# numericalEFT/FeynmanDiagram.jl

Hardware: AMD Instinct MI355X
Metric: graph-evaluations/sec (higher is better)
Workload: dtype f64

## Files before the change

### feynmandiagram.jl_amd/capi.py

```python
from __future__ import annotations

import ctypes as C
import os
from typing import Optional

import numpy as np

from .nodetable import NodeTable

_HERE = os.path.dirname(os.path.abspath(__file__))
LIB_PATH = os.environ.get("FDG_LIBRARY") or os.path.join(_HERE, "lib", "libfdg.so")
KERNEL_CACHE = os.path.join(_HERE, "kernel_cache")

FDG_OK = 0
FDG_E_INVALID, FDG_E_UNSUPPORTED, FDG_E_NO_DEVICE, FDG_E_NOMEM, FDG_E_JIT, FDG_E_INTERNAL = -1, -2, -3, -4, -5, -6
FDG_SPEC_DEFAULT, FDG_SPEC_KEEP_SOURCE, FDG_SPEC_FAST_MATH, FDG_SPEC_ISA, FDG_SPEC_AUTOTUNE = 0, 1, 2, 4, 8
FDG_DT_F64, FDG_DT_F32, FDG_DT_C64, FDG_DT_C32 = 0, 1, 2, 3
DTYPES = {"Float64": FDG_DT_F64, "Float32": FDG_DT_F32, "ComplexF64": FDG_DT_C64, "ComplexF32": FDG_DT_C32}
FDG_SPEC_ROW_MAJOR_COMPANION = 16
FDG_ASSOC_STATIC, FDG_ASSOC_INTERP = 0, 1
FDG_TILE_SAMPLES = 64

EXPORTS = [
    "fdg_last_error", "fdg_version", "fdg_graph_create", "fdg_graph_destroy", "fdg_graph_query",
    "fdg_graph_emit_source", "fdg_free", "fdg_graph_specialize", "fdg_eval_device", "fdg_eval",
    "fdg_accumulate_device", "fdg_fill_uniform_device", "fdg_copy_device", "fdg_read_device", "fdg_clock_probe_device", "fdg_graph_specialize_typed", "fdg_eval_device_typed", "fdg_graph_create_complex_view", "fdg_isa_check_hazards", "fdg_graph_release_device", "fdg_powi",
    "fdg_eval_strided", "fdg_graph_coop_program", "fdg_graph_set_opt_params", "fdg_graph_opt_program", "fdg_graph_set_schedule_groups", "fdg_leaf_eval_device", "fdg_leaf_eval_device_tiled",
    "fdg_comm_unique_id", "fdg_comm_create", "fdg_comm_destroy", "fdg_reduce_device",
    "fdg_graph_specialize_fused", "fdg_mc_eval_device", "fdg_mc_accumulate_device", "fdg_graph_mc_program",
    "fdg_graph_kernel_info",
    "fdg_eval_device_tiled", "fdg_accumulate_device_tiled", "fdg_fill_uniform_device_tiled", "fdg_graph_set_association",
    "fdg_batch_alloc", "fdg_batch_free", "fdg_graph_pool_program", "fdg_batch_alloc_pair", "fdg_graph_set_option", "fdg_graph_get_option", "fdg_set_default_option", "fdg_get_default_option", "fdg_selftest_pair_search",
    "fdg_repack_tile_major", "fdg_unpack_tile_major",
    "fdg_accumulate_device_binned", "fdg_mc_accumulate_device_binned",
    "fdg_accumulate_device_moments", "fdg_mc_accumulate_device_moments",
    "fdg_vegas_sample_device", "fdg_accumulate_device_vegas", "fdg_mc_accumulate_device_vegas", "fdg_vegas_refine",
    "fdg_vegas_sample_device_discrete", "fdg_accumulate_device_vegas_binned", "fdg_mc_accumulate_device_vegas_binned",
    "fdg_vegas_refine_discrete",
    "fdg_vegas_sample_device_polar", "fdg_sincos",
    "fdg_matsubara_phase", "fdg_accumulate_device_matsubara", "fdg_mc_accumulate_device_matsubara",
    "fdg_vegas_sample_device_grouped", "fdg_accumulate_device_grouped", "fdg_mc_accumulate_device_grouped",
    "fdg_accumulate_device_observables", "fdg_mc_accumulate_device_observables",
    "fdg_accumulate_device_freq_observables", "fdg_mc_accumulate_device_freq_observables",
    "fdg_vegas_sample_device_strat", "fdg_accumulate_device_strat", "fdg_mc_accumulate_device_strat", "fdg_strat_allocate",
    "fdg_vegas_sample_device_strat_grouped", "fdg_accumulate_device_strat_grouped", "fdg_mc_accumulate_device_strat_grouped",
    "fdg_strat_allocate_cols",
    "fdg_chain_propose_device", "fdg_chain_step_device", "fdg_mc_chain_step_device", "fdg_chain_reduce_device",
    "fdg_chain_step_device_matsubara", "fdg_mc_chain_step_device_matsubara",
    "fdg_chain_step_device_grouped", "fdg_mc_chain_step_device_grouped",
    "fdg_chain_propose_device_discrete", "fdg_chain_step_device_binned", "fdg_mc_chain_step_device_binned",
    "fdg_chain_propose_device_polar",
]
FDG_BIN_MAX = 16384
FDG_VEGAS_DIM_MAX, FDG_VEGAS_GRID_MAX = 64, 1024
FDG_VEGAS_EXT_MAX = 16
FDG_VEGAS_POLAR_MAX = 21
FDG_MATSUBARA_FREQ_MAX = 64
FDG_WEIGHT_GROUP_MAX = 8
FDG_OBS_MAX = 16
FDG_FREQ_OBS_MAX = 8
FDG_STRAT_CUBE_MAX = 1 << 20
FDG_CHAIN_INIT, FDG_CHAIN_MEASURE = 1, 2
FDG_CHAIN_BIN_MAX = 64
COMM_ID_BYTES = 128


class FdgLibraryMissing(ImportError):
    pass


class FdgError(RuntimeError):
    def __init__(self, code: int, msg: str):
        super().__init__(f"fdg error {code}: {msg}")
        self.code = code


class GraphDesc(C.Structure):
    _fields_ = [("n_leaf", C.c_uint32), ("n_node", C.c_uint32), ("n_root", C.c_uint32), ("n_edge", C.c_uint32),
                ("op", C.POINTER(C.c_uint8)), ("power", C.POINTER(C.c_int32)),
                ("child_off", C.POINTER(C.c_uint32)), ("child_idx", C.POINTER(C.c_uint32)),
                ("child_fac", C.POINTER(C.c_double)), ("root_slot", C.POINTER(C.c_uint32))]


class GraphInfo(C.Structure):
    _fields_ = [("n_leaf", C.c_uint32), ("n_node", C.c_uint32), ("n_root", C.c_uint32), ("n_edge", C.c_uint32),
                ("n_live_node", C.c_uint32), ("n_live_leaf", C.c_uint32),
                ("flops_alg", C.c_uint64), ("bytes_alg", C.c_uint64),
                ("max_live", C.c_uint32), ("n_slot_lds", C.c_uint32), ("n_slot_mem", C.c_uint32),
                ("n_ops", C.c_uint32), ("specialized", C.c_int32),
                ("spec_vgpr", C.c_uint32), ("spec_lds_bytes", C.c_uint32), ("spec_scratch_bytes", C.c_uint32)]

    def asdict(self):
        return {k: int(getattr(self, k)) for k, _ in self._fields_}


class KernelInfo(C.Structure):
    _fields_ = [("last_kernel", C.c_char * 48), ("n_valu", C.c_uint64 * 3), ("n_ld_leaf", C.c_uint32 * 3),
                ("n_panel", C.c_uint32 * 3), ("n_lds", C.c_uint32 * 3), ("waves_per_cu", C.c_uint32 * 3),
                ("has_acc", C.c_uint32), ("has_rm", C.c_uint32), ("has_coop", C.c_uint32), ("rm_bufs", C.c_uint32),
                ("has_pool", C.c_uint32), ("pool_fetch", C.c_uint32), ("pool_valu", C.c_uint64),
                ("has_rl", C.c_uint32), ("rl_reserved", C.c_uint32), ("rl_valu", C.c_uint64)]


class LeafTables(C.Structure):
    _fields_ = [("n_leaf", C.c_uint32), ("n_basis", C.c_uint32), ("n_loop", C.c_uint32), ("dim", C.c_uint32),
                ("n_tau", C.c_uint32), ("leaf_type", C.c_void_p), ("leaf_order", C.c_void_p), ("tau_in", C.c_void_p),
                ("tau_out", C.c_void_p), ("loop_index", C.c_void_p), ("basis", C.c_void_p),
                ("kF", C.c_double), ("beta", C.c_double), ("lambda_", C.c_double)]


class Matsubara(C.Structure):
    _fields_ = [("n_freq", C.c_uint32), ("fermionic", C.c_int32), ("freq", C.c_void_p), ("root_tau_in", C.c_void_p),
                ("root_tau_out", C.c_void_p), ("beta", C.c_double), ("d_T", C.c_void_p), ("t_sample_stride", C.c_int64),
                ("t_comp_stride", C.c_int64), ("n_tau", C.c_uint32), ("d_acc_re", C.c_void_p), ("d_acc_im", C.c_void_p),
                ("d_acc2_re", C.c_void_p), ("d_acc2_im", C.c_void_p)]


class ChainMatsubara(C.Structure):
    _fields_ = [("n_freq", C.c_uint32), ("fermionic", C.c_int32), ("freq", C.c_void_p), ("weight_freq", C.c_uint32),
                ("root_col_in", C.c_void_p), ("root_col_out", C.c_void_p), ("beta", C.c_double)]


class ChainGroups(C.Structure):
    _fields_ = [("n_group", C.c_uint32), ("root_group", C.c_void_p), ("var_mask", C.c_void_p), ("reweight", C.c_void_p)]


class WeightGroups(C.Structure):
    _fields_ = [("n_group", C.c_uint32), ("root_group", C.c_void_p), ("var_mask", C.c_void_p), ("weight_group_stride", C.c_int64)]


class Observables(C.Structure):
    _fields_ = [("n_obs", C.c_uint32), ("coef", C.c_void_p), ("d_obs", C.c_void_p), ("d_cov", C.c_void_p)]


class FreqObservables(C.Structure):
    _fields_ = [("n_obs", C.c_uint32), ("coef", C.c_void_p), ("d_fobs", C.c_void_p), ("d_fcov", C.c_void_p)]


class OptParams(C.Structure):
    _fields_ = [("n_reg", C.c_uint32), ("n_lds", C.c_uint32), ("lookahead_lds", C.c_uint32),
                ("lookahead_mem", C.c_uint32), ("lookahead_leaf", C.c_uint32), ("n_acc", C.c_uint32),
                ("vn_window", C.c_uint32), ("fma", C.c_uint32), ("remat_window", C.c_uint32), ("remat_cost", C.c_uint32)]


class MOp(C.Structure):
    _fields_ = [("kind", C.c_uint8), ("nega", C.c_uint8), ("negb", C.c_uint8), ("negc", C.c_uint8),
                ("d", C.c_uint32), ("a", C.c_uint32), ("b", C.c_uint32), ("imm", C.c_double),
                ("c", C.c_uint32), ("param", C.c_uint32)]


MOP_DTYPE = np.dtype([("kind", "u1"), ("nega", "u1"), ("negb", "u1"), ("negc", "u1"),
                      ("d", "<u4"), ("a", "<u4"), ("b", "<u4"), ("imm", "<f8"), ("c", "<u4"), ("param", "<u4")])

_lib = None


class BatchPairInfo(C.Structure):
    _fields_ = [("leaf_bytes", C.c_uint64), ("root_bytes", C.c_uint64), ("chunk_tiles", C.c_uint64), ("n_chunk", C.c_uint32),
                ("n_candidate", C.c_uint32), ("n_filler", C.c_uint32), ("n_probe", C.c_uint32), ("n_matched", C.c_uint32),
                ("calibrated", C.c_uint32), ("gbs_fast", C.c_double), ("gbs_slow", C.c_double), ("gbs_before_mean", C.c_double),
                ("gbs_before_min", C.c_double), ("gbs_after_mean", C.c_double), ("gbs_after_min", C.c_double), ("seconds", C.c_double),
                ("seconds_settling", C.c_double), ("level_reached", C.c_uint32), ("span_gb", C.c_uint32)]


def lib():
    global _lib
    if _lib is not None:
        return _lib
    if not os.path.exists(LIB_PATH):
        raise FdgLibraryMissing(
            f"{LIB_PATH} not found: build the HIP extension first "
            "(python -c 'import __graft_entry__ as g; g.build()' or make -C feynmandiagram.jl_amd/csrc). "
            "There is no CPU fallback for the evaluator.")
    if not os.environ.get("FDG_NO_TORCH_PRELOAD"):
        try:
            import torch
        except ImportError:
            pass
    L = C.CDLL(LIB_PATH)
    vp, i64, u64, u32, dp = C.c_void_p, C.c_int64, C.c_uint64, C.c_uint32, C.c_void_p
    L.fdg_last_error.restype = C.c_char_p
    L.fdg_version.restype = C.c_int
    L.fdg_graph_create.argtypes = [C.POINTER(GraphDesc), C.POINTER(vp)]
    L.fdg_graph_destroy.argtypes = [vp]
# ... 132 lines not shown
def check(rc: int):
    if rc != 0:
        raise FdgError(rc, lib().fdg_last_error().decode("utf-8", "replace"))


class GraphHandle:

    def __init__(self, table: NodeTable):
        t = table.normalized()
        t.validate()
        self.table = t
        d = GraphDesc()
        d.n_leaf, d.n_node, d.n_root, d.n_edge = t.n_leaf, t.n_node, t.n_root, t.n_edge
        d.op = t.op.ctypes.data_as(C.POINTER(C.c_uint8))
        d.power = t.power.ctypes.data_as(C.POINTER(C.c_int32))
        d.child_off = t.child_off.ctypes.data_as(C.POINTER(C.c_uint32))
        d.child_idx = t.child_idx.ctypes.data_as(C.POINTER(C.c_uint32))
        d.child_fac = t.child_fac.ctypes.data_as(C.POINTER(C.c_double))
        d.root_slot = t.root_slot.ctypes.data_as(C.POINTER(C.c_uint32))
        h = C.c_void_p()
        check(lib().fdg_graph_create(C.byref(d), C.byref(h)))
        self._h = h
        if getattr(t, "sched_group", None) is not None:
            self.set_schedule_groups(t.sched_group)

    def complex_view(self) -> "GraphHandle":
        from .nodetable import complex_to_real
        h = C.c_void_p()
        check(lib().fdg_graph_create_complex_view(self._h, C.byref(h)))
        v = GraphHandle.__new__(GraphHandle)
        v.table = complex_to_real(self.table)
        v._h = h
        return v

    def set_option(self, name: str, value=None):
        check(lib().fdg_graph_set_option(self._h, name.encode(), None if value is None else str(value).encode()))

    def set_options(self, options):
        for k, v in (options or {}).items():
            self.set_option(k, v)

    def get_option(self, name: str):
        v = lib().fdg_graph_get_option(self._h, name.encode())
        return None if v is None else v.decode()

    def set_association(self, assoc: int):
        check(lib().fdg_graph_set_association(self._h, assoc))

    def set_schedule_groups(self, group):
        if group is None:
            check(lib().fdg_graph_set_schedule_groups(self._h, None, 0))
            return
        g = np.ascontiguousarray(group, dtype=np.uint32)
        check(lib().fdg_graph_set_schedule_groups(self._h, g.ctypes.data, g.shape[0]))

    def close(self):
        if getattr(self, "_h", None):
            lib().fdg_graph_destroy(self._h)
            self._h = None

    def __del__(self):
        try:
            self.close()
        except Exception:
            pass

    @property
    def ptr(self):
        return self._h

    def info(self) -> dict:
        gi = GraphInfo()
        check(lib().fdg_graph_query(self._h, C.byref(gi)))
        return gi.asdict()

    def kernel_info(self) -> dict:
        ki = KernelInfo()
        check(lib().fdg_graph_kernel_info(self._h, C.byref(ki)))
        out = {"last_kernel": ki.last_kernel.decode()}
        for k in ("n_valu", "n_ld_leaf", "n_panel", "n_lds", "waves_per_cu"):
            out[k] = [int(x) for x in getattr(ki, k)]
        for k in ("has_acc", "has_rm", "has_coop", "rm_bufs", "has_pool", "pool_fetch", "pool_valu", "has_rl", "rl_valu"):
            out[k] = int(getattr(ki, k))
        return out

    def emit_source(self, flags: int = 0) -> str:
        s = C.c_char_p()
        check(lib().fdg_graph_emit_source(self._h, flags, C.byref(s)))
        try:
            return s.value.decode()
        finally:
            lib().fdg_free(s)

    def set_opt_params(self, n_reg=0, n_lds=0, lookahead_lds=0, lookahead_mem=0, lookahead_leaf=0, n_acc=0, vn_window=0, fma=0, remat_window=0, remat_cost=0):
        q = OptParams(n_reg, n_lds, lookahead_lds, lookahead_mem, lookahead_leaf, n_acc, vn_window, fma, remat_window, remat_cost)
        check(lib().fdg_graph_set_opt_params(self._h, C.byref(q)))

    def opt_program(self, n_reg=0, n_lds=0, lookahead_lds=0, lookahead_mem=0, lookahead_leaf=0, n_acc=0, vn_window=0, fma=0, remat_window=0, remat_cost=0):
        q = OptParams(n_reg, n_lds, lookahead_lds, lookahead_mem, lookahead_leaf, n_acc, vn_window, fma, remat_window, remat_cost)
        ops = C.POINTER(MOp)()
        n = C.c_uint64()
        nr, nl, nm, na = C.c_uint32(), C.c_uint32(), C.c_uint32(), C.c_uint32()
        check(lib().fdg_graph_opt_program(self._h, C.byref(q), C.byref(ops), C.byref(n), C.byref(nr), C.byref(nl),
                                          C.byref(nm), C.byref(na)))
        try:
            buf = C.string_at(ops, n.value * C.sizeof(MOp))
            arr = np.frombuffer(buf, dtype=MOP_DTYPE).copy()
        finally:
            lib().fdg_free(ops)
        self.last_n_acc = na.value
        return arr, nr.value, nl.value, nm.value

    def mc_program(self, tables, n_reg=0, n_lds=0, lookahead_lds=0, lookahead_mem=0, lookahead_leaf=0, n_acc=0, vn_window=0, fma=0, remat_window=0, remat_cost=0):
        q = OptParams(n_reg, n_lds, lookahead_lds, lookahead_mem, lookahead_leaf, n_acc, vn_window, fma, remat_window, remat_cost)
        ops = C.POINTER(MOp)()
        n = C.c_uint64()
        nr, nl, nm, na = C.c_uint32(), C.c_uint32(), C.c_uint32(), C.c_uint32()
        check(lib().fdg_graph_mc_program(self._h, C.byref(tables), C.byref(q), C.byref(ops), C.byref(n), C.byref(nr),
                                         C.byref(nl), C.byref(nm), C.byref(na)))
        try:
            arr = np.frombuffer(C.string_at(ops, n.value * C.sizeof(MOp)), dtype=MOP_DTYPE).copy()
        finally:
            lib().fdg_free(ops)
        return arr, nr.value, nl.value, nm.value

    def pool_program(self, **kw):
        return self.coop_program(_pooled=True, **kw)

    def coop_program(self, _pooled=False, **kw):
        q = OptParams(kw.get("n_reg", 0), kw.get("n_lds", 0), kw.get("lookahead_lds", 0), kw.get("lookahead_mem", 0),
                      kw.get("lookahead_leaf", 0), kw.get("n_acc", 0), kw.get("vn_window", 0), 0, 0, 0)
        progs, per_wave = [], []
        info = None
        for w in range(16):
            ops = C.POINTER(MOp)()
            n = C.c_uint64()
            inf = (C.c_uint32 * 8)()
            rc = (lib().fdg_graph_pool_program if _pooled else lib().fdg_graph_coop_program)(self._h, C.byref(q), w, C.byref(ops), C.byref(n), inf)
            if rc != 0 and w >= 4:
                break
            check(rc)
            try:
                progs.append(np.frombuffer(C.string_at(ops, n.value * C.sizeof(MOp)), dtype=MOP_DTYPE).copy())
            finally:
                lib().fdg_free(ops)
            per_wave.append(dict(n_reg=inf[0], n_lds=inf[1], n_mem=inf[2], n_acc=inf[3]))
            info = dict(n_shared=inf[4], n_epoch=inf[5], n_transfer=inf[6], n_duplicate=inf[7], waves=per_wave)
        return progs, info

    def specialize(self, cache_dir: Optional[str] = None, flags: int = 0):
        check(lib().fdg_graph_specialize(self._h, cache_dir.encode() if cache_dir else None, flags))

    def specialize_typed(self, dtype: int, cache_dir: Optional[str] = None, flags: int = 0):
        check(lib().fdg_graph_specialize_typed(self._h, dtype, cache_dir.encode() if cache_dir else None, flags))

    def eval_device_typed(self, dtype: int, d_leaf: int, ss: int, ls: int, d_root: int, rs: int, rk: int, B: int, stream: int = 0):
        check(lib().fdg_eval_device_typed(self._h, dtype, d_leaf, ss, ls, d_root, rs, rk, B, stream))

    def eval_device(self, d_leaf: int, ss: int, ls: int, d_root: int, rs: int, rk: int, B: int, stream: int = 0):
        check(lib().fdg_eval_device(self._h, d_leaf, ss, ls, d_root, rs, rk, B, stream))

    def accumulate_device(self, d_leaf: int, ss: int, ls: int, d_weight: int, d_acc: int, B: int, stream: int = 0):
        check(lib().fdg_accumulate_device(self._h, d_leaf, ss, ls, d_weight or None, d_acc, B, stream))

    def eval_device_tiled(self, d_leaf: int, ss: int, ls: int, lts: int, d_root: int, rs: int, rk: int, rts: int, B: int, stream: int = 0):
        check(lib().fdg_eval_device_tiled(self._h, d_leaf, ss, ls, lts, d_root, rs, rk, rts, B, stream))
# ... 1367 lines not shown
```

### feynmandiagram.jl_amd/csrc/fdg_internal.h

```cpp
#pragma once
#include <cstdint>
#include <mutex>
#include <string>
#include <vector>

#include "../../include/fdg.h"
#include "fdg_knobs.h"

namespace fdg {

constexpr uint32_t SP_LDS = 0u, SP_MEM = 1u, SP_LEAF = 2u;
constexpr uint32_t LOC_FAC = 1u << 29;
constexpr uint32_t LOC_IDX_MASK = (1u << 29) - 1u;
inline uint32_t mkloc(uint32_t space, uint32_t idx) { return (space << 30) | idx; }

constexpr uint32_t UOP_SUM = 0, UOP_PROD = 1, UOP_POW = 2, UOP_ROOT = 3, UOP_LEAF = 4, UOP_END = 5, UOP_PRODI = 6;

struct Lowered {
  uint32_t L = 0, N = 0, R = 0, E = 0;
  std::vector<uint8_t> op;
  std::vector<int32_t> power;
  std::vector<uint32_t> off, idx;
  std::vector<double> fac;
  std::vector<uint32_t> root_slot;

  std::vector<uint32_t> sched_group;
  bool assoc_interp = false;

  std::vector<uint8_t> live;
  std::vector<uint32_t> order;
  uint32_t n_live_leaf = 0;
  uint64_t flops_alg = 0;
  uint32_t max_live = 0;

  uint32_t lds_slots = 0;
  uint32_t mem_slots = 0;
  std::vector<uint32_t> code;
  uint32_t n_ops = 0;
  uint64_t opnd_lds = 0, opnd_mem = 0, opnd_leaf = 0;
};

int validate_desc(const fdg_graph_desc *d, std::string &err);
struct RealTwinTable { uint32_t n_leaf = 0; std::vector<uint8_t> op; std::vector<int32_t> power; std::vector<uint32_t> off, idx, root_slot; std::vector<double> fac; };
bool complex_to_real_table(const Lowered &p, RealTwinTable &out, std::string &why);
void analyse(Lowered &p);
void build_interpreter_program(Lowered &p, uint32_t lds_slot_budget);

std::string emit_hip_source(const Lowered &p, unsigned flags);
std::string emit_hip_source_typed(const Lowered &p, int dtype, bool &ok, std::string &why);
std::string emit_fused_source(const Lowered &p, const std::string &leaf_stmts, const std::string &device_functions);

void set_error(const std::string &s);

double powi(double x, int32_t n);

}

struct fdg_ws_set {
  void *key = nullptr;
  void *d_ws = nullptr, *d_ws2 = nullptr, *d_ws3 = nullptr, *d_ws4 = nullptr;
  size_t ws_bytes = 0, ws2_bytes = 0, ws3_bytes = 0, ws4_bytes = 0;
  void *s2 = nullptr, *ev_t[2] = {nullptr, nullptr}, *ev_k[2] = {nullptr, nullptr}, *ev_in = nullptr;
  uint64_t last_use = 0;
};

struct fdg_launch_cfg {
  bool no_rl = false, no_fused_acc = false, no_pool = false, pool_no_acc = false, no_streaming = false, no_w2 = false, no_coop = false, no_rm = false;
  bool transpose_narrow = false;
  uint32_t root_scratch_min = 16;
  uint64_t root_scratch_mb = 256;
  int waves_per_cu = 0;
  int oversub = 0;
  long mem_waves = -1;
  long mem_oversub = 1;
  double mem_ratio = 2.5;
  uint64_t sm_chunk_bytes = 1ull << 29;
  long long eval_chunk = 0, mc_chunk = 0;
};

enum { FDG_K_EVAL = 0, FDG_K_NT, FDG_K_W2, FDG_K_ACC, FDG_K_ACC_NT, FDG_K_RM, FDG_K_RM_ACC, FDG_K_RL, FDG_K_RL_ACC, FDG_K_COOP, FDG_K_POOL, FDG_K_COUNT };
static const char *const FDG_ISA_KERNEL[FDG_K_COUNT] = {"fdg_isa_eval", "fdg_isa_eval_nt", "fdg_isa_eval_w2", "fdg_isa_eval_acc", "fdg_isa_eval_acc_nt",
    "fdg_isa_eval_rm", "fdg_isa_eval_rm_acc", "fdg_isa_eval_rl", "fdg_isa_eval_rl_acc", "fdg_isa_eval_coop", "fdg_isa_eval_pool"};
inline const char *fdg_isa_suffix(int k) { return FDG_ISA_KERNEL[k] + sizeof("fdg_isa_eval") - 1; }
struct fdg_isa_kernel {
  bool present = false;
  void *fn = nullptr;
  uint32_t vgpr = 0, lds_bytes = 0, mem_slots = 0, threads = 64;
};

struct fdg_graph {
  fdg::Lowered prog;
  fdg::KnobMap knobs;
  fdg_launch_cfg cfg;
  fdg_opt_params opt = {0, 0, 0, 0, 0, 0, 0, 0, 0, 0};
  bool has_opt = false;
  std::vector<fdg_ws_set> ws_pool;
  void *ws_key = nullptr;
  bool ws_bound = true;
  uint64_t ws_clock = 0;
  std::vector<char> code_object;
  std::string spec_source_hash;
  unsigned spec_flags = 0;
  uint32_t spec_vgpr = 0, spec_lds = 0, spec_scratch = 0;
  std::mutex mu;
  void *d_code = nullptr;
  void *d_root_live = nullptr;
  void *d_ws = nullptr;
  size_t ws_bytes = 0;
  void *module = nullptr;
  void *fn_eval_sm = nullptr, *fn_eval_gen = nullptr;
  bool isa = false;
  bool isa_fma = false;
  fdg_isa_kernel kern[FDG_K_COUNT];
  uint64_t st_valu[3] = {0, 0, 0};
  uint32_t st_ld_leaf[3] = {0, 0, 0}, st_panel[3] = {0, 0, 0}, st_lds[3] = {0, 0, 0};
  const char *last_kernel = "";
  uint32_t rm_bufs = 0;
  uint64_t rl_valu = 0;
  bool coop_enabled = false;
  uint32_t coop_panel_wg = 0;
  uint32_t pool_panel_wg = 0, pool_fetch = 0, pool_unit = 1;
  uint64_t pool_valu = 0;
  std::vector<char> alt_code;
  void *alt_module = nullptr, *fn_alt_sm = nullptr, *fn_alt_gen = nullptr;
  std::vector<char> fused_code;
  void *fused_module = nullptr, *fn_fused = nullptr;
  std::vector<char> typed_code[4];
  void *typed_module[4] = {nullptr, nullptr, nullptr, nullptr}, *fn_typed[4] = {nullptr, nullptr, nullptr, nullptr};
  fdg_graph *cx_twin = nullptr;
  bool cx_twin_tried = false;
  int mc_route = 0;
  std::vector<int32_t> lt_i32[5];
  std::vector<double> lt_basis;
  uint32_t lt_hdr[5] = {0, 0, 0, 0, 0};
  std::vector<char> mc_code;
  void *mc_module = nullptr;
  bool mc_built = false;
  fdg_isa_kernel mc_kern[FDG_K_COUNT];
  std::string mc_dir;
  unsigned mc_flags = 0;
  void *d_ws4 = nullptr;
  size_t ws4_bytes = 0;
  void *d_ws2 = nullptr;
  size_t ws2_bytes = 0;
  void *d_ws3 = nullptr;
  size_t ws3_bytes = 0;
  void *s2 = nullptr;
  void *ev_t[2] = {nullptr, nullptr}, *ev_k[2] = {nullptr, nullptr}, *ev_in = nullptr;
  int device = -1;
  int n_cu = 0;
};

#ifdef FDG_RUNTIME_TU
#include <hip/hip_runtime.h>
#define HIP_TRY(expr)                                                                   \
  do {                                                                                  \
    hipError_t e_ = (expr);                                                             \
    if (e_ != hipSuccess) {                                                             \
      fdg::set_error(std::string(#expr) + ": " + hipGetErrorString(e_));                     \
      return FDG_E_NO_DEVICE;                                                           \
    }                                                                                   \
  } while (0)

__device__ __forceinline__ void philox4x32_10(uint32_t c0, uint32_t c1, uint32_t c2, uint32_t c3,
                                              uint32_t k0, uint32_t k1, uint32_t out[4]) {
#pragma unroll
  for (int r = 0; r < 10; ++r) {
    const uint64_t p0 = (uint64_t)0xD2511F53u * c0;
    const uint64_t p1 = (uint64_t)0xCD9E8D57u * c2;
    const uint32_t n0 = (uint32_t)(p1 >> 32) ^ c1 ^ k0;
    const uint32_t n1 = (uint32_t)p1;
    const uint32_t n2 = (uint32_t)(p0 >> 32) ^ c3 ^ k1;
    const uint32_t n3 = (uint32_t)p0;
    c0 = n0; c1 = n1; c2 = n2; c3 = n3;
    k0 += 0x9E3779B9u; k1 += 0xBB67AE85u;
  }
  out[0] = c0; out[1] = c1; out[2] = c2; out[3] = c3;
}

__device__ __forceinline__ double fdg_philox_u53(uint64_t sample, uint32_t column, uint64_t seed) {
  uint32_t o[4];
  philox4x32_10((uint32_t)sample, (uint32_t)(sample >> 32), column, 0u, (uint32_t)seed, (uint32_t)(seed >> 32), o);
  const uint64_t m = ((uint64_t)(o[0] >> 5) << 26) | (uint64_t)(o[1] >> 6);
  return (double)m * 0x1.0p-53;
}

void parse_launch_cfg(fdg_graph *g);
int ensure_device(fdg_graph *g);
int fdg_bind_stream_ws(fdg_graph *g, void *stream);
int ensure_ws(fdg_graph *g, size_t bytes);
int fdg_run_locked(fdg_graph *g, int mode, const double *d_leaf, int64_t ss, int64_t ls, double *d_root, int64_t rs, int64_t rk,
                   const double *d_weight, double *d_acc, int64_t B, hipStream_t st,
                   int64_t lts = 0, int64_t rts = 0);
int launch_reduce_partials(const double *partial, uint32_t nblk, uint32_t R, double *acc, hipStream_t st);
int ensure_root_scratch(fdg_graph *g, size_t need);
int root_live_mask(fdg_graph *g, const uint8_t **out);
int fdg_mc_run_locked(fdg_graph *g, int mode, const double *d_K, int64_t ks, int64_t kc, const double *d_T, int64_t ts, int64_t tc,
                      double kF, double beta, double lambda, double *d_root, int64_t rs, int64_t rk, const double *d_weight,
                      double *d_acc, int64_t B, hipStream_t st);
// ... 15 lines not shown
```

### feynmandiagram.jl_amd/csrc/fdg_isa.cpp

```cpp
#include <algorithm>
#include <cctype>
#include <cinttypes>
#include <cmath>
#include <cstdio>
#include <cstdlib>
#include <cstring>
#include <map>
#include <sstream>

#include "fdg_opt.h"

namespace fdg {
namespace {

constexpr int V_LANE8 = 1, V_LEAFOFF = 2, V_ROOTOFF = 3, V_TMP = 4, V_BASE = 6;
constexpr int S_LEAF = 4, S_SS = 6, S_LS = 8, S_ROOT = 10, S_RS = 12, S_RK = 14, S_WS = 16, S_B = 18, S_NWG = 20;
constexpr int S_TILE = 22, S_NTILES = 23, S_LT = 24, S_RT = 26, S_PANEL = 28, S_LS8 = 30, S_RK8 = 32, S_A = 34,
              S_T = 36, S_C = 38, S_X = 40;
constexpr int S_WGT = 44;
constexpr int S_RTS = 44;
constexpr int S_LTS = 46;
constexpr int S_LP = 48;
constexpr int S_DELTA = 50;
constexpr int N_DELTA = 6;
constexpr int S_POOL = S_DELTA + 2 * N_DELTA;
constexpr int N_POOL = 20;
constexpr int S_END = S_POOL + 2 * N_POOL;
constexpr int N_POOL_MC = 13;
constexpr int S_PARAM = S_POOL + 2 * N_POOL_MC;
constexpr int S_LEAF2 = S_PARAM + 2 * MC_N_PARAM, S_LS82 = S_LEAF2 + 2, S_LT2 = S_LEAF2 + 4;
static_assert(S_LT2 + 2 == S_END && S_PARAM % 4 == 0 && S_LEAF2 % 4 == 0, "SGPR map");

const double kLog2e = 0x1.71547652b82fep+0, kLn2Hi = 0x1.62e42fefa39efp-1, kLn2Lo = 0x1.abc9e3b39803fp-56;
constexpr int kExpDeg = 11;
const double kExpC[kExpDeg + 1] = {0x1.0000000000000p+0, 0x1.0000000000000p+0, 0x1.0000000000011p-1, 0x1.555555555555ap-3,
                                   0x1.555555554f0a5p-5, 0x1.111111110f218p-7, 0x1.6c16c18804745p-10, 0x1.a01a01b148c00p-13,
                                   0x1.a019919593233p-16, 0x1.71ddf5667e394p-19, 0x1.28b41ab9f014bp-22, 0x1.af63371ef88d9p-26};


enum HzRes : uint8_t { HZ_VGPR, HZ_SGPR  };
enum HzProd : uint8_t {
  HP_TRANS,
  HP_VALU_SGPR,
  HP_VALU_VGPR,
  HP_STORE_WIDE,
  HP_SALU_SGPR,
};
enum HzCons : uint8_t {
  HC_VALU_READ,
  HC_DIV_FMAS,
  HC_VMEM_SADDR,
  HC_LANE_READ,
  HC_VALU_WRITE,
  HC_LDS_DIRECT,
};
struct HzRule { HzProd prod; HzCons cons; HzRes res; int wait; const char *what; };
const HzRule kHazards[] = {
    {HP_TRANS, HC_VALU_READ, HZ_VGPR, 2, "trans result -> VALU read (gfx940: not forwarded; measured: stale read with 0)"},
    {HP_VALU_SGPR, HC_VALU_READ, HZ_SGPR, 2, "VALU write of SGPR/VCC -> VALU read as mask/carry/constant (gfx940; measured with v_cmp -> v_cndmask)"},
    {HP_VALU_SGPR, HC_DIV_FMAS, HZ_SGPR, 4, "VALU write of VCC -> v_div_fmas"},
    {HP_VALU_SGPR, HC_VMEM_SADDR, HZ_SGPR, 5, "VALU write of SGPR -> VMEM/SMEM read of it"},
    {HP_VALU_VGPR, HC_LANE_READ, HZ_VGPR, 2, "VALU write of VGPR -> v_readlane/v_readfirstlane (measured: stale read with 0)"},
    {HP_STORE_WIDE, HC_VALU_WRITE, HZ_VGPR, 2, "store data wider than 64 bits -> VALU overwrite of the data registers"},
    {HP_SALU_SGPR, HC_VMEM_SADDR, HZ_SGPR, 0, "SALU write of SGPR -> VMEM read of it: interlocked by hardware (every leaf load does this back to back)"},
    {HP_SALU_SGPR, HC_LDS_DIRECT, HZ_SGPR, 1, "SALU write of M0 -> LDS-direct load (global_load_lds_*)"},
};
constexpr int HZ_MAX_WAIT = 5;

constexpr int HR_AGPR = 512, HR_SGPR = 1024, HR_VCC = 1024 + 106, HR_EXEC = 1024 + 126, HR_M0 = 1024 + 124;
struct HzInst {
  std::string op;
  bool valu = false, salu = false, vmem = false, ds = false, smem = false, trans = false, lane_read = false, div_fmas = false, store = false, lds_direct = false;
  int nop = 0;
  std::vector<int> wr, rd;
  std::vector<int> store_wide;
};
static bool hz_starts(const std::string &s, const char *p) { return s.compare(0, std::strlen(p), p) == 0; }
static void hz_parse_reg(std::string t, int &first, int &n) {
  first = 0; n = 0;
  while (!t.empty() && (t[0] == '-' || t[0] == '|' || t[0] == ' ')) t.erase(0, 1);
  while (!t.empty() && (t.back() == '|' || t.back() == ' ')) t.pop_back();
  if (t == "vcc") { first = HR_VCC; n = 2; return; }
  if (t == "vcc_lo") { first = HR_VCC; n = 1; return; }
  if (t == "vcc_hi") { first = HR_VCC + 1; n = 1; return; }
  if (t == "exec") { first = HR_EXEC; n = 2; return; }
  if (t == "m0") { first = HR_M0; n = 1; return; }
  if (t.size() < 2 || (t[0] != 'v' && t[0] != 's' && t[0] != 'a')) return;
  const int base = t[0] == 'v' ? 0 : (t[0] == 'a' ? HR_AGPR : HR_SGPR);
  if (t[1] == '[') {
    int a = 0, b = 0;
    if (std::sscanf(t.c_str() + 2, "%d:%d", &a, &b) == 2 && b >= a) { first = base + a; n = b - a + 1; }
    return;
  }
  if (t[1] < '0' || t[1] > '9') return;
  first = base + std::atoi(t.c_str() + 1); n = 1;
}
static HzInst hz_decode(const std::string &line) {
  HzInst I;
  size_t p = 0;
  while (p < line.size() && (line[p] == ' ' || line[p] == '\t')) ++p;
  size_t q = p;
  while (q < line.size() && line[q] != ' ' && line[q] != '\t') ++q;
  I.op = line.substr(p, q - p);
  std::vector<std::string> opnd;
  {
    std::string rest = line.substr(q), cur;
    int depth = 0;
    for (char c : rest) {
      if (c == '[') depth++;
      if (c == ']') depth--;
      if (c == ',' && depth == 0) { opnd.push_back(cur); cur.clear(); } else cur.push_back(c);
    }
    if (!cur.empty()) opnd.push_back(cur);
    for (std::string &o : opnd) {
      while (!o.empty() && (o[0] == ' ' || o[0] == '\t')) o.erase(0, 1);
      const size_t sp = o.find_first_of(" \t");
      if (sp != std::string::npos) o.erase(sp);
    }
  }
  auto add = [](std::vector<int> &v, const std::string &t) { int f, n; hz_parse_reg(t, f, n); for (int i = 0; i < n; ++i) v.push_back(f + i); };
  const std::string &op = I.op;
  if (op == "s_nop") { I.salu = true; I.nop = (opnd.empty() ? 0 : std::atoi(opnd[0].c_str())) + 1; return I; }
  if (hz_starts(op, "s_waitcnt") || op == "s_endpgm" || op == "s_barrier" || hz_starts(op, "s_cbranch") || op == "s_branch") { I.salu = true; return I; }
  if (hz_starts(op, "s_load") || hz_starts(op, "s_buffer_load")) {
    I.smem = true;
    if (!opnd.empty()) add(I.wr, opnd[0]);
    for (size_t i = 1; i < opnd.size(); ++i) add(I.rd, opnd[i]);
    return I;
  }
  if (hz_starts(op, "s_")) {
    I.salu = true;
    const bool nodst = hz_starts(op, "s_cmp") || hz_starts(op, "s_setpc") || hz_starts(op, "s_bitcmp");
    for (size_t i = 0; i < opnd.size(); ++i) add((i == 0 && !nodst) ? I.wr : I.rd, opnd[i]);
    if (hz_starts(op, "s_addc") || hz_starts(op, "s_subb") || hz_starts(op, "s_cselect")) {}
    return I;
  }
  if (hz_starts(op, "global_load") || hz_starts(op, "global_store") || hz_starts(op, "buffer_") || hz_starts(op, "flat_")) {
    I.vmem = true;
    I.store = op.find("store") != std::string::npos;
    if (op.find("_lds_") != std::string::npos) {
      I.lds_direct = true;
      I.rd.push_back(HR_M0);
      for (size_t i = 0; i < opnd.size(); ++i) add(I.rd, opnd[i]);
      return I;
    }
    const bool wide = op.find("dwordx3") != std::string::npos || op.find("dwordx4") != std::string::npos;
    for (size_t i = 0; i < opnd.size(); ++i) {
      if (!I.store && i == 0) add(I.wr, opnd[i]);
      else { add(I.rd, opnd[i]); if (I.store && i == 1 && wide) add(I.store_wide, opnd[i]); }
    }
    return I;
  }
  if (hz_starts(op, "ds_")) {
    I.ds = true;
    I.store = hz_starts(op, "ds_write");
    const bool wide = op.find("b96") != std::string::npos || op.find("b128") != std::string::npos;
    for (size_t i = 0; i < opnd.size(); ++i) {
      if (!I.store && i == 0) add(I.wr, opnd[i]);
      else { add(I.rd, opnd[i]); if (I.store && i == 1 && wide) add(I.store_wide, opnd[i]); }
    }
    return I;
  }
  if (hz_starts(op, "v_")) {
    I.valu = true;
    static const char *trans[] = {"v_rcp_", "v_rsq_", "v_sqrt_", "v_exp_", "v_log_", "v_sin_", "v_cos_"};
    for (const char *t : trans) if (hz_starts(op, t)) I.trans = true;
    I.lane_read = hz_starts(op, "v_readlane") || hz_starts(op, "v_readfirstlane");
    I.div_fmas = hz_starts(op, "v_div_fmas");
    size_t ndst = 1;
    if (hz_starts(op, "v_div_scale") || ((hz_starts(op, "v_add_co") || hz_starts(op, "v_sub_co") || hz_starts(op, "v_addc_co") || hz_starts(op, "v_subb_co")) && opnd.size() >= 4)) ndst = 2;
    if (hz_starts(op, "v_cmpx")) { ndst = 0; I.wr.push_back(HR_EXEC); I.wr.push_back(HR_EXEC + 1); }
    for (size_t i = 0; i < opnd.size(); ++i) add(i < ndst ? I.wr : I.rd, opnd[i]);
    if (I.div_fmas) { I.rd.push_back(HR_VCC); I.rd.push_back(HR_VCC + 1); }
    return I;
  }
  return I;
}
static bool hz_is_inst(const std::string &line) {
  size_t p = 0;
  while (p < line.size() && (line[p] == ' ' || line[p] == '\t')) ++p;
  if (p >= line.size() || line[p] == '.' || line[p] == ';' || line[p] == '/' || line[p] == '-') return false;
  const size_t q = line.find_first_of(" \t", p);
  const std::string w = line.substr(p, q == std::string::npos ? std::string::npos : q - p);
  if (!w.empty() && w.back() == ':') return false;
  return hz_starts(w, "s_") || hz_starts(w, "v_") || hz_starts(w, "ds_") || hz_starts(w, "global_") || hz_starts(w, "buffer_") || hz_starts(w, "flat_");
}

struct HzTracker {
  struct Past { HzInst inst; int age; };
  std::vector<Past> past;
  int missing(const HzInst &I, const char **why = nullptr) const {
    int need = 0;
    auto has = [](const std::vector<int> &v, int r) { return std::find(v.begin(), v.end(), r) != v.end(); };
    for (const Past &P : past) {
      for (const HzRule &R : kHazards) {
        if (R.wait <= P.age) continue;
        const std::vector<int> *pr = nullptr;
        switch (R.prod) {
          case HP_TRANS: if (P.inst.trans) pr = &P.inst.wr; break;
          case HP_VALU_SGPR: if (P.inst.valu) pr = &P.inst.wr; break;
          case HP_VALU_VGPR: if (P.inst.valu) pr = &P.inst.wr; break;
          case HP_STORE_WIDE: if (!P.inst.store_wide.empty()) pr = &P.inst.store_wide; break;
          case HP_SALU_SGPR: if (P.inst.salu) pr = &P.inst.wr; break;
        }
        if (!pr) continue;
        const std::vector<int> *cr = nullptr;
        switch (R.cons) {
          case HC_VALU_READ: if (I.valu && !I.div_fmas) cr = &I.rd; break;
          case HC_DIV_FMAS: if (I.div_fmas) cr = &I.rd; break;
          case HC_VMEM_SADDR: if (I.vmem || I.smem) cr = &I.rd; break;
          case HC_LANE_READ: if (I.lane_read) cr = &I.rd; break;
          case HC_VALU_WRITE: if (I.valu) cr = &I.wr; break;
          case HC_LDS_DIRECT: if (I.lds_direct) cr = &I.rd; break;
        }
        if (!cr) continue;
        for (int r : *pr) {
          const bool sg = r >= HR_SGPR;
          if ((R.res == HZ_SGPR) != sg) continue;
          if (R.cons == HC_LDS_DIRECT && r != HR_M0) continue;
          if (has(*cr, r)) { if (R.wait - P.age > need) { need = R.wait - P.age; if (why) *why = R.what; } break; }
// ... 138 lines not shown

std::string f64_inline(double f, bool &ok) {
  ok = true;
  if (f == 0.5) return "0.5";
  if (f == -0.5) return "-0.5";
  if (f == 2.0) return "2.0";
  if (f == -2.0) return "-2.0";
  if (f == 4.0) return "4.0";
  if (f == -4.0) return "-4.0";
  if (f == 1.0) return "1.0";
  if (f == -1.0) return "-1.0";
  ok = false;
  return "";
}

std::string hex32(uint32_t v) {
  char b[16];
  std::snprintf(b, sizeof b, "0x%08x", v);
  return b;
}

void emit_scaled_addr(Emit &E, int dst, int base, int mul8, uint32_t k) {
  if (k == 0) {
    E.ins("s_mov_b64 s[" + std::to_string(dst) + ":" + std::to_string(dst + 1) + "], s[" + std::to_string(base) + ":" +
          std::to_string(base + 1) + "]");
    return;
  }
  const std::string ks = hex32(k);
  E.ins("s_mul_i32 s" + std::to_string(S_X) + ", s" + std::to_string(mul8) + ", " + ks);
  E.ins("s_mul_hi_u32 s" + std::to_string(S_X + 1) + ", s" + std::to_string(mul8) + ", " + ks);
  E.ins("s_mul_i32 s" + std::to_string(S_X + 2) + ", s" + std::to_string(mul8 + 1) + ", " + ks);
  E.ins("s_add_u32 s" + std::to_string(S_X + 1) + ", s" + std::to_string(S_X + 1) + ", s" + std::to_string(S_X + 2));
  E.ins("s_add_u32 s" + std::to_string(dst) + ", s" + std::to_string(base) + ", s" + std::to_string(S_X));
  E.ins("s_addc_u32 s" + std::to_string(dst + 1) + ", s" + std::to_string(base + 1) + ", s" + std::to_string(S_X + 1));
}

struct KernelMeta { std::string name; uint32_t lds_bytes, accum, n_agpr; int n_args, n_sgpr; uint32_t wg = 64; };

constexpr uint32_t RM_CHUNK = 16, RM_BUF_BYTES = 64 * RM_CHUNK * 8, RM_WINDOW = 800;
struct RmFetch { uint32_t chunk, buf; };
static void rm_plan(const Lowered &p, const OptProgram &prog, uint32_t rm_bufs, std::vector<std::vector<RmFetch>> &rm_fetch,
                    std::vector<int> &rm_ld_buf) {
  const uint32_t rm_full = p.L / RM_CHUNK, rm_tail = (p.L % RM_CHUNK) ? 1u : 0u, n_chunk = rm_full + rm_tail;
  auto rm_chunk_of = [&](uint32_t leaf) { return leaf < rm_full * RM_CHUNK ? leaf / RM_CHUNK : rm_full; };
  const uint32_t G = (prog.params.rm_pair && rm_bufs >= 4 && rm_bufs % 2 == 0) ? 2u : 1u;
  const uint32_t n_unit = (n_chunk + G - 1) / G, n_ubuf = rm_bufs / G;
  const size_t n_ops = prog.ops.size();
  rm_fetch.assign(n_ops + 1, {});
  rm_ld_buf.assign(n_ops, -1);
  std::vector<std::vector<size_t>> uses(n_unit);
  for (size_t q = 0; q < n_ops; ++q) if (prog.ops[q].kind == M_LD_LEAF) uses[rm_chunk_of(prog.ops[q].a) / G].push_back(q);
  std::vector<size_t> cursor(uses.size(), 0);
  std::vector<int64_t> resident(n_ubuf, -1);
  std::vector<size_t> free_from(n_ubuf, 0);
  for (size_t q = 0; q < n_ops; ++q) {
    if (prog.ops[q].kind != M_LD_LEAF) continue;
    const uint32_t c = rm_chunk_of(prog.ops[q].a), u = c / G;
    cursor[u]++;
    int b = -1;
    for (uint32_t k = 0; k < n_ubuf; ++k) if (resident[k] == (int64_t)u) b = (int)k;
    if (b < 0) {
      size_t soon = 1;
      for (size_t k = cursor[u]; k < uses[u].size() && uses[u][k] <= q + RM_WINDOW; ++k) soon++;
      if (soon < 3) continue;
      size_t far = 0;
      for (uint32_t k = 0; k < n_ubuf; ++k) {
        size_t nu;
        if (resident[k] < 0) nu = std::numeric_limits<size_t>::max();
        else { const auto &uu = uses[(size_t)resident[k]]; const size_t cu = cursor[(size_t)resident[k]]; nu = cu < uu.size() ? uu[cu] : std::numeric_limits<size_t>::max() - 1; }
        if (b < 0 || nu > far) { b = (int)k; far = nu; }
      }
      for (uint32_t k = 0; k < G && G * u + k < n_chunk; ++k)
        rm_fetch[std::min(free_from[(size_t)b], q)].push_back(RmFetch{G * u + k, G * (uint32_t)b + k});
      resident[(size_t)b] = u;
    }
    rm_ld_buf[q] = (int)(G * (uint32_t)b + c % G);
    free_from[(size_t)b] = q + 1;
  }
}

struct CoopSec { uint32_t wave, n_shared, priv_base_bytes, panel_wg_bytes, panel_prefix_bytes; bool pooled = false; uint32_t pool_unit = 1;
                 uint32_t slack = 0, flag_base_bytes = 0, n_wave = 4; };
static KernelMeta emit_kernel(Emit &E, const Lowered &p, const OptProgram &prog, const std::string &kname, int W, bool accumulate = false,
                              uint32_t rm_bufs = 0, const CoopSec *cs = nullptr, bool rl = false) {
  E.vm_issued = E.lg_issued = E.vm_done = E.lg_done = 0;
  E.pend.assign(std::max<uint32_t>(prog.n_reg_used, 1), {0, 0});
  const uint32_t SLOT = 512u * W;
  const uint32_t stage_base = (prog.n_lds_used * SLOT + 1023u) & ~1023u;
  const uint32_t rl_image = rl ? ((512u * p.L + 1023u) & ~1023u) : 0u;
  const uint32_t lds_bytes = rl ? stage_base + rl_image : (rm_bufs ? stage_base + rm_bufs * RM_BUF_BYTES : prog.n_lds_used * SLOT);
  const uint32_t panel_bytes_per_wave = std::max<uint32_t>(prog.n_mem_used, 1) * SLOT;
  const int RW = 2 * W;
  const int TSH = W == 2 ? 7 : 6;
  const std::string sfx = "_" + kname;
  std::ostringstream &os = E.os;
  if (!cs) {
    os << "\t.text\n\t.protected\t" << kname << "\n\t.globl\t" << kname << "\n\t.p2align\t8\n\t.type\t" << kname << ",@function\n";
    os << kname << ":\n";
    E.off = 0;
    E.klabel = kname;
    E.pad_ok = true;
    for (int i = 0; i < E.shift; ++i) E.ins("s_nop 0");
  } else {
    os << ".Lsec" << sfx << ":\n";
  }
  auto S = [](int r) { return "s" + std::to_string(r); };
  auto S2 = [](int r) { return "s[" + std::to_string(r) + ":" + std::to_string(r + 1) + "]"; };
  auto V = [](int r) { return "v" + std::to_string(r); };
  auto vlo = [&](uint32_t r) { const int b = V_BASE + RW * r; return "v[" + std::to_string(b) + ":" + std::to_string(b + 1) + "]"; };
  auto vhi = [&](uint32_t r) { const int b = V_BASE + RW * r + 2; return "v[" + std::to_string(b) + ":" + std::to_string(b + 1) + "]"; };
  auto vall = [&](uint32_t r) { const int b = V_BASE + RW * r; return "v[" + std::to_string(b) + ":" + std::to_string(b + RW - 1) + "]"; };
  const std::string LD = W == 2 ? "global_load_dwordx4 " : "global_load_dwordx2 ";
  const std::string ST = W == 2 ? "global_store_dwordx4 " : "global_store_dwordx2 ";
  const std::string leaf_policy_env = fdg::knob("FDG_ISA_LEAF_POLICY") ? std::string(" ") + fdg::knob("FDG_ISA_LEAF_POLICY") : std::string();
  const std::string root_policy = fdg::knob("FDG_ISA_ROOT_POLICY") ? std::string(" ") + fdg::knob("FDG_ISA_ROOT_POLICY") : std::string(E.streaming || (cs && cs->pooled) ? " nt" : "");
  std::vector<uint8_t> final_load(prog.ops.size(), 0);
  if (E.streaming) {
    const long nt_dist = fdg::knob("FDG_ISA_NT_DIST") ? std::atol(fdg::knob("FDG_ISA_NT_DIST")) : E.nt_dist;
    std::vector<long> next_at(p.L + 1, -1);
    long ord = 0;
    for (size_t i = prog.ops.size(); i-- > 0;)
      if ((prog.ops[i].kind == M_LD_LEAF || prog.ops[i].kind == M_LD_LEAF_ACC) && prog.ops[i].a < next_at.size()) {
        const uint32_t a = prog.ops[i].a;
        if (next_at[a] < 0 || (nt_dist >= 0 && ord - next_at[a] > nt_dist)) final_load[i] = 1;
        next_at[a] = ord++;
      }
  }
  std::string leaf_policy = leaf_policy_env;
  const std::string DSR = W == 2 ? "ds_read_b128 " : "ds_read_b64 ";
  const std::string DSW = W == 2 ? "ds_write_b128 " : "ds_write_b64 ";

  const char *dbg = fdg::knob("FDG_ISA_DEBUG");
  const bool dbg_noleaf = dbg && std::strstr(dbg, "noleaf");
  const bool dbg_nolds = dbg && std::strstr(dbg, "nolds");
  const bool use_ldexp = fdg::knob("FDG_ISA_NO_LDEXP") == nullptr;
  const bool dbg_novalu = dbg && std::strstr(dbg, "novalu");
  const bool dbg_nopanel = dbg && std::strstr(dbg, "nopanel");
  const bool dbg_norecv = dbg && std::strstr(dbg, "norecv");
  const bool dbg_nofetch = dbg && std::strstr(dbg, "nopoolfetch");
  const bool dbg_noacc = dbg && std::strstr(dbg, "noacc");
  const bool dbg_nohead = dbg && std::strstr(dbg, "nohead");
  bool in_head = true;
  int tile_run = 0;
  if (dbg && std::strstr(dbg, "chunk") && !cs) tile_run = std::max(0, std::min(9, std::atoi(std::strstr(dbg, "chunk") + 5)));
  const bool tile_xcd = dbg && std::strstr(dbg, "xcd") && !cs && !tile_run;
  int tile_rot = 0;
  if (dbg && std::strstr(dbg, "rot") && !cs && !tile_run && !tile_xcd) tile_rot = std::max(0, std::atoi(std::strstr(dbg, "rot") + 3));
  const int S_ROTB = S_POOL + 2 * (N_POOL - 1), S_ROTS = S_ROTB + 1;
  E.vm_slack = (dbg && std::strstr(dbg, "noackwait") && !accumulate) ? p.R : 0;
  E.no_vm_wait = dbg && std::strstr(dbg, "novmwait");
  if (cs) E.ins("v_and_b32_e32 v0, 63, v0");
  E.ins("s_load_dwordx8 s[4:11], s[0:1], 0x0");
  E.ins("s_load_dwordx8 s[12:19], s[0:1], 0x20");
  E.ins("s_load_dwordx2 s[20:21], s[0:1], 0x40");
  if (accumulate) E.ins("s_load_dwordx2 " + S2(S_WGT) + ", s[0:1], 0x48");
  const uint32_t n_k = prog.mc_n_k;
  const bool mc = n_k > 0 || prog.mc_n_t > 0;
  const bool tm_imm = dbg && std::strstr(dbg, "tmimm") && !mc && !rm_bufs && !rl && !cs && W == 1;
  int64_t tm_base = -1;
  const int tile_arg = mc ? 0x80 : 0x50;
  E.ins("s_load_dwordx2 " + S2(S_LTS) + ", s[0:1], " + hex32((uint32_t)tile_arg));
  if (!accumulate) E.ins("s_load_dwordx2 " + S2(S_RTS) + ", s[0:1], " + hex32((uint32_t)tile_arg + 8));
  if (mc) {
    E.ins("s_load_dwordx4 s[" + std::to_string(S_LEAF2) + ":" + std::to_string(S_LEAF2 + 3) + "], s[0:1], 0x50");
    E.ins("s_load_dwordx8 s[" + std::to_string(S_PARAM) + ":" + std::to_string(S_PARAM + 7) + "], s[0:1], 0x60");
  }
  E.ins("s_waitcnt lgkmcnt(0)");
  uint64_t w_seq = 0;
  const uint32_t acc0 = V_BASE + RW * std::max<uint32_t>(prog.n_reg_used, 1);
  const bool aa = accumulate && prog.params.acc_in_agpr;
  const uint32_t A0 = RW * prog.n_acc_used;
  const uint32_t acc_pairs_v = accumulate ? (aa ? 3 : p.R + 2) : 0;
  const uint32_t wgt0 = aa ? acc0 : acc0 + 2 * p.R;
  auto vpair = [&](uint32_t b) { return "v[" + std::to_string(b) + ":" + std::to_string(b + 1) + "]"; };
  auto vacc = [&](uint32_t k) { return vpair(acc0 + 2 * k); };
  const std::string vwgt = vpair(wgt0), vtmp = vpair(wgt0 + 2), vtmp2 = vpair(wgt0 + 4);
  auto acc_to_tmp2 = [&](uint32_t k) {
    E.ins("v_accvgpr_read_b32 v" + std::to_string(wgt0 + 4) + ", a" + std::to_string(A0 + 2 * k));
    E.ins("v_accvgpr_read_b32 v" + std::to_string(wgt0 + 5) + ", a" + std::to_string(A0 + 2 * k + 1));
  };
  auto tmp2_to_acc = [&](uint32_t k) {
    E.ins("v_accvgpr_write_b32 a" + std::to_string(A0 + 2 * k) + ", v" + std::to_string(wgt0 + 4));
    E.ins("v_accvgpr_write_b32 a" + std::to_string(A0 + 2 * k + 1) + ", v" + std::to_string(wgt0 + 5));
  };
  bool has_macro = false;
  uint32_t n_tmp_pairs = 0;
  for (const MOp &o : prog.ops) { if (mop_is_macro(o.kind)) has_macro = true; n_tmp_pairs = std::max(n_tmp_pairs, mop_tmp_pairs(o.kind)); }
  const uint32_t tmp0 = acc0 + 2 * acc_pairs_v;
  auto tpair = [&](uint32_t k) { return "v[" + std::to_string(tmp0 + 2 * k) + ":" + std::to_string(tmp0 + 2 * k + 1) + "]"; };
  const std::string tA = tpair(0), tB = tpair(1), tC = tpair(2), tD = tpair(3);
  auto tAd = [&](int h) { return "v" + std::to_string(tmp0 + h); };
  if (accumulate)
    for (uint32_t k = 0; k < p.R; ++k) {
      if (aa) {
        E.ins("v_accvgpr_write_b32 a" + std::to_string(A0 + 2 * k) + ", 0");
        E.ins("v_accvgpr_write_b32 a" + std::to_string(A0 + 2 * k + 1) + ", 0");
        continue;
      }
      E.ins("v_mov_b32_e32 v" + std::to_string(acc0 + 2 * k) + ", 0");
      E.ins("v_mov_b32_e32 v" + std::to_string(acc0 + 2 * k + 1) + ", 0");
    }
  E.ins("v_lshlrev_b32_e32 " + V(V_LANE8) + ", " + std::to_string(W == 2 ? 4 : 3) + ", v0");
  E.ins("v_mul_lo_u32 " + V(V_LEAFOFF) + ", v0, " + S(S_SS));
  E.ins("v_lshlrev_b32_e32 " + V(V_LEAFOFF) + ", " + std::to_string(W == 2 ? 4 : 3) + ", " + V(V_LEAFOFF));
  E.ins("v_mul_lo_u32 " + V(V_ROOTOFF) + ", v0, " + S(S_RS));
  E.ins("v_lshlrev_b32_e32 " + V(V_ROOTOFF) + ", " + std::to_string(W == 2 ? 4 : 3) + ", " + V(V_ROOTOFF));
  E.ins("s_lshl_b64 " + S2(S_LS8) + ", " + S2(S_LS) + ", 3");
  E.ins("s_lshl_b64 " + S2(S_RK8) + ", " + S2(S_RK) + ", 3");
  if (mc) E.ins("s_lshl_b64 " + S2(S_LS82) + ", " + S2(S_LS82) + ", 3");
  const uint32_t rm0 = tmp0 + 2 * n_tmp_pairs;
  const int S_ROW8 = S_DELTA, S_FA = S_DELTA + 2;
  if (cs) {
    E.ins("v_add_u32_e32 v" + std::to_string(rm0) + ", " + hex32(cs->priv_base_bytes) + ", " + V(V_LANE8));
    E.ins("v_add_u32_e32 v" + std::to_string(rm0 + 1) + ", 0x10000, " + V(V_LANE8));
    E.ins("v_lshlrev_b32_e32 v" + std::to_string(rm0 + 2) + ", 4, v0");
    if (cs->pooled) {
      E.ins("s_mov_b32 " + S(S_DELTA + 4) + ", 0");
      E.ins("s_mov_b32 " + S(S_DELTA + 5) + ", -1");
    }
    if (cs->slack) {
      E.ins("v_lshlrev_b32_e32 v" + std::to_string(rm0 + 4) + ", 2, v0");
      E.ins("v_add_u32_e32 v" + std::to_string(rm0 + 4) + ", " + hex32(cs->flag_base_bytes + 256u * cs->wave) + ", v" + std::to_string(rm0 + 4));
      E.ins("v_and_b32_e32 v" + std::to_string(rm0 + 5) + ", " + std::to_string(cs->n_wave - 1) + ", v0");
      E.ins("v_lshlrev_b32_e32 v" + std::to_string(rm0 + 5) + ", 8, v" + std::to_string(rm0 + 5));
      E.ins("v_add_u32_e32 v" + std::to_string(rm0 + 5) + ", " + hex32(cs->flag_base_bytes) + ", v" + std::to_string(rm0 + 5));
      E.ins("s_movk_i32 " + S(S_DELTA + 6) + ", 0x400");
      E.ins("v_mov_b32_e32 " + V(V_TMP) + ", " + S(S_DELTA + 6));
      E.ins("ds_write_b32 v" + std::to_string(rm0 + 4) + ", " + V(V_TMP));
      E.ins("s_waitcnt lgkmcnt(0)");
      E.ins("s_barrier");
      E.ins("ds_read_b32 v" + std::to_string(rm0 + 6) + ", v" + std::to_string(rm0 + 5));
      E.ins("s_waitcnt lgkmcnt(0)");
    }
  }
  if (rl) {
    E.ins("v_mul_u32_u24_e32 v" + std::to_string(rm0) + ", " + hex32(8u * p.L) + ", v0");
    E.ins("v_lshlrev_b32_e32 v" + std::to_string(rm0 + 1) + ", 4, v0");
  }
  if (rm_bufs) {
    const std::string vg = "v" + std::to_string(rm0), vg2 = "v" + std::to_string(rm0 + 9);
    auto vj = [&](int j) { return "v" + std::to_string(rm0 + 1 + j); };
    E.ins("v_lshrrev_b32_e32 " + vj(0) + ", 3, v0");
    E.ins("v_mul_lo_u32 " + vj(0) + ", " + vj(0) + ", " + S(S_SS));
    E.ins("v_lshlrev_b32_e32 " + vj(0) + ", 3, " + vj(0));
    E.ins("v_lshrrev_b32_e32 " + vj(1) + ", 4, v0");
    E.ins("v_and_b32_e32 " + vj(2) + ", 7, v0");
    E.ins("v_xor_b32_e32 " + vj(1) + ", " + vj(1) + ", " + vj(2));
    E.ins("v_xor_b32_e32 " + vj(2) + ", 4, " + vj(1));
    E.ins("v_lshlrev_b32_e32 " + vj(1) + ", 4, " + vj(1));
    E.ins("v_lshlrev_b32_e32 " + vj(2) + ", 4, " + vj(2));
    E.ins("v_add_u32_e32 " + vg + ", " + vj(0) + ", " + vj(1));
    E.ins("v_add_u32_e32 " + vg2 + ", " + vj(0) + ", " + vj(2));
    E.ins("v_lshlrev_b32_e32 " + V(V_TMP) + ", 7, v0");
    E.ins("v_bfe_u32 " + V(V_TMP + 1) + ", v0, 1, 3");
    for (int j = 0; j < 8; ++j) {
      E.ins("v_xor_b32_e32 " + vj(j) + ", " + std::to_string(j) + ", " + V(V_TMP + 1));
      E.ins("v_lshlrev_b32_e32 " + vj(j) + ", 4, " + vj(j));
      E.ins("v_add_u32_e32 " + vj(j) + ", " + vj(j) + ", " + V(V_TMP));
    }
    E.ins("s_lshl_b64 " + S2(S_ROW8) + ", " + S2(S_SS) + ", 6");
  }
  std::vector<int64_t> delta_tab;
  {
    std::map<int64_t, int> hist;
    int64_t last = -1;
    for (const MOp &o : prog.ops) if (o.kind == M_LD_LEAF || o.kind == M_LD_LEAF_ACC) {
      const bool same_space = !mc || (o.a < n_k && last < (int64_t)n_k);
      if (last >= 0 && same_space && (int64_t)o.a - last > 1) hist[(int64_t)o.a - last]++;
      last = o.a;
    }
    std::vector<std::pair<int, int64_t>> v;
    for (auto &kv : hist) if (kv.second >= 2) v.push_back({kv.second, kv.first});
    std::sort(v.begin(), v.end(), [](const auto &x, const auto &y) { return x.first > y.first || (x.first == y.first && x.second < y.second); });
    for (size_t i = 0; i < v.size() && i < (size_t)N_DELTA && !rm_bufs && !rl; ++i) delta_tab.push_back(v[i].second);
  }
  for (size_t k = 0; k < delta_tab.size(); ++k) {
    const int d = S_DELTA + 2 * (int)k;
    const std::string ks = hex32((uint32_t)delta_tab[k]);
    E.ins("s_mul_i32 " + S(d) + ", " + S(S_LS8) + ", " + ks);
    E.ins("s_mul_hi_u32 " + S(d + 1) + ", " + S(S_LS8) + ", " + ks);
    E.ins("s_mul_i32 " + S(S_X) + ", " + S(S_LS8 + 1) + ", " + ks);
    E.ins("s_add_u32 " + S(d + 1) + ", " + S(d + 1) + ", " + S(S_X));
  }
  std::vector<uint64_t> pool;
  {
    std::map<uint64_t, int> hist;
    auto count = [&](double f) { bool inl; f64_inline(f, inl); if (!inl) { uint64_t u; std::memcpy(&u, &f, 8); hist[u]++; } };
    for (const MOp &o : prog.ops) {
      if ((o.kind == M_MULC || o.kind == M_FMAC || o.kind == M_ADDC || o.kind == M_FIXZ || o.kind == M_SELC || o.kind == M_FMAK) && !o.param) count(o.imm);
      if (o.kind == M_EXP) { count(kLog2e); count(-kLn2Hi); count(-kLn2Lo); for (int k = 0; k <= kExpDeg; ++k) count(kExpC[k]); }
    }
    std::vector<std::pair<int, uint64_t>> v;
    for (auto &kv : hist) v.push_back({kv.second, kv.first});
    std::sort(v.begin(), v.end(), [](const auto &x, const auto &y) { return x.first > y.first || (x.first == y.first && x.second < y.second); });
    for (size_t i = 0; i < v.size() && i < (size_t)(mc ? N_POOL_MC : (has_macro ? N_POOL : 16)); ++i) pool.push_back(v[i].second);
  }
  for (size_t k = 0; k < pool.size(); ++k) {
    E.ins("s_mov_b32 " + S(S_POOL + 2 * (int)k) + ", " + hex32((uint32_t)pool[k]));
    E.ins("s_mov_b32 " + S(S_POOL + 2 * (int)k + 1) + ", " + hex32((uint32_t)(pool[k] >> 32)));
  }
  E.ins("s_add_u32 " + S(S_X) + ", " + S(S_B) + ", " + std::to_string((1 << TSH) - 1));
  E.ins("s_addc_u32 " + S(S_X + 1) + ", " + S(S_B + 1) + ", 0");
  E.ins("s_lshr_b64 " + S2(S_X) + ", " + S2(S_X) + ", " + std::to_string(TSH));
  E.ins("s_mov_b32 " + S(S_NTILES) + ", " + S(S_X));
  if (tile_run) E.ins("s_lshl_b32 " + S(S_TILE) + ", s2, " + std::to_string(tile_run));
  else if (tile_xcd) {
    E.ins("s_and_b32 " + S(S_X) + ", s2, 7");
    E.ins("s_add_u32 " + S(S_T) + ", " + S(S_NTILES) + ", 7");
    E.ins("s_lshr_b32 " + S(S_T) + ", " + S(S_T) + ", 3");
    E.ins("s_mul_i32 " + S(S_A) + ", " + S(S_X) + ", " + S(S_T));
    E.ins("s_lshr_b32 " + S(S_A + 1) + ", s2, 3");
    E.ins("s_add_u32 " + S(S_TILE) + ", " + S(S_A) + ", " + S(S_A + 1));
    E.ins("s_add_u32 " + S(S_A) + ", " + S(S_A) + ", " + S(S_T));
    E.ins("s_min_u32 " + S(S_NTILES) + ", " + S(S_A) + ", " + S(S_NTILES));
  }
  else {
    E.ins("s_mov_b32 " + S(S_TILE) + ", s2");
    if (tile_rot) { E.ins("s_mov_b32 " + S(S_ROTB) + ", 0"); E.ins("s_mov_b32 " + S(S_ROTS) + ", s2"); }
  }
  E.ins("s_mul_i32 " + S(S_X) + ", s2, " + hex32(cs ? cs->panel_wg_bytes : panel_bytes_per_wave));
  E.ins("s_mul_hi_u32 " + S(S_X + 1) + ", s2, " + hex32(cs ? cs->panel_wg_bytes : panel_bytes_per_wave));
  E.ins("s_add_u32 " + S(S_PANEL) + ", " + S(S_WS) + ", " + S(S_X));
  E.ins("s_addc_u32 " + S(S_PANEL + 1) + ", " + S(S_WS + 1) + ", " + S(S_X + 1));
  if (cs && cs->panel_prefix_bytes) {
    E.ins("s_add_u32 " + S(S_PANEL) + ", " + S(S_PANEL) + ", " + hex32(cs->panel_prefix_bytes));
    E.ins("s_addc_u32 " + S(S_PANEL + 1) + ", " + S(S_PANEL + 1) + ", 0");
  }
  std::map<uint32_t, int> panel_base;
  if (!mc) {
    std::map<uint32_t, uint64_t> hist;
    for (const MOp &o : prog.ops) {
      if (o.kind != M_LD_MEM && o.kind != M_ST_MEM) continue;
      const uint32_t slot = o.kind == M_LD_MEM ? o.a : o.d;
      const uint64_t byte = (uint64_t)slot * SLOT;
      if (byte >= 4096) hist[(uint32_t)((byte + 4096) / 8192)]++;
    }
    std::vector<std::pair<uint64_t, uint32_t>> v;
    for (auto &kv : hist) v.push_back({kv.second, kv.first});
    std::sort(v.begin(), v.end(), [](const auto &x, const auto &y) { return x.first > y.first || (x.first == y.first && x.second < y.second); });
    for (size_t i = 0; i < v.size() && pool.size() + i < (size_t)N_POOL; ++i) {
      const int r = S_POOL + 2 * (int)(pool.size() + i);
      panel_base[v[i].second] = r;
      E.ins("s_add_u32 " + S(r) + ", " + S(S_PANEL) + ", " + hex32(v[i].second * 8192u));
      E.ins("s_addc_u32 " + S(r + 1) + ", " + S(S_PANEL + 1) + ", 0");
    }
  }
  E.ins("s_cmp_ge_u32 " + S(S_TILE) + ", " + S(S_NTILES));
  E.ins("s_cbranch_scc0 .Ltile" + sfx);
  E.ins("s_endpgm");
  os << ".Ltile" << sfx << ":\n";
  if (cs && cs->slack) E.ins("s_mov_b32 " + S(S_DELTA + 7) + ", " + S(S_DELTA + 6));
  E.ins("s_mov_b32 " + S(S_X + 1) + ", 0");
  E.ins("s_mov_b32 " + S(S_X) + ", " + S(S_TILE));
  E.ins("s_lshl_b64 " + S2(S_X) + ", " + S2(S_X) + ", " + std::to_string(TSH));
  if (W == 1) {
    E.ins("s_sub_u32 " + S(S_T) + ", " + S(S_B) + ", " + S(S_X));
    E.ins("s_subb_u32 " + S(S_T + 1) + ", " + S(S_B + 1) + ", " + S(S_X + 1));
    E.ins("s_cmp_lg_u32 " + S(S_T + 1) + ", 0");
    E.ins("s_cselect_b32 " + S(S_T) + ", 64, " + S(S_T));
    E.ins("s_min_u32 " + S(S_T) + ", " + S(S_T) + ", 64");
    E.ins("s_bfm_b64 " + S2(S_A) + ", " + S(S_T) + ", 0");
    E.ins("s_cmp_ge_u32 " + S(S_T) + ", 64");
    E.ins("s_cselect_b64 exec, -1, " + S2(S_A));
  }
  auto tile_base = [&](int dst, int base, int stride) {
    E.ins("s_mul_i32 " + S(S_A) + ", " + S(S_TILE) + ", " + S(stride));
    E.ins("s_mul_hi_u32 " + S(S_A + 1) + ", " + S(S_TILE) + ", " + S(stride));
    E.ins("s_mul_i32 " + S(S_T) + ", " + S(S_TILE) + ", " + S(stride + 1));
    E.ins("s_add_u32 " + S(S_A + 1) + ", " + S(S_A + 1) + ", " + S(S_T));
    E.ins("s_lshl_b64 " + S2(S_A) + ", " + S2(S_A) + ", 3");
    E.ins("s_add_u32 " + S(dst) + ", " + S(base) + ", " + S(S_A));
    E.ins("s_addc_u32 " + S(dst + 1) + ", " + S(base + 1) + ", " + S(S_A + 1));
  };
  tile_base(S_LT, S_LEAF, S_LTS);
  if (mc) tile_base(S_LT2, S_LEAF2, S_LTS);
  if (!accumulate) tile_base(S_RT, S_ROOT, S_RTS);
  if (accumulate) {
    E.ins("v_mov_b32_e32 v" + std::to_string(wgt0) + ", 0");
    E.ins("v_mov_b32_e32 v" + std::to_string(wgt0 + 1) + ", 0x3ff00000");
    E.ins("s_cmp_eq_u64 " + S2(S_WGT) + ", 0");
    E.ins("s_cbranch_scc1 .Lnow" + sfx);
    E.ins("s_lshl_b64 " + S2(S_A) + ", " + S2(S_X) + ", 3");
    E.ins("s_add_u32 " + S(S_A) + ", " + S(S_A) + ", " + S(S_WGT));
    E.ins("s_addc_u32 " + S(S_A + 1) + ", " + S(S_A + 1) + ", " + S(S_WGT + 1));
    E.ins("global_load_dwordx2 " + vwgt + ", " + V(V_LANE8) + ", " + S2(S_A));
    os << ".Lnow" << sfx << ":\n";
    w_seq = ++E.vm_issued;
  }

  uint64_t rl_ready = 0;
  if (rl) {
    const uint32_t n_inst = (512u * p.L + 1023u) / 1024u;
    E.ins("s_mov_b64 " + S2(S_DELTA + 2) + ", " + S2(S_LT));
    for (uint32_t n = 0; n < n_inst; ++n) {
      if (n && n % 4 == 0) {
        E.ins("s_add_u32 " + S(S_DELTA + 2) + ", " + S(S_DELTA + 2) + ", 0x1000");
        E.ins("s_addc_u32 " + S(S_DELTA + 3) + ", " + S(S_DELTA + 3) + ", 0");
      }
      const bool half = (n + 1) * 1024u > 512u * p.L;
      if (half) E.ins("s_mov_b64 exec, 0xffffffff");
      if (n % 4 == 0 || half) E.ins("s_mov_b32 m0, " + hex32(stage_base + (n / 4) * 4096u));
      E.ins("global_load_lds_dwordx4 v" + std::to_string(rm0 + 1) + ", " + S2(S_DELTA + 2) + " offset:" + std::to_string((n % 4) * 1024u) + " nt");
      if (half) E.ins("s_mov_b64 exec, -1");
      ++E.vm_issued;
    }
    rl_ready = E.vm_issued;
  }
  auto panel_operand = [&](uint32_t slot) -> std::string {
    const uint64_t byte = (uint64_t)slot * SLOT;
    const uint64_t hi = byte & ~4095ull, lo = byte & 4095ull;
    if (hi == 0) return S2(S_PANEL) + " offset:" + std::to_string(lo);
    const auto it = panel_base.find((uint32_t)((byte + 4096) / 8192));
    if (it != panel_base.end()) return S2(it->second) + " offset:" + std::to_string((int64_t)byte - (int64_t)it->first * 8192);
    E.ins("s_add_u32 " + S(S_A) + ", " + S(S_PANEL) + ", " + hex32((uint32_t)hi));
    E.ins("s_addc_u32 " + S(S_A + 1) + ", " + S(S_PANEL + 1) + ", " + hex32((uint32_t)(hi >> 32)));
    return S2(S_A) + " offset:" + std::to_string(lo);
  };
  auto valu2 = [&](const std::string &opc, const MOp &o, const std::string &second_lo, const std::string &second_hi) {
    E.ins(opc + vlo(o.d) + ", " + (o.nega ? "-" : "") + vlo(o.a) + ", " + second_lo);
    if (W == 2) E.ins(opc + vhi(o.d) + ", " + (o.nega ? "-" : "") + vhi(o.a) + ", " + second_hi);
  };

  auto const_operand = [&](double imm) -> std::string {
    bool inl;
    std::string c = f64_inline(imm, inl);
    if (inl) return c;
    uint64_t u;
    std::memcpy(&u, &imm, 8);
    for (size_t k = 0; k < pool.size(); ++k) if (pool[k] == u) return S2(S_POOL + 2 * (int)k);
    E.ins("s_mov_b32 " + S(S_C) + ", " + hex32((uint32_t)u));
    E.ins("s_mov_b32 " + S(S_C + 1) + ", " + hex32((uint32_t)(u >> 32)));
    return S2(S_C);
  };
  auto const_sgpr = [&](double imm) -> int {
// ... 414 lines not shown
        E.wait_reg(o.c);
        E.wait_reg(o.d);
        const std::string k = o.kind == M_FMAC ? op_const(o) : std::string();
        for (int h = 0; h < W; ++h) {
          auto part = [&](uint32_t r) { return h ? vhi(r) : vlo(r); };
          E.ins("v_fma_f64 " + part(o.d) + ", " + (o.nega ? "-" : "") + part(o.a) + ", " +
                (o.kind == M_FMA ? (o.negb ? "-" : "") + part(o.b) : k) + ", " + (o.negc ? "-" : "") + part(o.c));
        }
        break;
      }
      case M_LD_ACC:
        if (dbg_noacc) break;
        E.wait_reg(o.d);
        if (o.a < E.pend_acc.size() && E.pend_acc[o.a]) { E.wait_vm(E.pend_acc[o.a]); E.pend_acc[o.a] = 0; }
        for (int k = 0; k < RW; ++k)
          E.ins("v_accvgpr_read_b32 v" + std::to_string(V_BASE + RW * o.d + k) + ", a" + std::to_string(RW * o.a + k));
        break;
      case M_ST_ACC:
        if (dbg_noacc) break;
        E.wait_reg(o.a);
        for (int k = 0; k < RW; ++k)
          E.ins("v_accvgpr_write_b32 a" + std::to_string(RW * o.d + k) + ", v" + std::to_string(V_BASE + RW * o.a + k));
        break;
      case M_ROOT: {
        E.wait_reg(o.a);
        if (accumulate) {
          if (w_seq > E.vm_done) {
            const uint64_t n = std::min<uint64_t>(E.vm_issued - w_seq, 63);
            E.ins("s_waitcnt vmcnt(" + std::to_string(n) + ")");
            E.vm_done = std::max(E.vm_done, std::max(E.vm_issued - n, w_seq));
          }
          E.ins("v_mul_f64 " + vtmp + ", " + vwgt + ", " + (o.nega ? "-" : "") + vlo(o.a));
          if (aa) {
            acc_to_tmp2(o.d);
            E.ins("v_add_f64 " + vtmp2 + ", " + vtmp2 + ", " + vtmp);
            tmp2_to_acc(o.d);
            break;
          }
          E.ins("v_add_f64 " + vacc(o.d) + ", " + vacc(o.d) + ", " + vtmp);
          break;
        }
        emit_scaled_addr(E, S_A, S_RT, S_RK8, o.d);
        for (int h = 0; h < W; ++h) {
          const int src = V_BASE + RW * o.a + 2 * h;
          if (h == 1) {
            E.ins("s_lshl_b64 " + S2(S_T) + ", " + S2(S_RS) + ", 3");
            E.ins("s_add_u32 " + S(S_A) + ", " + S(S_A) + ", " + S(S_T));
            E.ins("s_addc_u32 " + S(S_A + 1) + ", " + S(S_A + 1) + ", " + S(S_T + 1));
          }
          if (o.nega) {
            E.ins("v_mov_b32_e32 " + V(V_TMP) + ", v" + std::to_string(src));
            E.ins("v_xor_b32_e32 " + V(V_TMP + 1) + ", 0x80000000, v" + std::to_string(src + 1));
            E.ins("global_store_dwordx2 " + V(V_ROOTOFF) + ", v[" + std::to_string(V_TMP) + ":" + std::to_string(V_TMP + 1) + "], " + S2(S_A) + root_policy);
          } else {
            E.ins("global_store_dwordx2 " + V(V_ROOTOFF) + ", v[" + std::to_string(src) + ":" + std::to_string(src + 1) + "], " + S2(S_A) + root_policy);
          }
          ++E.vm_issued;
        }
        break;
      }
      default:
        break;
    }
  }
  for (uint32_t r = 0; r < E.pend.size(); ++r) E.wait_reg(r);
  E.ins("s_waitcnt lgkmcnt(0)");
  if (tile_run) {
    E.ins("s_add_u32 " + S(S_TILE) + ", " + S(S_TILE) + ", 1");
    E.ins("s_and_b32 " + S(S_X) + ", " + S(S_TILE) + ", " + std::to_string((1 << tile_run) - 1));
    E.ins("s_cbranch_scc1 .Lrun" + sfx);
    E.ins("s_lshl_b32 " + S(S_X) + ", " + S(S_NWG) + ", " + std::to_string(tile_run));
    E.ins("s_add_u32 " + S(S_TILE) + ", " + S(S_TILE) + ", " + S(S_X));
    E.ins("s_sub_u32 " + S(S_TILE) + ", " + S(S_TILE) + ", " + std::to_string(1 << tile_run));
    os << ".Lrun" << sfx << ":\n";
  } else if (tile_xcd) {
    E.ins("s_lshr_b32 " + S(S_X) + ", " + S(S_NWG) + ", 3");
    E.ins("s_add_u32 " + S(S_TILE) + ", " + S(S_TILE) + ", " + S(S_X));
  } else if (tile_rot) {
    E.ins("s_add_u32 " + S(S_ROTB) + ", " + S(S_ROTB) + ", " + S(S_NWG));
    E.ins("s_add_u32 " + S(S_ROTS) + ", " + S(S_ROTS) + ", " + std::to_string(tile_rot));
    E.ins("s_sub_u32 " + S(S_X) + ", " + S(S_NWG) + ", 1");
    E.ins("s_and_b32 " + S(S_ROTS) + ", " + S(S_ROTS) + ", " + S(S_X));
    E.ins("s_add_u32 " + S(S_TILE) + ", " + S(S_ROTB) + ", " + S(S_ROTS));
  } else {
    E.ins("s_add_u32 " + S(S_TILE) + ", " + S(S_TILE) + ", " + S(S_NWG));
  }
  E.ins("s_cmp_ge_u32 " + S(S_TILE) + ", " + S(S_NTILES));
  E.ins("s_cbranch_scc0 .Lback" + sfx);
  if (accumulate) {
    E.ins("s_mov_b64 exec, -1");
    E.ins("v_lshlrev_b32_e32 " + V(V_TMP) + ", 2, v0");
    if (aa)
      for (uint32_t k = 0; k < p.R; ++k) {
        acc_to_tmp2(k);
        for (int off = 32; off >= 1; off >>= 1) {
          E.ins("v_xor_b32_e32 " + V(V_TMP + 1) + ", " + std::to_string(off * 4) + ", " + V(V_TMP));
          E.ins("ds_bpermute_b32 v" + std::to_string(wgt0 + 2) + ", " + V(V_TMP + 1) + ", v" + std::to_string(wgt0 + 4));
          E.ins("ds_bpermute_b32 v" + std::to_string(wgt0 + 3) + ", " + V(V_TMP + 1) + ", v" + std::to_string(wgt0 + 5));
          E.ins("s_waitcnt lgkmcnt(0)");
          E.ins("v_add_f64 " + vtmp2 + ", " + vtmp2 + ", " + vtmp);
        }
        tmp2_to_acc(k);
      }
    for (int off = 32; off >= 1 && !aa; off >>= 1) {
      E.ins("v_xor_b32_e32 " + V(V_TMP + 1) + ", " + std::to_string(off * 4) + ", " + V(V_TMP));
      for (uint32_t k = 0; k < p.R; ++k) {
        const uint32_t a = acc0 + 2 * k, t = acc0 + 2 * (p.R + 1);
        E.ins("ds_bpermute_b32 v" + std::to_string(t) + ", " + V(V_TMP + 1) + ", v" + std::to_string(a));
        E.ins("ds_bpermute_b32 v" + std::to_string(t + 1) + ", " + V(V_TMP + 1) + ", v" + std::to_string(a + 1));
        E.ins("s_waitcnt lgkmcnt(0)");
        E.ins("v_add_f64 " + vacc(k) + ", " + vacc(k) + ", " + vtmp);
      }
    }
    E.ins("s_mov_b64 exec, 1");
    E.ins("v_mov_b32_e32 " + V(V_TMP) + ", 0");
    E.ins("s_lshl_b32 " + S(S_X) + ", s2, 3");
    E.ins("s_add_u32 " + S(S_A) + ", " + S(S_ROOT) + ", " + S(S_X));
    E.ins("s_addc_u32 " + S(S_A + 1) + ", " + S(S_ROOT + 1) + ", 0");
    E.ins("s_lshl_b32 " + S(S_T) + ", " + S(S_NWG) + ", 3");
    for (uint32_t k = 0; k < p.R; ++k) {
      if (aa) acc_to_tmp2(k);
      E.ins("global_store_dwordx2 " + V(V_TMP) + ", " + (aa ? vtmp2 : vacc(k)) + ", " + S2(S_A));
      E.ins("s_add_u32 " + S(S_A) + ", " + S(S_A) + ", " + S(S_T));
      E.ins("s_addc_u32 " + S(S_A + 1) + ", " + S(S_A + 1) + ", 0");
    }
  }
  E.ins("s_endpgm");
  os << ".Lback" << sfx << ":\n";
  E.ins("s_getpc_b64 " + S2(S_A));
  os << ".Lpc" << sfx << ":\n";
  E.ins("s_add_u32 " + S(S_A) + ", " + S(S_A) + ", (.Ltile" + sfx + "-.Lpc" + sfx + ")&0xffffffff");
  E.ins("s_addc_u32 " + S(S_A + 1) + ", " + S(S_A + 1) + ", (.Ltile" + sfx + "-.Lpc" + sfx + ")>>32");
  E.ins("s_setpc_b64 " + S2(S_A));
  E.ins("s_endpgm");

  const uint32_t next_vgpr = std::max<uint32_t>(V_BASE + RW * std::max<uint32_t>(prog.n_reg_used, 1) + 2 * acc_pairs_v + 2 * n_tmp_pairs + (rm_bufs ? 10 : 0) + (cs ? (cs->slack ? 7 : 4) : 0) + (rl ? 2 : 0), 8);
  const uint32_t accum = (next_vgpr + 3) & ~3u;
  const uint32_t n_agpr = RW * prog.n_acc_used + (aa ? 2 * p.R : 0);
  if (cs) return KernelMeta{kname, lds_bytes, accum, n_agpr, 12, (mc || has_macro) ? S_END : S_POOL + 2 * 16};
  os << "\t.section\t.rodata,\"a\",@progbits\n\t.p2align\t6, 0x0\n\t.amdhsa_kernel " << kname << "\n";
  os << "\t\t.amdhsa_group_segment_fixed_size " << lds_bytes << "\n";
  os << "\t\t.amdhsa_private_segment_fixed_size 0\n\t\t.amdhsa_kernarg_size " << (mc ? 144 : 96) << "\n\t\t.amdhsa_user_sgpr_count 2\n";
  os << "\t\t.amdhsa_user_sgpr_kernarg_segment_ptr 1\n\t\t.amdhsa_system_sgpr_workgroup_id_x 1\n";
  os << "\t\t.amdhsa_system_vgpr_workitem_id 0\n";
  const int n_sgpr = (mc || has_macro) ? S_END : S_POOL + 2 * 16;
  os << "\t\t.amdhsa_next_free_vgpr " << (accum + n_agpr) << "\n\t\t.amdhsa_next_free_sgpr " << n_sgpr << "\n";
  os << "\t\t.amdhsa_accum_offset " << accum << "\n\t\t.amdhsa_reserve_vcc 1\n";
  os << "\t\t.amdhsa_float_round_mode_32 0\n\t\t.amdhsa_float_round_mode_16_64 0\n";
  os << "\t\t.amdhsa_float_denorm_mode_32 3\n\t\t.amdhsa_float_denorm_mode_16_64 3\n";
  os << "\t\t.amdhsa_dx10_clamp 1\n\t\t.amdhsa_ieee_mode 1\n";
  os << "\t.end_amdhsa_kernel\n";
  (void)p;
  return KernelMeta{kname, lds_bytes, accum, n_agpr, mc ? 18 : 12, n_sgpr};
}

}

static KernelMeta emit_coop(Emit &E, const Lowered &p, const CoopProgram &cp, const std::string &kname) {
  std::ostringstream &os = E.os;
  os << "\t.text\n\t.protected\t" << kname << "\n\t.globl\t" << kname << "\n\t.p2align\t8\n\t.type\t" << kname << ",@function\n";
  os << kname << ":\n";
  E.off = 0;
  E.klabel = kname;
  const char *ca = fdg::knob("FDG_COOP_ALIGN");
  E.pad_ok = ca ? ca[0] == '1' : cp.pooled;
  const int align_before = E.align;
  if (cp.pooled && !ca && E.align == 1) E.align = 2;
  E.hz.reset();
  E.ins("v_lshrrev_b32_e32 v1, 6, v0");
  E.ins("v_readfirstlane_b32 s3, v1");
  for (uint32_t w = 0; w < cp.n_wave; ++w) {
    const std::string lab = ".Lsec_" + kname + "_w" + std::to_string(w), here = ".Lpc_" + kname + "_d" + std::to_string(w);
    E.ins("s_cmp_lg_u32 s3, " + std::to_string(w));
    E.ins("s_cbranch_scc1 .Lnot_" + kname + "_" + std::to_string(w));
    E.ins("s_getpc_b64 s[4:5]");
    os << here << ":\n";
    E.ins("s_add_u32 s4, s4, (" + lab + "-" + here + ")&0xffffffff");
    E.ins("s_addc_u32 s5, s5, (" + lab + "-" + here + ")>>32");
    E.ins("s_setpc_b64 s[4:5]");
    os << ".Lnot_" << kname << "_" << w << ":\n";
  }
  E.ins("s_endpgm");
  uint32_t panel_wg = 0, prefix[CoopProgram::MAXW];
  for (uint32_t w = 0; w < cp.n_wave; ++w) { prefix[w] = panel_wg; panel_wg += std::max<uint32_t>(cp.wave[w].n_mem_used, 1) * 512u; }
  uint32_t accum = 0, n_agpr = 0;
  int n_sgpr = 0;
  for (uint32_t w = 0; w < cp.n_wave; ++w) {
    const CoopSec cs{w, cp.n_shared, (cp.n_shared + w * cp.n_priv_lds) * 512u, panel_wg, prefix[w], cp.pooled, cp.pool_unit,
                     cp.pooled ? cp.slack : 0u, (cp.n_shared + cp.n_wave * cp.n_priv_lds) * 512u, cp.n_wave};
    E.hz.reset();
    const KernelMeta m = emit_kernel(E, p, cp.wave[w], kname + "_w" + std::to_string(w), 1, false, 0, &cs);
    accum = std::max(accum, m.accum); n_agpr = std::max(n_agpr, m.n_agpr); n_sgpr = std::max(n_sgpr, m.n_sgpr);
  }
  const uint32_t lds_bytes = (cp.n_shared + cp.n_wave * cp.n_priv_lds) * 512u + (cp.pooled && cp.slack ? 256u * cp.n_wave : 0u);
  E.align = align_before;
  os << "\t.section\t.rodata,\"a\",@progbits\n\t.p2align\t6, 0x0\n\t.amdhsa_kernel " << kname << "\n";
  os << "\t\t.amdhsa_group_segment_fixed_size " << lds_bytes << "\n";
  os << "\t\t.amdhsa_private_segment_fixed_size 0\n\t\t.amdhsa_kernarg_size 96\n\t\t.amdhsa_user_sgpr_count 2\n";
  os << "\t\t.amdhsa_user_sgpr_kernarg_segment_ptr 1\n\t\t.amdhsa_system_sgpr_workgroup_id_x 1\n";
  os << "\t\t.amdhsa_system_vgpr_workitem_id 0\n";
  os << "\t\t.amdhsa_next_free_vgpr " << (accum + n_agpr) << "\n\t\t.amdhsa_next_free_sgpr " << n_sgpr << "\n";
  os << "\t\t.amdhsa_accum_offset " << accum << "\n\t\t.amdhsa_reserve_vcc 1\n";
  os << "\t\t.amdhsa_float_round_mode_32 0\n\t\t.amdhsa_float_round_mode_16_64 0\n";
  os << "\t\t.amdhsa_float_denorm_mode_32 3\n\t\t.amdhsa_float_denorm_mode_16_64 3\n";
  os << "\t\t.amdhsa_dx10_clamp 1\n\t\t.amdhsa_ieee_mode 1\n";
  os << "\t.end_amdhsa_kernel\n";
  return KernelMeta{kname, lds_bytes, accum, n_agpr, 12, n_sgpr};
}

void rm_plan_stats(const Lowered &p, const OptProgram &prog, uint32_t bufs, uint64_t &fetches, uint64_t &gathers) {
  std::vector<std::vector<RmFetch>> f;
  std::vector<int> ld;
  rm_plan(p, prog, bufs, f, ld);
  fetches = gathers = 0;
  for (const auto &v : f) fetches += v.size();
  for (size_t q = 0; q < prog.ops.size(); ++q) if (prog.ops[q].kind == M_LD_LEAF && ld[q] < 0) gathers++;
}

int check_isa_hazards(const std::string &text, std::string &report) {
  HzTracker hz;
  std::istringstream in(text);
  std::string line;
  std::ostringstream rep;
  long lineno = 0, n_inst = 0, n_bad = 0, n_nop = 0, n_trans = 0, n_sgpr_w = 0;
  while (std::getline(in, line)) {
    ++lineno;
    if (!hz_is_inst(line)) continue;
    const HzInst I = hz_decode(line);
    ++n_inst;
    if (I.nop) n_nop++;
    if (I.trans) n_trans++;
    if (I.valu) for (int r : I.wr) if (r >= HR_SGPR) { n_sgpr_w++; break; }
    const char *why = nullptr;
    const int need = hz.missing(I, &why);
    if (need > 0) {
      ++n_bad;
      if (n_bad <= 50) rep << "line " << lineno << ": " << line << "   ; " << need << " more wait state(s): " << (why ? why : "") << "\n";
    }
    hz.issue(I);
  }
  rep << "checked " << n_inst << " instructions (" << n_trans << " transcendental, " << n_sgpr_w << " VALU writes of SGPR/VCC, " << n_nop
      << " s_nop) against " << (sizeof(kHazards) / sizeof(kHazards[0])) << " rules: " << n_bad << " violation(s)\n";
  report = rep.str();
  return (int)n_bad;
}

std::string isa_hazard_table() {
  std::ostringstream os;
  for (const HzRule &R : kHazards) os << R.wait << " wait state(s): " << R.what << "\n";
  return os.str();
}

std::string emit_isa(const Lowered &p, const IsaPrograms &V, std::vector<IsaKernelRecord> *records) {
  const OptProgram &prog = *V.main, *prog2 = V.w2_prog(), *prog_acc = V.acc_prog(), *prog_rm = V.rm_prog(), *prog_rm_acc = V.rm_acc_prog(), *prog_rl = V.rl_prog(),
                   *prog_rl_acc = V.rl_acc_prog();
  const CoopProgram *coop = V.coop_prog(), *pool = V.pool_prog();
  const std::string &kname = V.kname;
  const uint32_t rm_bufs = V.rm_bufs;
  Emit E;
  { const char *a = fdg::knob("FDG_ISA_ALIGN"); E.align = a && a[0] >= '0' && a[0] <= '2' ? a[0] - '0' : 1; }
  { const char *a = fdg::knob("FDG_ISA_SHIFT"); E.shift = a ? std::atoi(a) : 0; }
  E.check_off = fdg::knob("FDG_ISA_CHECK_OFF") != nullptr;
  E.os << "\t.amdgcn_target \"amdgcn-amd-amdhsa--gfx950\"\n\t.amdhsa_code_object_version 6\n";
  std::vector<KernelMeta> ks;
  const bool long_program = prog.ops.size() > 60000 && prog.mc_n_k == 0 && prog.mc_n_t == 0 && !fdg::knob("FDG_ISA_NO_STREAMING");
  E.streaming = long_program;
  E.nt_dist = long_program ? 512 : -1;
  ks.push_back(emit_kernel(E, p, prog, kname, 1));
  E.streaming = false;
  if (prog2) ks.push_back(emit_kernel(E, p, *prog2, kname + "_w2", 2));
  if (prog_acc) {
    E.streaming = long_program && prog_acc->ops.size() > 60000;
    ks.push_back(emit_kernel(E, p, *prog_acc, kname + "_acc", 1, true));
    E.streaming = false;
  }
  E.nt_dist = -1;
  if (!fdg::knob("FDG_ISA_NO_STREAMING") && prog.ops.size() <= 60000 && prog.mc_n_k == 0 && prog.mc_n_t == 0) {
    E.streaming = true;
    ks.push_back(emit_kernel(E, p, prog, kname + "_nt", 1));
    if (prog_acc && prog_acc->ops.size() <= 60000) ks.push_back(emit_kernel(E, p, *prog_acc, kname + "_acc_nt", 1, true));
    E.streaming = false;
  }
  if (prog_rm) ks.push_back(emit_kernel(E, p, *prog_rm, kname + "_rm", 1, false, rm_bufs));
  if (prog_rm_acc) ks.push_back(emit_kernel(E, p, *prog_rm_acc, kname + "_rm_acc", 1, true, rm_bufs));
  if (prog_rl) ks.push_back(emit_kernel(E, p, *prog_rl, kname + "_rl", 1, false, 0, nullptr, true));
  if (prog_rl_acc) ks.push_back(emit_kernel(E, p, *prog_rl_acc, kname + "_rl_acc", 1, true, 0, nullptr, true));
  if (coop) { ks.push_back(emit_coop(E, p, *coop, kname + "_coop")); ks.back().wg = 64 * coop->n_wave; }
  if (pool) { ks.push_back(emit_coop(E, p, *pool, kname + "_pool")); ks.back().wg = 64 * pool->n_wave; }
  std::ostringstream &os = E.os;
  os << "\t.text\n\t.amdgpu_metadata\n---\namdhsa.kernels:\n";
  const char *kinds[18] = {"global_buffer", "by_value", "by_value", "global_buffer", "by_value", "by_value",
                           "global_buffer", "by_value", "by_value", "global_buffer", "global_buffer", "by_value",
                           "by_value", "by_value", "by_value", "by_value", "by_value", "by_value"};
  for (const KernelMeta &k : ks) {
    os << "  - .agpr_count: " << k.n_agpr << "\n    .args:\n";
    for (int i = 0; i < k.n_args; ++i) {
      const char *kind = (k.n_args == 12 && i >= 10) ? "by_value" : kinds[i];
      os << "      - .offset: " << i * 8 << "\n        .size: 8\n        .value_kind: " << kind << "\n";
      if (std::strcmp(kind, "global_buffer") == 0) os << "        .address_space: global\n";
    }
    os << "    .group_segment_fixed_size: " << k.lds_bytes << "\n    .kernarg_segment_align: 8\n    .kernarg_segment_size: " << 8 * k.n_args << "\n";
    os << "    .max_flat_workgroup_size: " << k.wg << "\n    .name: " << k.name << "\n    .private_segment_fixed_size: 0\n";
    os << "    .sgpr_count: " << (k.n_sgpr + 6) << "\n    .sgpr_spill_count: 0\n    .symbol: " << k.name << ".kd\n";
    os << "    .uniform_work_group_size: 1\n    .uses_dynamic_stack: false\n    .vgpr_count: " << (k.accum + k.n_agpr)
       << "\n    .vgpr_spill_count: 0\n    .wavefront_size: 64\n";
  }
  if (records) for (const KernelMeta &k : ks) records->push_back(IsaKernelRecord{k.name, k.accum + k.n_agpr, k.lds_bytes, k.wg});
  os << "amdhsa.target: amdgcn-amd-amdhsa--gfx950\namdhsa.version:\n  - 1\n  - 2\n...\n\t.end_amdgpu_metadata\n";
  return os.str();
}

}
```

### feynmandiagram.jl_amd/csrc/fdg_opt.h

```cpp
#pragma once
#include <cstdint>
#include <string>
#include <vector>

#include "fdg_internal.h"

namespace fdg {

enum MKind : uint8_t {
  M_LD_LEAF = 0,
  M_LD_LDS,
  M_LD_MEM,
  M_ST_LDS,
  M_ST_MEM,
  M_MUL,
  M_ADD,
  M_MULC,
  M_ROOT,
  M_MOV,
  M_LD_ACC,
  M_ST_ACC,
  M_FMA = 14,
  M_FMAC = 15,
  M_ADDC = 16,
// ... 34 lines not shown
  uint32_t n_lds = 80;
  uint32_t n_acc = 0;
  uint32_t lookahead_lds = 32;
  uint32_t lookahead_mem = 128;
  uint32_t vn_window = 200;
  uint32_t lookahead_leaf = 300;
  bool fma = false;
  uint32_t remat_window = 0;
  uint32_t remat_cost = 4;
  bool roots_last = false;
  bool keep_root_order = false;
  uint32_t n_land = 0;
  uint32_t lookahead_land = 1500;
  bool keep_minus_one = false;
  bool mul_keeps_signs = false;
  bool acc_in_agpr = false;
  bool pool_leaves = false;
  bool leaves_once = false;
  bool rm_pair = false;
  uint32_t reserve_pairs = 0;
};

struct OptProgram {
  OptParams params;
  std::vector<MOp> ops;
  uint32_t n_reg_used = 0, n_lds_used = 0, n_mem_used = 0, n_acc_used = 0;
  uint64_t n_valu = 0, n_ld_leaf = 0, n_ld_lds = 0, n_ld_mem = 0, n_st_lds = 0, n_st_mem = 0, n_ld_acc = 0, n_st_acc = 0;
  uint64_t n_send = 0, n_recv = 0, n_barrier = 0;
  uint64_t n_ld_land = 0;
  uint32_t max_live = 0;
  uint32_t mc_n_k = 0, mc_n_t = 0;
  bool supported = true;
  std::string why;
};

void build_opt_program(const Lowered &p, const OptParams &prm, OptProgram &out);

struct LeafSpec {
  const fdg_leaf_tables *tab = nullptr;
  double kF = 0, beta = 0, lambda = 0;
};
void build_mc_program(const Lowered &p, const LeafSpec &ls, const OptParams &prm, OptProgram &out);

struct SchedOp { uint8_t kind; uint32_t d, a, b; double imm; };
bool build_schedule(const Lowered &p, const OptParams &prm, std::vector<SchedOp> &ops, uint32_t &n_value, std::string &why);
struct CoopProgram {
  static constexpr uint32_t MAXW = 16;
  uint32_t n_wave = 4;
  OptProgram wave[MAXW];
  uint32_t n_shared = 0;
  uint32_t n_priv_lds = 0;
  uint32_t n_epoch = 0;
  uint64_t n_transfer = 0;
  uint64_t n_duplicate = 0;
  bool pooled = false;
  uint32_t pool_unit = 1;
  uint32_t slack = 0;
  uint64_t n_fetch = 0;
  bool supported = false;
  std::string why;
};
void build_coop_program(const Lowered &p, const OptParams &prm, CoopProgram &out, uint32_t n_wave = 4);
void build_pool_program(const Lowered &p, const OptParams &prm, CoopProgram &out, uint32_t n_wave = 8, uint32_t epoch_ops = 0, uint32_t ahead = 0);

struct IsaPrograms {
  const OptProgram *main = nullptr;
  std::string kname = "fdg_isa_eval";
  OptProgram p2, pa, pr, pra, prl, prla;
  CoopProgram coop, pool;
  bool w2 = false, acc = false, rm_acc = false, rl = false, rl_acc = false;
  uint32_t rm_bufs = 0;
  int coop_verdict = -1;
  const OptProgram *w2_prog() const { return w2 ? &p2 : nullptr; }
  const OptProgram *acc_prog() const { return acc ? &pa : nullptr; }
  const OptProgram *rm_prog() const { return rm_bufs ? &pr : nullptr; }
  const OptProgram *rm_acc_prog() const { return rm_bufs && rm_acc ? &pra : nullptr; }
  const OptProgram *rl_prog() const { return rl ? &prl : nullptr; }
  const OptProgram *rl_acc_prog() const { return rl && rl_acc ? &prla : nullptr; }
  const CoopProgram *coop_prog() const { return coop.supported ? &coop : nullptr; }
  const CoopProgram *pool_prog() const { return pool.supported ? &pool : nullptr; }
};
struct IsaKernelRecord { std::string name; uint32_t vgpr = 0 , lds_bytes = 0, threads = 64; };
std::string emit_isa(const Lowered &p, const IsaPrograms &V, std::vector<IsaKernelRecord> *records = nullptr);

void rm_plan_stats(const Lowered &p, const OptProgram &prog, uint32_t bufs, uint64_t &fetches, uint64_t &gathers);
int check_isa_hazards(const std::string &text, std::string &report);
std::string isa_hazard_table();

}
```

### feynmandiagram.jl_amd/csrc/fdg_runtime.hip

```cpp
#include <hip/hip_runtime.h>
#include <hip/hiprtc.h>
#include <fcntl.h>
#include <sys/stat.h>
#include <sys/wait.h>
#include <unistd.h>

#include <atomic>
#include <cstdio>
#include <cstdlib>
#include <cstring>
#include <fstream>
#include <sstream>

#define FDG_RUNTIME_TU 1
#include "fdg_internal.h"
#include "fdg_opt.h"
#include "fdg_powi.h"

using namespace fdg;


typedef const __attribute__((address_space(4))) uint32_t cword;

__device__ __forceinline__ double fdg_block_sum256(double v, double *sh) {
// ... 474 lines not shown
  if (g->d_code) return FDG_OK;
  const size_t nb = g->prog.code.size() * sizeof(uint32_t);
  HIP_TRY(hipMalloc(&g->d_code, nb));
  HIP_TRY(hipMemcpy(g->d_code, g->prog.code.data(), nb, hipMemcpyHostToDevice));
  return FDG_OK;
}

int root_live_mask(fdg_graph *g, const uint8_t **out) {
  *out = nullptr;
  const Lowered &p = g->prog;
  bool any = false;
  for (uint32_t k = 0; k < p.R; ++k) any = any || p.root_slot[k] == FDG_NO_ROOT;
  if (!any) return FDG_OK;
  if (!g->d_root_live) {
    std::vector<uint8_t> m(p.R);
    for (uint32_t k = 0; k < p.R; ++k) m[k] = p.root_slot[k] != FDG_NO_ROOT;
    HIP_TRY(hipMalloc(&g->d_root_live, p.R));
    HIP_TRY(hipMemcpy(g->d_root_live, m.data(), p.R, hipMemcpyHostToDevice));
  }
  *out = (const uint8_t *)g->d_root_live;
  return FDG_OK;
}

static uint32_t isa_waves_per_cu(uint32_t vgpr, uint32_t lds_bytes) {
  const uint32_t valloc = std::max<uint32_t>(8, (vgpr + 7) & ~7u);
  uint32_t per_cu = std::min<uint32_t>(8, 512 / valloc) * 4;
  if (lds_bytes) per_cu = std::min<uint32_t>(per_cu, (160u * 1024u) / lds_bytes);
  return std::max<uint32_t>(1, std::min<uint32_t>(per_cu, 32));
}

static int resolve_isa_kernels(hipModule_t m, const std::string &kname, fdg_isa_kernel *kern) {
  for (int k = 0; k < FDG_K_COUNT; ++k) {
    if (!kern[k].present) continue;
    hipFunction_t f;
    const hipError_t e = hipModuleGetFunction(&f, m, (kname + fdg_isa_suffix(k)).c_str());
    if (e != hipSuccess) { hipModuleUnload(m); set_error("kernel " + kname + fdg_isa_suffix(k) + " is missing from its code object: " + hipGetErrorString(e)); return FDG_E_NO_DEVICE; }
    kern[k].fn = f;
  }
  return FDG_OK;
}
static void forget_isa_kernels(fdg_isa_kernel *kern) { for (int k = 0; k < FDG_K_COUNT; ++k) kern[k].fn = nullptr; }

static int ensure_module(fdg_graph *g) {
  if (g->module || g->code_object.empty()) return FDG_OK;
  hipModule_t m;
  hipError_t e = hipModuleLoadData(&m, g->code_object.data());
  if (e != hipSuccess) { set_error("hipModuleLoadData failed: " + std::string(hipGetErrorString(e))); return FDG_E_JIT; }
  if (g->isa) {
    const int rc = resolve_isa_kernels(m, "fdg_isa_eval", g->kern);
    if (rc) return rc;
    g->module = m;
    return FDG_OK;
  }
  hipFunction_t f1, f2;
  HIP_TRY(hipModuleGetFunction(&f1, m, "fdg_spec_sm"));
  HIP_TRY(hipModuleGetFunction(&f2, m, "fdg_spec_gen"));
  g->module = m; g->fn_eval_sm = f1; g->fn_eval_gen = f2;
  int v = 0;
  if (hipFuncGetAttribute(&v, HIP_FUNC_ATTRIBUTE_NUM_REGS, f1) == hipSuccess) g->spec_vgpr = (uint32_t)v;
  if (hipFuncGetAttribute(&v, HIP_FUNC_ATTRIBUTE_SHARED_SIZE_BYTES, f1) == hipSuccess) g->spec_lds = (uint32_t)v;
  if (hipFuncGetAttribute(&v, HIP_FUNC_ATTRIBUTE_LOCAL_SIZE_BYTES, f1) == hipSuccess) g->spec_scratch = (uint32_t)v;
  return FDG_OK;
}

void parse_launch_cfg(fdg_graph *g) {
  fdg_launch_cfg c;
  auto get = [&](const char *n) -> const char * { auto it = g->knobs.find(n); return it == g->knobs.end() ? nullptr : it->second.c_str(); };
  c.no_rl = get("FDG_ISA_NO_RL") != nullptr;
  c.no_fused_acc = get("FDG_ISA_NO_FUSED_ACC") != nullptr;
  c.no_pool = get("FDG_ISA_NO_POOL") != nullptr;
  c.pool_no_acc = get("FDG_ISA_POOL_NO_ACC") != nullptr;
  c.no_streaming = get("FDG_ISA_NO_STREAMING") != nullptr;
  c.no_w2 = get("FDG_ISA_NO_W2") != nullptr;
  c.no_coop = get("FDG_ISA_NO_COOP") != nullptr;
  c.no_rm = get("FDG_ISA_NO_RM") != nullptr;
  c.transpose_narrow = get("FDG_TRANSPOSE_NARROW") != nullptr;
  if (const char *e = get("FDG_ROOT_SCRATCH_MIN")) c.root_scratch_min = (uint32_t)std::max(0, std::atoi(e));
  if (const char *e = get("FDG_ROOT_SCRATCH_MB")) c.root_scratch_mb = (uint64_t)std::max(1, std::atoi(e));
  if (const char *e = get("FDG_ISA_WAVES_PER_CU")) c.waves_per_cu = std::max(1, std::atoi(e));
  if (const char *e = get("FDG_ISA_OVERSUB")) c.oversub = std::max(1, std::atoi(e));
  if (const char *e = get("FDG_ISA_MEM_WAVES")) c.mem_waves = std::max(0l, std::atol(e));
  if (const char *e = get("FDG_ISA_MEM_OVERSUB")) c.mem_oversub = std::max(1l, std::atol(e));
  if (const char *e = get("FDG_ISA_MEM_RATIO")) c.mem_ratio = std::atof(e);
  if (const char *e = get("FDG_SM_CHUNK_MB")) c.sm_chunk_bytes = (uint64_t)std::max(1, std::atoi(e)) << 20;
  if (const char *e = get("FDG_EVAL_CHUNK")) c.eval_chunk = std::atoll(e);
  if (const char *e = get("FDG_MC_CHUNK")) c.mc_chunk = std::atoll(e);
  g->cfg = c;
}

static int run(fdg_graph *g, int mode, const double *d_leaf, int64_t ss, int64_t ls, double *d_root,
               int64_t rs, int64_t rk, const double *d_weight, double *d_acc, int64_t B, hipStream_t st,
               int64_t lts = 0, int64_t rts = 0) {
  if (!g) { set_error("null handle"); return FDG_E_INVALID; }
  if (B < 0) { set_error("n_sample < 0"); return FDG_E_INVALID; }
  if (B == 0) return FDG_OK;
  if ((g->prog.L && !d_leaf) || (mode == 0 && g->prog.R && !d_root) || (mode == 1 && !d_acc)) {
    set_error("null device buffer"); return FDG_E_INVALID;
  }
  if (mode == 1 && g->prog.R == 0) return FDG_OK;
  std::lock_guard<std::mutex> lk(g->mu);
  fdg::KnobScope knob_scope(&g->knobs);
  { const int rcb = fdg_bind_stream_ws(g, (void *)st); if (rcb) return rcb; }
  return fdg_run_locked(g, mode, d_leaf, ss, ls, d_root, rs, rk, d_weight, d_acc, B, st, lts, rts);
}

static int launch_hip_source(fdg_graph *g, hipFunction_t fn, int mode, const double *d_leaf, int64_t ss, int64_t ls, double *d_root,
                             int64_t rs, int64_t rk, const double *d_weight, double *d_acc, int64_t B, hipStream_t st) {
  const uint32_t R = g->prog.R;
  const long nblk = (long)((B + 255) / 256);
  const long grid = std::min<long>(nblk, (long)g->n_cu * 8);
  double *partial = nullptr;
  if (mode == 1) {
    int rc = ensure_ws(g, (size_t)grid * R * sizeof(double));
    if (rc) return rc;
    partial = (double *)g->d_ws;
  }
  long a_ss = ss, a_ls = ls, a_rs = rs, a_rk = rk, a_B = B;
  int a_mode = mode;
  void *args[] = {(void *)&d_leaf, &a_ss, &a_ls, (void *)&d_root, &a_rs, &a_rk, (void *)&d_weight,
                  (void *)&partial, &a_B, &a_mode};
  HIP_TRY(hipModuleLaunchKernel(fn, (unsigned)grid, 1, 1, 256, 1, 1, 0, st, args, nullptr));
  if (mode == 1) {
    hipLaunchKernelGGL(fdg_reduce_partials, dim3(std::min<uint32_t>(R, 64u)), dim3(256), 0, st, partial,
                       (uint32_t)grid, R, d_acc);
    HIP_TRY(hipGetLastError());
  }
  return FDG_OK;
}

namespace {
struct RunArgs {
  int mode;
  const double *d_leaf; int64_t ss, ls;
  double *d_root; int64_t rs, rk;
  const double *d_weight; double *d_acc;
  int64_t B; hipStream_t st;
  int64_t lts, rts;
};
inline bool root_stride_ok(const RunArgs &a) { return !(a.rs < 0 || a.rs >= (1ll << 23)); }
}

int ensure_root_scratch(fdg_graph *g, size_t need) {
  if (g->ws2_bytes >= need) return FDG_OK;
  if (g->d_ws2) { HIP_TRY(hipDeviceSynchronize()); HIP_TRY(hipFree(g->d_ws2)); g->d_ws2 = nullptr; g->ws2_bytes = 0; }
  if (hipMalloc(&g->d_ws2, need) != hipSuccess) { set_error("hipMalloc(root scratch) failed"); return FDG_E_NOMEM; }
  g->ws2_bytes = need;
  return FDG_OK;
}

namespace {

int run_through_root_scratch(fdg_graph *g, const RunArgs &a) {
  const uint32_t R = g->prog.R;
  long Bc = std::max<long>(64, (long)((g->cfg.root_scratch_mb << 20) / (8ull * R)) & ~63l);
  Bc = std::min<long>(Bc, (long)((a.B + 63) & ~(int64_t)63));
  int rc = ensure_root_scratch(g, (size_t)Bc * R * sizeof(double) + (size_t)2048 * R * sizeof(double));
  if (rc) return rc;
  double *scratch = (double *)g->d_ws2;
  const uint8_t *live = nullptr;
  rc = root_live_mask(g, &live);
  if (rc) return rc;
  for (long c0 = 0; c0 < (long)a.B; c0 += Bc) {
    const long n = std::min<long>(Bc, (long)a.B - c0);
    const double *lf = a.lts ? a.d_leaf + (size_t)(c0 / 64) * (size_t)a.lts : a.d_leaf + (size_t)c0 * (size_t)a.ss;
    rc = fdg_run_locked(g, 0, lf, a.ss, a.ls, scratch, 1, Bc, nullptr, nullptr, n, a.st, a.lts, 0);
    if (rc) return rc;
    const long ntile = ((n + 63) / 64) * ((R + 31) / 32);
    hipLaunchKernelGGL(fdg_transpose_from_leaf_major, dim3((unsigned)std::min<long>(ntile, (long)g->n_cu * 16)), dim3(256), 0, a.st,
                       scratch, Bc, a.d_root + (size_t)c0 * (size_t)a.rs, (long)a.rs, (long)a.rk, n, R, live);
    HIP_TRY(hipGetLastError());
  }
  return FDG_OK;
}

int run_companion(fdg_graph *g, const RunArgs &a) {
  if (!g->alt_module) {
    hipModule_t m; hipFunction_t f1, f2;
    hipError_t e = hipModuleLoadData(&m, g->alt_code.data());
    if (e != hipSuccess) { set_error("hipModuleLoadData failed: " + std::string(hipGetErrorString(e))); return FDG_E_JIT; }
    HIP_TRY(hipModuleGetFunction(&f1, m, "fdg_spec_sm"));
    HIP_TRY(hipModuleGetFunction(&f2, m, "fdg_spec_gen"));
    g->alt_module = m; g->fn_alt_sm = f1; g->fn_alt_gen = f2;
  }
  g->last_kernel = "fdg_spec_sm";
  return launch_hip_source(g, (hipFunction_t)g->fn_alt_sm, a.mode, a.d_leaf, a.ss, a.ls, a.d_root, a.rs, a.rk, a.d_weight, a.d_acc, a.B, a.st);
}

int run_interpreter(fdg_graph *g, const RunArgs &a) {
  const Lowered &p = g->prog;
  const uint32_t R = p.R;
  const int mode = a.mode;
  const long nblk = (long)((a.B + 255) / 256);
  g->last_kernel = "fdg_interp";
  int rc = ensure_code(g);
  if (rc) return rc;
  const bool staged = (a.ls == 1 && a.ss != 1 && p.L > 0);
  const size_t lds_bytes = ((size_t)p.lds_slots + (mode ? 1u : 0u)) * 256u * sizeof(double);
  int per_cu = lds_bytes ? (int)std::min<size_t>(8, (160u * 1024u) / lds_bytes) : 8;
  if (per_cu < 1) { set_error("interpreter LDS budget exceeded"); return FDG_E_INTERNAL; }
  const long grid = std::min<long>(nblk, (long)g->n_cu * per_cu);
  const size_t per_block = (size_t)(p.mem_slots + (staged ? p.L : 0u) + (mode ? R : 0u)) * 256u;
  const size_t ws_doubles = (size_t)grid * per_block + (mode ? (size_t)grid * R : 0u);
  rc = ensure_ws(g, std::max<size_t>(ws_doubles, 1) * sizeof(double));
  if (rc) return rc;
  double *ws = (double *)g->d_ws;
  double *partial = ws + (size_t)grid * per_block;
  const uint32_t *code = (const uint32_t *)g->d_code;
#define FDG_LAUNCH(M, S)                                                                              \
  do {                                                                                                \
    if (lds_bytes > 64 * 1024)                                                                        \
      HIP_TRY(hipFuncSetAttribute((const void *)fdg_interp<M, S>, hipFuncAttributeMaxDynamicSharedMemorySize, \
                                  (int)lds_bytes));                                                   \
    hipLaunchKernelGGL((fdg_interp<M, S>), dim3((unsigned)grid), dim3(256), lds_bytes, a.st, code, a.d_leaf, \
                       (long)a.ss, (long)a.ls, a.d_root, (long)a.rs, (long)a.rk, a.d_weight, partial, (long)a.B, ws,  \
                       p.lds_slots, p.mem_slots, p.L, R);                                              \
  } while (0)
  if (mode == 0) { if (staged) FDG_LAUNCH(0, true); else FDG_LAUNCH(0, false); }
  else { if (staged) FDG_LAUNCH(1, true); else FDG_LAUNCH(1, false); }
#undef FDG_LAUNCH
  HIP_TRY(hipGetLastError());
  if (mode == 1) {
    hipLaunchKernelGGL(fdg_reduce_partials, dim3(std::min<uint32_t>(R, 64u)), dim3(256), 0, a.st, partial,
                       (uint32_t)grid, R, a.d_acc);
    HIP_TRY(hipGetLastError());
  }
  return FDG_OK;
}

static int launch_reduce_lane_partials(double *part, uint32_t nwg, uint32_t R, double *acc, hipStream_t st) {
  hipLaunchKernelGGL(fdg_reduce_lane_partials, dim3(std::min<uint32_t>(R, 64u)), dim3(256), 0, st, part, nwg, R, acc);
  HIP_TRY(hipGetLastError());
  return FDG_OK;
}

struct IsaRun {
  fdg_graph *g;
  const RunArgs &a;
  const Lowered &p;
  const uint32_t R;
  const bool tiled;
  long ntiles = 0, grid = 0, grid2 = 0, grid3 = 0, grid4 = 0, grid5 = 0;
  size_t panel_all = 0;
  bool pool_ok = false, fused_acc = false, wide_ss = false, named = false;
  double *roots = nullptr;
  long a_rs = 0, a_rk = 0;

  IsaRun(fdg_graph *g_, const RunArgs &a_) : g(g_), a(a_), p(g_->prog), R(g_->prog.R), tiled(a_.lts != 0 || a_.rts != 0) {}

  const fdg_isa_kernel &K(int k) const { return g->kern[k]; }
  uint32_t waves_per_cu(const fdg_isa_kernel &k) const {
    return g->cfg.waves_per_cu > 0 ? (uint32_t)g->cfg.waves_per_cu : isa_waves_per_cu(k.vgpr, k.lds_bytes);
  }
  long oversub(long resident, size_t bytes_per_wg) const {
    if (g->cfg.waves_per_cu > 0) return resident;
    long f = g->cfg.oversub > 0 ? g->cfg.oversub : 8;
    while (f > 1 && (ntiles < resident * f * 4 || bytes_per_wg * (size_t)(resident * f) > ((size_t)32 << 20))) f >>= 1;
    return resident * f;
  }
  long shape(uint64_t valu, uint64_t bytes, const fdg_isa_kernel &k, size_t bytes_per_wg, bool accumulating = false) const {
    const long full = (long)waves_per_cu(k);
    const long mem_waves = g->cfg.mem_waves >= 0 ? g->cfg.mem_waves : (p.L >= 24 ? 4 : (accumulating ? 8 : 5));
    if (mem_waves > 0 && g->cfg.waves_per_cu <= 0 && g->cfg.oversub <= 0 && bytes && (double)valu < g->cfg.mem_ratio * (double)bytes && full > mem_waves) {
      long f = g->cfg.mem_oversub;
      while (f > 1 && ntiles < (long)g->n_cu * mem_waves * f * 4) f >>= 1;
      return (long)g->n_cu * mem_waves * f;
    }
    return oversub((long)g->n_cu * full, bytes_per_wg);
  }
  bool line_aligned(const void *base, long sample_stride, long col_stride) const {
    return sample_stride == 1 && (col_stride & 15) == 0 && ((uintptr_t)base & 127) == 0 && !g->cfg.no_streaming;
  }

  int plan() {
    ntiles = (long)((a.B + 63) / 64);
    const fdg_isa_kernel &ev = K(FDG_K_EVAL), &w2 = K(FDG_K_W2), &ac = K(FDG_K_ACC), &rm = K(FDG_K_RM), &rma = K(FDG_K_RM_ACC);
    grid = std::min<long>(ntiles, shape(g->st_valu[0], 8ull * (p.L + R), ev, (size_t)ev.mem_slots * 512u));
    grid2 = w2.present ? (long)g->n_cu * waves_per_cu(w2) : 0;
    const size_t panel = std::max((size_t)std::max<uint32_t>(ev.mem_slots, 1) * 512u * (size_t)grid,
                                  (size_t)std::max<uint32_t>(w2.mem_slots, 1) * 1024u * (size_t)grid2);
    pool_ok = K(FDG_K_POOL).present && K(FDG_K_POOL).fn && a.ss == 1 && a.ls > 0 && (g->pool_unit == 1 || a.ls == 64) &&
              (uint64_t)a.ls * 8u * (uint64_t)std::max<uint32_t>(p.L, 1) < (1ull << 31) && a.B >= 64 && !g->cfg.no_pool;
    fused_acc = a.mode == 1 && ac.present && !g->cfg.no_fused_acc && !(pool_ok && !g->cfg.pool_no_acc);
    grid3 = ac.present ? shape(g->st_valu[1], 8ull * p.L, ac, ((size_t)ac.mem_slots + R) * 512u, true) : 0;
    const size_t panel3 = (size_t)std::max<uint32_t>(ac.mem_slots, 1) * 512u * (size_t)grid3;
    grid4 = rm.present ? (long)g->n_cu * waves_per_cu(rm) : 0;
    const size_t panel4 = (size_t)std::max<uint32_t>(rm.mem_slots, 1) * 512u * (size_t)grid4;
    grid5 = rma.present ? (long)g->n_cu * waves_per_cu(rma) : 0;
    const size_t panel5 = (size_t)std::max<uint32_t>(rma.mem_slots, 1) * 512u * (size_t)grid5;
    panel_all = (std::max(std::max(panel, panel3), std::max(panel4, panel5)) + 4095) & ~(size_t)4095;
    int rc = ensure_ws(g, panel_all + (size_t)std::max(grid3, grid5) * R * 512u + 4096);
    if (rc) return rc;
    roots = a.d_root; a_rs = (long)a.rs; a_rk = (long)a.rk;
    if (a.mode == 1 && !fused_acc) {
      rc = ensure_root_scratch(g, (size_t)((a.B + 15) & ~(int64_t)15) * std::max<uint32_t>(R, 1) * sizeof(double) + (size_t)2048 * R * sizeof(double));
      if (rc) return rc;
      roots = (double *)g->d_ws2; a_rs = 1; a_rk = (long)((a.B + 15) & ~(int64_t)15);
    }
    wide_ss = a.ss < 0 || a.ss >= (1ll << 23);
    return FDG_OK;
  }

  int launch(int k, const double *lf, long lss, long lls, double *rt, long rrs, long rrk, long n, long nwg, const double *wt, long tls, long trs) {
    void *a_wsp = g->d_ws;
    void *args[] = {(void *)&lf, &lss, &lls, (void *)&rt, &rrs, &rrk, &a_wsp, &n, &nwg, (void *)&wt, &tls, &trs};
    HIP_TRY(hipModuleLaunchKernel((hipFunction_t)K(k).fn, (unsigned)nwg, 1, 1, K(k).threads, 1, 1, 0, a.st, args, nullptr));
    return FDG_OK;
  }
  int launch_reduced(int k, const double *lf, long lss, long lls, double *part, long n, long nwg, const double *wt, long tls) {
    const int rc = launch(k, lf, lss, lls, part, 0, 0, n, nwg, wt, tls, 0);
    return rc ? rc : launch_reduce_lane_partials(part, (uint32_t)nwg, R, a.d_acc, a.st);
  }
  int launch_acc(const double *lf, long lss, long lls, const double *wt, long n, long tls = 0) {
    double *part = (double *)((char *)g->d_ws + panel_all);
    if (!tls) tls = 64 * lss;
    const int k = K(FDG_K_ACC_NT).fn && line_aligned(lf, lss, lls) && (tls & 15) == 0 ? FDG_K_ACC_NT : FDG_K_ACC;
    if (!named) g->last_kernel = FDG_ISA_KERNEL[k];
    return launch_reduced(k, lf, lss, lls, part, n, std::min<long>((n + 63) / 64, grid3), wt, tls);
  }
  int launch_isa(const double *lf, long lss, long lls, double *rt, long rrs, long rrk, long n, long tls = 0, long trs = 0) {
    long done = 0;
    if (K(FDG_K_W2).present && lss == 1 && n >= 128 && !tls && !trs && !g->cfg.no_w2) {
      const long n2 = n & ~127l;
      const int rc = launch(FDG_K_W2, lf, lss, lls, rt, rrs, rrk, n2, std::min<long>(n2 / 128, grid2), nullptr, 128 * lss, 128 * rrs);
      if (rc) return rc;
      g->last_kernel = FDG_ISA_KERNEL[FDG_K_W2];
      done = n2;
    }
    if (done < n) {
      const double *lf1 = lf + done * lss;
      double *rt1 = rt + done * rrs;
      const long n1 = n - done;
      if (!tls) tls = 64 * lss;
      if (!trs) trs = 64 * rrs;
      const int k = K(FDG_K_NT).fn && line_aligned(lf1, lss, lls) && line_aligned(rt1, rrs, rrk) && ((tls | trs) & 15) == 0 ? FDG_K_NT : FDG_K_EVAL;
      if (!named && done == 0) g->last_kernel = FDG_ISA_KERNEL[k];
      return launch(k, lf1, lss, lls, rt1, rrs, rrk, n1, std::min<long>((n1 + 63) / 64, grid), nullptr, tls, trs);
    }
    return FDG_OK;
  }
  int finish_scratch_acc() {
    double *partial = roots + (size_t)a_rk * R;
    const uint32_t pb = weighted_segments((long)a.B, R);
    const uint8_t *live = nullptr;
    const int rcl = root_live_mask(g, &live);
    if (rcl) return rcl;
    hipLaunchKernelGGL(fdg_weighted_partials, dim3(pb * R), dim3(256), 0, a.st, roots, a_rk, a.d_weight, (long)a.B, R, pb, partial, live);
    hipLaunchKernelGGL(fdg_reduce_partials, dim3(std::min<uint32_t>(R, 64u)), dim3(256), 0, a.st, partial, pb, R, a.d_acc);
    HIP_TRY(hipGetLastError());
    return FDG_OK;
  }

  bool wants_pool() const { return pool_ok && ((a.mode == 0 && root_stride_ok(a)) || (a.mode == 1 && !fused_acc)); }
  int run_pool() {
    const int mode = a.mode;
    const long n4 = (long)(a.B & ~(int64_t)63), tail = (long)a.B - n4;
    double *rt0 = mode == 0 ? a.d_root : roots;
    const double *lf = a.d_leaf;
    long nwg = std::min<long>(n4 / 64, (long)g->n_cu), lss = a.ss, lls = a.ls, rrs = mode == 0 ? a.rs : a_rs, rrk = mode == 0 ? a.rk : a_rk;
    int rc = ensure_ws(g, std::max(panel_all + (size_t)grid3 * R * 512u + 4096, (size_t)g->pool_panel_wg * (size_t)nwg + 4096));
    if (rc) return rc;
    long tls = a.lts ? (long)a.lts : 64 * lss, trs = (mode == 0 && a.rts) ? (long)a.rts : 64 * rrs;
    rc = launch(FDG_K_POOL, lf, lss, lls, rt0, rrs, rrk, n4, nwg, nullptr, tls, trs);
    if (rc) return rc;
    g->last_kernel = FDG_ISA_KERNEL[FDG_K_POOL];
    named = true;
    if (tail) { rc = launch_isa(a.d_leaf + (size_t)(n4 / 64) * (size_t)tls, lss, lls, rt0 + (size_t)(n4 / 64) * (size_t)trs, rrs, rrk, tail, a.lts ? tls : 0, (mode == 0 && a.rts) ? trs : 0); if (rc) return rc; }
    return mode == 1 ? finish_scratch_acc() : FDG_OK;
  }

  bool wants_coop() const {
    return a.mode == 0 && K(FDG_K_COOP).present && g->coop_enabled && K(FDG_K_COOP).fn && !(a.ls == 1 && a.ss != 1 && p.L > 1) && !wide_ss && root_stride_ok(a) && !g->cfg.no_coop;
  }
  int run_coop() {
    const double *lf = a.d_leaf; double *rt = a.d_root;
    long nwg = std::min<long>((long)((a.B + 63) / 64), (long)g->n_cu), lss = a.ss, lls = a.ls, rrs = a.rs, rrk = a.rk, n = (long)a.B;
    int rc = ensure_ws(g, std::max(panel_all + (size_t)grid3 * R * 512u + 4096, (size_t)g->coop_panel_wg * (size_t)nwg + 4096));
    if (rc) return rc;
    rc = launch(FDG_K_COOP, lf, lss, lls, rt, rrs, rrk, n, nwg, nullptr, a.lts ? (long)a.lts : 64 * lss, a.rts ? (long)a.rts : 64 * rrs);
    if (rc) return rc;
    g->last_kernel = FDG_ISA_KERNEL[FDG_K_COOP];
    return FDG_OK;
  }

  int run_rl_acc() {
    const long n4 = (long)(a.B & ~(int64_t)63), tail = (long)a.B - n4;
    const long grid7 = (long)g->n_cu * waves_per_cu(K(FDG_K_RL_ACC));
    const size_t panel7 = ((size_t)std::max<uint32_t>(K(FDG_K_RL_ACC).mem_slots, 1) * 512u * (size_t)grid7 + 4095) & ~(size_t)4095;
    int rc = ensure_ws(g, std::max(panel_all, panel7) + (size_t)std::max(std::max(grid3, grid5), grid7) * R * 512u + 4096);
    if (rc) return rc;
    double *part = (double *)((char *)g->d_ws + std::max(panel_all, panel7));
    const long lss = a.ss, lls = a.ls;
    rc = launch_reduced(FDG_K_RL_ACC, a.d_leaf, lss, lls, part, n4, std::min<long>(n4 / 64, grid7), a.d_weight, 64 * lss);
    if (rc) return rc;
    g->last_kernel = FDG_ISA_KERNEL[FDG_K_RL_ACC];
    named = true;
    if (tail) { rc = launch_acc(a.d_leaf + (size_t)n4 * (size_t)a.ss, lss, lls, a.d_weight ? a.d_weight + n4 : nullptr, tail); if (rc) return rc; }
    return FDG_OK;
  }
  int run_rl() {
    const long n4 = (long)(a.B & ~(int64_t)63), tail = (long)a.B - n4;
    const long grid6 = (long)g->n_cu * waves_per_cu(K(FDG_K_RL));
    int rc = ensure_ws(g, std::max(panel_all + (size_t)std::max(grid3, grid5) * R * 512u + 4096, (size_t)std::max<uint32_t>(K(FDG_K_RL).mem_slots, 1) * 512u * (size_t)grid6 + 4096));
    if (rc) return rc;
    const long lss = a.ss, lls = a.ls, rrs = a.rs, rrk = a.rk;
    rc = launch(FDG_K_RL, a.d_leaf, lss, lls, a.d_root, rrs, rrk, n4, std::min<long>(n4 / 64, grid6), nullptr, 64 * lss, 64 * rrs);
    if (rc) return rc;
    g->last_kernel = FDG_ISA_KERNEL[FDG_K_RL];
    named = true;
    if (tail) { rc = launch_isa(a.d_leaf + (size_t)n4 * (size_t)a.ss, lss, lls, a.d_root + (size_t)n4 * (size_t)a.rs, rrs, rrk, tail); if (rc) return rc; }
    return FDG_OK;
  }

  bool wants_rm() const {
    const bool rm_shape = a.ls == 1 && a.ss >= (int64_t)p.L && !wide_ss && p.L >= 16 && a.B >= 64 && !tiled && !g->cfg.no_rm;
    return rm_shape && ((a.mode == 0 && K(FDG_K_RM).present && K(FDG_K_RM).fn && root_stride_ok(a)) || (fused_acc && K(FDG_K_RM_ACC).present && K(FDG_K_RM_ACC).fn));
  }
  int run_rm() {
    const long n4 = (long)(a.B & ~(int64_t)63), lss = a.ss, lls = a.ls, tail = (long)a.B - n4;
    int rc;
// ... 340 lines not shown
  std::lock_guard<std::mutex> lk(const_cast<fdg_graph *>(g)->mu);
  auto it = g->knobs.find(name);
  if (it == g->knobs.end()) return nullptr;
  std::string &h = hold[slot++ & 3u];
  h = it->second;
  return h.c_str();
}

int fdg_graph_set_association(fdg_graph *g, int assoc) {
  if (!g) { set_error("null handle"); return FDG_E_INVALID; }
  if (assoc != FDG_ASSOC_STATIC && assoc != FDG_ASSOC_INTERP) { set_error("unknown association"); return FDG_E_INVALID; }
  std::lock_guard<std::mutex> lk(g->mu);
  fdg::KnobScope knob_scope(&g->knobs);
  const bool want = assoc == FDG_ASSOC_INTERP;
  if (g->prog.assoc_interp == want) return FDG_OK;
  if (!g->code_object.empty() || !g->alt_code.empty() || !g->fused_code.empty() || !g->mc_code.empty() || g->cx_twin || g->mc_route ||
      !g->typed_code[1].empty() || !g->typed_code[2].empty() || !g->typed_code[3].empty()) {
    set_error("fdg_graph_set_association must be called before the handle is specialised"); return FDG_E_INVALID;
  }
  g->prog.assoc_interp = want;
  build_interpreter_program(g->prog, interp_lds_budget());
  if (g->d_code) { hipDeviceSynchronize(); hipFree(g->d_code); g->d_code = nullptr; }
  return FDG_OK;
}

int fdg_graph_release_device(fdg_graph *g) {
  if (!g) return FDG_OK;
  std::lock_guard<std::mutex> lk(g->mu);
  fdg::KnobScope knob_scope(&g->knobs);
  if (g->d_code) { hipFree(g->d_code); g->d_code = nullptr; }
  if (g->d_root_live) { hipFree(g->d_root_live); g->d_root_live = nullptr; }
  {
    fdg_ws_set cur;
    park_current_ws(g, cur);
    free_ws_set(cur);
    load_ws(g, fdg_ws_set());
    for (fdg_ws_set &w : g->ws_pool) free_ws_set(w);
    g->ws_pool.clear();
    g->ws_bound = true;
    g->ws_key = nullptr;
  }
  if (g->module) { hipModuleUnload((hipModule_t)g->module); g->module = nullptr; g->fn_eval_sm = g->fn_eval_gen = nullptr; forget_isa_kernels(g->kern); }
  if (g->fused_module) { hipModuleUnload((hipModule_t)g->fused_module); g->fused_module = nullptr; g->fn_fused = nullptr; }
  if (g->alt_module) { hipModuleUnload((hipModule_t)g->alt_module); g->alt_module = nullptr; g->fn_alt_sm = g->fn_alt_gen = nullptr; }
  if (g->mc_module) { hipModuleUnload((hipModule_t)g->mc_module); g->mc_module = nullptr; forget_isa_kernels(g->mc_kern); }
  if (g->cx_twin) fdg_graph_release_device(g->cx_twin);
  for (int t = 0; t < 4; ++t) if (g->typed_module[t]) { hipModuleUnload((hipModule_t)g->typed_module[t]); g->typed_module[t] = nullptr; g->fn_typed[t] = nullptr; }
  return FDG_OK;
}

int fdg_graph_destroy(fdg_graph *g) {
  if (!g) return FDG_OK;
  if (g->cx_twin) { fdg_graph_destroy(g->cx_twin); g->cx_twin = nullptr; }
  fdg_graph_release_device(g);
  delete g;
  return FDG_OK;
}

int fdg_graph_query(const fdg_graph *g, fdg_graph_info *o) {
  if (!g || !o) { set_error("null argument"); return FDG_E_INVALID; }
  const Lowered &p = g->prog;
  std::memset(o, 0, sizeof *o);
  o->n_leaf = p.L; o->n_node = p.N; o->n_root = p.R; o->n_edge = p.E;
  o->n_live_node = (uint32_t)p.order.size(); o->n_live_leaf = p.n_live_leaf;
  o->flops_alg = p.flops_alg; o->bytes_alg = 8ull * ((uint64_t)p.L + p.R);
  o->max_live = p.max_live; o->n_slot_lds = p.lds_slots; o->n_slot_mem = p.mem_slots; o->n_ops = p.n_ops;
  o->specialized = g->code_object.empty() ? 0 : 1;
  o->spec_vgpr = g->spec_vgpr; o->spec_lds_bytes = g->spec_lds; o->spec_scratch_bytes = g->spec_scratch;
  return FDG_OK;
}

int fdg_graph_kernel_info(fdg_graph *g, fdg_kernel_info *o) {
  if (!g || !o) { set_error("null argument"); return FDG_E_INVALID; }
  std::lock_guard<std::mutex> lk(g->mu);
  fdg::KnobScope knob_scope(&g->knobs);
  std::memset(o, 0, sizeof *o);
  std::snprintf(o->last_kernel, sizeof o->last_kernel, "%s", g->last_kernel ? g->last_kernel : "");
  if (!(g->isa && !g->code_object.empty())) return FDG_OK;
  for (int i = 0; i < 3; ++i) { o->n_valu[i] = g->st_valu[i]; o->n_ld_leaf[i] = g->st_ld_leaf[i]; o->n_panel[i] = g->st_panel[i]; o->n_lds[i] = g->st_lds[i]; }
  const int slot[3] = {FDG_K_EVAL, FDG_K_ACC, FDG_K_RM};
  for (int i = 0; i < 3; ++i) if (g->kern[slot[i]].present) o->waves_per_cu[i] = isa_waves_per_cu(g->kern[slot[i]].vgpr, g->kern[slot[i]].lds_bytes);
  o->has_acc = g->kern[FDG_K_ACC].present; o->has_rm = g->kern[FDG_K_RM].present; o->has_coop = g->kern[FDG_K_COOP].present && g->coop_enabled; o->rm_bufs = g->rm_bufs;
  o->has_pool = g->kern[FDG_K_POOL].present; o->pool_fetch = g->pool_fetch; o->pool_valu = g->pool_valu;
  o->has_rl = g->kern[FDG_K_RL].present; o->rl_reserved = 0; o->rl_valu = g->rl_valu;
  return FDG_OK;
}

int fdg_graph_emit_source(const fdg_graph *g, unsigned flags, char **source) {
  const fdg::KnobMap knobs_now = knobs_snapshot(g);
  fdg::KnobScope knob_scope(g ? &knobs_now : nullptr);
  if (!g || !source) { set_error("null argument"); return FDG_E_INVALID; }
  std::string s = emit_hip_source(g->prog, flags);
  char *m = (char *)std::malloc(s.size() + 1);
  if (!m) { set_error("out of memory"); return FDG_E_NOMEM; }
  std::memcpy(m, s.c_str(), s.size() + 1);
  *source = m;
  return FDG_OK;
}

static void apply_land_env(fdg::OptParams &q);
static fdg::OptParams to_params(const fdg_opt_params *q) {
  fdg::OptParams prm;
  if (q) {
    if (q->n_reg) prm.n_reg = std::min<uint32_t>(q->n_reg, 125);
    if (q->n_lds) prm.n_lds = std::min<uint32_t>(q->n_lds, 127);
    if (q->lookahead_lds) prm.lookahead_lds = q->lookahead_lds;
    if (q->lookahead_mem) prm.lookahead_mem = q->lookahead_mem;
    if (q->lookahead_leaf) prm.lookahead_leaf = q->lookahead_leaf;
    if (q->n_acc) prm.n_acc = std::min<uint32_t>(q->n_acc, 124);
    if (q->vn_window) prm.vn_window = q->vn_window;
    prm.fma = q->fma != 0;
    prm.remat_window = q->remat_window;
    if (q->remat_cost) prm.remat_cost = std::min<uint32_t>(q->remat_cost, 64);
  }
  return prm;
}

int fdg_graph_set_schedule_groups(fdg_graph *g, const uint32_t *group, uint32_t n_node) {
  if (!g) { set_error("null handle"); return FDG_E_INVALID; }
  std::lock_guard<std::mutex> lk(g->mu);
  fdg::KnobScope knob_scope(&g->knobs);
  if (!group) { g->prog.sched_group.clear(); return FDG_OK; }
  if (n_node != g->prog.N) { set_error("schedule groups: length differs from n_node"); return FDG_E_INVALID; }
  g->prog.sched_group.assign(group, group + n_node);
  return FDG_OK;
}

int fdg_graph_set_opt_params(fdg_graph *g, const fdg_opt_params *prm) {
  if (!g || !prm) { set_error("null argument"); return FDG_E_INVALID; }
  std::lock_guard<std::mutex> lk(g->mu);
  fdg::KnobScope knob_scope(&g->knobs);
  g->opt = *prm;
  g->has_opt = true;
  return FDG_OK;
}

static fdg_opt_params get_opt_params(const fdg_graph *g) { return g->opt; }

int fdg_graph_opt_program(const fdg_graph *g, const fdg_opt_params *q, fdg_mop **ops, uint64_t *n_ops,
                          uint32_t *n_reg_used, uint32_t *n_lds_used, uint32_t *n_mem_used, uint32_t *n_acc_used) {
  const fdg::KnobMap knobs_now = knobs_snapshot(g);
  fdg::KnobScope knob_scope(g ? &knobs_now : nullptr);
  if (!g || !ops || !n_ops) { set_error("null argument"); return FDG_E_INVALID; }
  fdg::OptProgram prog;
  fdg::OptParams prm = to_params(q);
  apply_land_env(prm);
  fdg::build_opt_program(g->prog, prm, prog);
  if (!prog.supported) { set_error("optimizing back end does not cover this graph: " + prog.why); return FDG_E_UNSUPPORTED; }
  fdg_mop *m = (fdg_mop *)std::malloc(std::max<size_t>(1, prog.ops.size()) * sizeof(fdg_mop));
  if (!m) { set_error("out of memory"); return FDG_E_NOMEM; }
  for (size_t i = 0; i < prog.ops.size(); ++i) {
    const fdg::MOp &o = prog.ops[i];
    m[i] = fdg_mop{o.kind, o.nega, o.negb, o.negc, o.d, o.a, o.b, o.imm, o.c, o.param};
  }
  *ops = m; *n_ops = prog.ops.size();
  if (n_reg_used) *n_reg_used = prog.n_reg_used;
  if (n_lds_used) *n_lds_used = prog.n_lds_used;
  if (n_mem_used) *n_mem_used = prog.n_mem_used;
  if (n_acc_used) *n_acc_used = prog.n_acc_used;
  return FDG_OK;
}

static uint32_t coop_waves() { const char *e = fdg::knob("FDG_COOP_WAVES"); const int n = e ? std::atoi(e) : 8; return n == 4 ? 4u : (n == 16 ? 16u : 8u); }

static uint32_t pool_waves() { const char *e = fdg::knob("FDG_POOL_WAVES"); const int n = e ? std::atoi(e) : 4; return n == 8 ? 8u : 4u; }
static fdg::OptParams pool_params(fdg::OptParams q, uint32_t nw) {
  q.n_reg = std::min<uint32_t>(q.n_reg ? q.n_reg : 120, 120);
// ... 34 lines not shown
  const uint32_t nw = coop_waves();
  if (nw >= 8) prm.n_acc = 0;
  if (nw == 16) prm.n_reg = std::min<uint32_t>(prm.n_reg, 58);
  fdg::build_coop_program(g->prog, prm, cp, nw);
  if (cp.supported && wave >= cp.n_wave) { set_error("wave out of range"); return FDG_E_INVALID; }
  if (!cp.supported) { set_error("the cooperative variant does not cover this graph: " + cp.why); return FDG_E_UNSUPPORTED; }
  return coop_program_out(cp, wave, ops, n_ops, info);
}

static int coop_program_out(const fdg::CoopProgram &cp, uint32_t wave, fdg_mop **ops, uint64_t *n_ops, uint32_t *info) {
  const fdg::OptProgram &prog = cp.wave[wave];
  fdg_mop *m = (fdg_mop *)std::malloc(std::max<size_t>(1, prog.ops.size()) * sizeof(fdg_mop));
  if (!m) { set_error("out of memory"); return FDG_E_NOMEM; }
  for (size_t i = 0; i < prog.ops.size(); ++i) {
    const fdg::MOp &o = prog.ops[i];
    m[i] = fdg_mop{o.kind, o.nega, o.negb, o.negc, o.d, o.a, o.b, o.imm, o.c, o.param};
  }
  *ops = m; *n_ops = prog.ops.size();
  if (info) {
    info[0] = prog.n_reg_used; info[1] = prog.n_lds_used; info[2] = prog.n_mem_used; info[3] = prog.n_acc_used;
    info[4] = cp.n_shared; info[5] = cp.n_epoch; info[6] = (uint32_t)cp.n_transfer; info[7] = (uint32_t)cp.n_duplicate;
  }
  return FDG_OK;
}

int fdg_graph_mc_program(const fdg_graph *g, const fdg_leaf_tables *tab, const fdg_opt_params *q, fdg_mop **ops, uint64_t *n_ops,
                         uint32_t *n_reg_used, uint32_t *n_lds_used, uint32_t *n_mem_used, uint32_t *n_acc_used) {
  const fdg::KnobMap knobs_now = knobs_snapshot(g);
  fdg::KnobScope knob_scope(g ? &knobs_now : nullptr);
  if (!g || !tab || !ops || !n_ops) { set_error("null argument"); return FDG_E_INVALID; }
  if (tab->n_leaf != g->prog.L) { set_error("leaf tables: n_leaf differs from the graph's"); return FDG_E_INVALID; }
  fdg::LeafSpec ls; ls.tab = tab; ls.kF = tab->kF; ls.beta = tab->beta; ls.lambda = tab->lambda;
  fdg::OptProgram prog;
  fdg::build_mc_program(g->prog, ls, to_params(q), prog);
  if (!prog.supported) { set_error("the fused ISA step does not cover this graph / these leaves: " + prog.why); return FDG_E_UNSUPPORTED; }
  fdg_mop *m = (fdg_mop *)std::malloc(std::max<size_t>(1, prog.ops.size()) * sizeof(fdg_mop));
  if (!m) { set_error("out of memory"); return FDG_E_NOMEM; }
  for (size_t i = 0; i < prog.ops.size(); ++i) {
    const fdg::MOp &o = prog.ops[i];
    m[i] = fdg_mop{o.kind, o.nega, o.negb, o.negc, o.d, o.a, o.b, o.imm, o.c, o.param};
  }
  *ops = m; *n_ops = prog.ops.size();
  if (n_reg_used) *n_reg_used = prog.n_reg_used;
  if (n_lds_used) *n_lds_used = prog.n_lds_used;
  if (n_mem_used) *n_mem_used = prog.n_mem_used;
  if (n_acc_used) *n_acc_used = prog.n_acc_used;
  return FDG_OK;
}

static bool has_opt_params(const fdg_graph *g) { return g->has_opt; }

static int assemble_isa(const fdg_graph *g, const fdg::IsaPrograms &V, const std::string &dir, unsigned flags, std::vector<char> &co, std::string &hash,
                        std::vector<fdg::IsaKernelRecord> &records) {
  records.clear();
  const std::string src = fdg::emit_isa(g->prog, V, &records);
  char hbuf[40];
  std::snprintf(hbuf, sizeof hbuf, "%016llx", (unsigned long long)fnv1a(src, fnv1a("isa")));
  hash = hbuf;
  const std::string base = dir + "/fdg_isa_" + hbuf;
  if (!read_cached(dir, std::string("fdg_isa_") + hbuf + ".hsaco", co)) {
    const std::string tmp = base + tmp_suffix();
    if (!write_file(tmp + ".s", src.c_str(), src.size())) { set_error("cannot write " + tmp + ".s"); return FDG_E_JIT; }
    const char *llvm = fdg::knob("FDG_LLVM_BIN");
    const std::string bin = llvm ? llvm : "/opt/rocm/lib/llvm/bin";
    int rc = run_cmd({bin + "/clang", "-x", "assembler", "-target", "amdgcn-amd-amdhsa", "-mcpu=gfx950", "-c", tmp + ".s", "-o", tmp + ".o"}, tmp + ".log");
    if (rc == 0) rc = run_cmd({bin + "/ld.lld", "-shared", tmp + ".o", "-o", tmp + ".hsaco"}, tmp + ".log");
    const std::string log = slurp_and_remove(tmp + ".log");
    std::remove((tmp + ".o").c_str());
    if (flags & FDG_SPEC_KEEP_SOURCE) std::rename((tmp + ".s").c_str(), (base + ".s").c_str());
    else std::remove((tmp + ".s").c_str());
    if (rc == 0) ::chmod((tmp + ".hsaco").c_str(), 0644);
    if (rc != 0 || std::rename((tmp + ".hsaco").c_str(), (base + ".hsaco").c_str()) != 0 || !read_file(base + ".hsaco", co)) {
      std::remove((tmp + ".hsaco").c_str());
      set_error("assembling the ISA kernel failed:\n" + log.substr(0, 2000));
      return FDG_E_JIT;
    }
  } else if (flags & FDG_SPEC_KEEP_SOURCE) {
    write_file(base + ".s", src.c_str(), src.size());
  }
  return FDG_OK;
}

static void fill_isa_kernels(fdg_isa_kernel *kern, const fdg::IsaPrograms &V, const std::vector<fdg::IsaKernelRecord> &records) {
  const fdg::OptProgram *prog[FDG_K_COUNT] = {V.main, V.main, V.w2_prog(), V.acc_prog(), V.acc_prog(), V.rm_prog(), V.rm_acc_prog(), V.rl_prog(), V.rl_acc_prog(), nullptr, nullptr};
  for (int k = 0; k < FDG_K_COUNT; ++k) {
    kern[k] = fdg_isa_kernel();
    for (const fdg::IsaKernelRecord &r : records) {
      if (r.name != V.kname + fdg_isa_suffix(k)) continue;
      kern[k].present = true;
      kern[k].vgpr = r.vgpr; kern[k].lds_bytes = r.lds_bytes; kern[k].threads = r.threads;
      if (prog[k]) kern[k].mem_slots = prog[k]->n_mem_used;
    }
  }
}
static uint32_t panel_bytes_per_wg(const fdg::CoopProgram &cp) {
  uint32_t bytes = 0;
  for (uint32_t w = 0; w < cp.n_wave; ++w) bytes += std::max<uint32_t>(cp.wave[w].n_mem_used, 1) * 512u;
  return bytes;
}

static void install_isa(fdg_graph *g, const fdg::IsaPrograms &V, std::vector<char> &co, const std::string &hash, unsigned flags,
                        const std::vector<fdg::IsaKernelRecord> &records) {
  if (g->module) { hipModuleUnload((hipModule_t)g->module); g->module = nullptr; }
  fill_isa_kernels(g->kern, V, records);
  const fdg_isa_kernel *K = g->kern;
  if (K[FDG_K_RL].present) g->rl_valu = V.prl.n_valu;
  if (K[FDG_K_POOL].present) {
    g->pool_panel_wg = panel_bytes_per_wg(V.pool);
    g->pool_fetch = (uint32_t)V.pool.n_transfer;
    g->pool_unit = V.pool.pool_unit;
    g->pool_valu = 0;
    for (uint32_t w = 0; w < V.pool.n_wave; ++w) g->pool_valu += V.pool.wave[w].n_valu;
  }
  g->coop_enabled = K[FDG_K_COOP].present;
  if (K[FDG_K_COOP].present) g->coop_panel_wg = panel_bytes_per_wg(V.coop);
  g->code_object.swap(co);
  g->isa = true;
  g->spec_vgpr = K[FDG_K_EVAL].vgpr; g->spec_lds = K[FDG_K_EVAL].lds_bytes; g->spec_scratch = 0;
  const fdg::OptProgram *pp[3] = {V.main, V.acc_prog(), V.rm_prog()};
  for (int i = 0; i < 3; ++i) {
    g->st_valu[i] = pp[i] ? pp[i]->n_valu : 0;
    g->st_ld_leaf[i] = pp[i] ? (uint32_t)pp[i]->n_ld_leaf : 0;
    g->st_panel[i] = pp[i] ? (uint32_t)(pp[i]->n_ld_mem + pp[i]->n_st_mem) : 0;
    g->st_lds[i] = pp[i] ? (uint32_t)(pp[i]->n_ld_lds + pp[i]->n_st_lds) : 0;
  }
  g->rm_bufs = V.rm_bufs;
  g->last_kernel = "";
  g->spec_source_hash = hash;
  g->spec_flags = flags;
}

static void build_prog(const fdg_graph *g, fdg::OptParams prm, fdg::OptProgram &out) {
  prm.fma = prm.fma || g->isa_fma;
  if (const char *e = fdg::knob("FDG_LA_LDS")) prm.lookahead_lds = (uint32_t)std::max(1, std::atoi(e));
  if (const char *e = fdg::knob("FDG_LA_LDS_B")) { if (prm.n_acc) prm.lookahead_lds = (uint32_t)std::max(1, std::atoi(e)); }
  if (fdg::knob("FDG_ROOTS_LAST") && !g->isa_fma) prm.roots_last = true;
  fdg::build_opt_program(g->prog, prm, out);
}

static fdg::OptParams cfg_S() { fdg::OptParams S; S.n_reg = 28; S.n_lds = 1; S.n_acc = 0; S.lookahead_leaf = 300; S.vn_window = 200; return S; }
static fdg::OptParams cfg_A() { fdg::OptParams A; A.n_reg = 120; A.n_lds = 40; A.n_acc = 0; A.lookahead_leaf = 300; A.vn_window = 200; return A; }
static fdg::OptParams cfg_B() {
  fdg::OptParams B; B.n_reg = 120; B.n_lds = 80; B.n_acc = 124; B.lookahead_leaf = 100; B.lookahead_mem = 64; B.vn_window = 1000; return B;
}

static void apply_land_env(fdg::OptParams &q) {
  if (const char *e = fdg::knob("FDG_LAND")) q.n_land = q.n_acc ? std::min<uint32_t>((uint32_t)std::max(0, std::atoi(e)), q.n_acc / 2) : 0;
  if (const char *e = fdg::knob("FDG_LAND_LA")) q.lookahead_land = (uint32_t)std::max(1, std::atoi(e));
}

static fdg::OptParams auto_program(const fdg_graph *g, fdg::OptProgram &prog) {
  fdg::OptProgram ps;
  build_prog(g, cfg_S(), ps);
  const bool small_ok = ps.supported && ps.n_ld_leaf <= g->prog.n_live_leaf && ps.n_ld_lds + ps.n_st_lds + ps.n_ld_mem + ps.n_st_mem == 0;
  if (small_ok) { prog = std::move(ps); return cfg_S(); }
  build_prog(g, cfg_A(), prog);
  if (prog.supported && (prog.n_ld_mem + prog.n_st_mem) * 100 > prog.n_valu) {
    fdg::OptProgram pb;
    fdg::OptParams qb = cfg_B();
    apply_land_env(qb);
    build_prog(g, qb, pb);
    if (pb.supported) { prog = std::move(pb); return qb; }
  }
  return cfg_A();
}

static std::string tuned_path(const fdg_graph *g, const std::string &dir) {
  const fdg::Lowered &p = g->prog;
  uint64_t th = fnv1a("tuned-v2");
  auto mix = [&](const void *d, size_t n) { th = fnv1a(std::string((const char *)d, n), th); };
  mix(&p.L, 4); mix(&p.N, 4); mix(&p.R, 4);
  if (p.N) { mix(p.op.data(), p.op.size()); mix(p.power.data(), p.power.size() * 4); mix(p.off.data(), p.off.size() * 4); }
  if (p.E) { mix(p.idx.data(), p.idx.size() * 4); mix(p.fac.data(), p.fac.size() * 8); }
  if (p.R) mix(p.root_slot.data(), p.root_slot.size() * 4);
  if (!p.sched_group.empty()) mix(p.sched_group.data(), p.sched_group.size() * 4);
  if (p.assoc_interp) mix("eval!", 5);
  char hb[40];
  std::snprintf(hb, sizeof hb, "%016llx", (unsigned long long)th);
  return dir + "/fdg_tuned_" + hb + ".txt";
}

static fdg::OptParams cfg_W2() { fdg::OptParams q; q.n_reg = 60; q.n_lds = 20; q.n_acc = 0; q.lookahead_leaf = 300; q.vn_window = 200; return q; }
static fdg::OptParams cfg_W2T() { fdg::OptParams q; q.n_reg = 14; q.n_lds = 1; q.n_acc = 0; q.lookahead_leaf = 300; q.vn_window = 200; return q; }

static bool auto_program_w2(const fdg_graph *g, fdg::OptProgram &p2) {
  if (!fdg::knob("FDG_ISA_W2")) return false;
  const fdg::Lowered &p = g->prog;
  build_prog(g, cfg_W2T(), p2);
  bool ok = p2.supported && p2.n_ld_leaf <= p.n_live_leaf && p2.n_ld_lds + p2.n_st_lds + p2.n_ld_mem + p2.n_st_mem == 0;
  if (!ok) {
    build_prog(g, cfg_W2(), p2);
    ok = p2.supported && p2.n_ld_mem + p2.n_st_mem == 0;
  }
  if (!ok) return false;
  for (const fdg::MOp &o : p2.ops)
    if (fdg::mop_is_macro(o.kind) || o.kind == fdg::M_FMAK || o.kind == fdg::M_CONST || o.kind == fdg::M_FMA || o.kind == fdg::M_FMAC) return false;
// ... 942 lines not shown
```

### include/fdg.h

```cpp
#ifndef FDG_H
#define FDG_H

#include <stddef.h>
#include <stdint.h>

#ifdef __cplusplus
extern "C" {
#endif

#define FDG_VERSION 102

#define FDG_OP_SUM 0u
#define FDG_OP_PROD 1u
#define FDG_OP_POWER 2u
#define FDG_NO_ROOT 0xFFFFFFFFu

enum {
  FDG_OK = 0,
  FDG_E_INVALID = -1,
  FDG_E_UNSUPPORTED = -2,
  FDG_E_NO_DEVICE = -3,
  FDG_E_NOMEM = -4,
  FDG_E_JIT = -5,
  FDG_E_INTERNAL = -6
};

typedef struct fdg_graph_desc {
  uint32_t n_leaf;
  uint32_t n_node;
  uint32_t n_root;
  uint32_t n_edge;
  const uint8_t *op;
  const int32_t *power;
  const uint32_t *child_off;
  const uint32_t *child_idx;
  const double *child_fac;
  const uint32_t *root_slot;
} fdg_graph_desc;

typedef struct fdg_graph fdg_graph;

typedef struct fdg_graph_info {
  uint32_t n_leaf, n_node, n_root, n_edge;
  uint32_t n_live_node;
  uint32_t n_live_leaf;
  uint64_t flops_alg;
  uint64_t bytes_alg;
  uint32_t max_live;
  uint32_t n_slot_lds;
  uint32_t n_slot_mem;
  uint32_t n_ops;
  int32_t specialized;
  uint32_t spec_vgpr, spec_lds_bytes, spec_scratch_bytes;
} fdg_graph_info;

#define FDG_SPEC_DEFAULT 0u
#define FDG_SPEC_KEEP_SOURCE 1u
#define FDG_SPEC_FAST_MATH 2u
#define FDG_SPEC_AUTOTUNE 8u
#define FDG_SPEC_ROW_MAJOR_COMPANION 16u
#define FDG_SPEC_ISA 4u

const char *fdg_last_error(void);
int fdg_version(void);

int fdg_graph_create(const fdg_graph_desc *desc, fdg_graph **out);
int fdg_graph_destroy(fdg_graph *g);
int fdg_graph_query(const fdg_graph *g, fdg_graph_info *info);

#define FDG_ASSOC_STATIC 0
#define FDG_ASSOC_INTERP 1
int fdg_graph_set_association(fdg_graph *g, int assoc);

int fdg_graph_set_option(fdg_graph *g, const char *name, const char *value);
const char *fdg_graph_get_option(const fdg_graph *g, const char *name);
int fdg_set_default_option(const char *name, const char *value);
const char *fdg_get_default_option(const char *name);

typedef struct fdg_kernel_info {
  char last_kernel[48];
  uint64_t n_valu[3];
  uint32_t n_ld_leaf[3];
  uint32_t n_panel[3];
  uint32_t n_lds[3];
  uint32_t waves_per_cu[3];
  uint32_t has_acc, has_rm, has_coop, rm_bufs;
  uint32_t has_pool;
  uint32_t pool_fetch;
  uint64_t pool_valu;
  uint32_t has_rl;
  uint32_t rl_reserved;
  uint64_t rl_valu;
} fdg_kernel_info;
int fdg_graph_kernel_info(fdg_graph *g, fdg_kernel_info *info);

int fdg_graph_emit_source(const fdg_graph *g, unsigned flags, char **source);
void fdg_free(void *p);

int fdg_graph_specialize(fdg_graph *g, const char *cache_dir, unsigned flags);

typedef struct fdg_opt_params {
  uint32_t n_reg;
  uint32_t n_lds;
  uint32_t lookahead_lds;
  uint32_t lookahead_mem;
  uint32_t lookahead_leaf;
  uint32_t n_acc;
  uint32_t vn_window;
  uint32_t fma;
  uint32_t remat_window;
  uint32_t remat_cost;
} fdg_opt_params;

typedef struct fdg_mop {
  uint8_t kind, nega, negb, negc;
  uint32_t d, a, b;
  double imm;
  uint32_t c, param;
} fdg_mop;

int fdg_graph_set_schedule_groups(fdg_graph *g, const uint32_t *group, uint32_t n_node);

int fdg_graph_set_opt_params(fdg_graph *g, const fdg_opt_params *prm);
int fdg_graph_opt_program(const fdg_graph *g, const fdg_opt_params *prm, fdg_mop **ops, uint64_t *n_ops,
                          uint32_t *n_reg_used, uint32_t *n_lds_used, uint32_t *n_mem_used, uint32_t *n_acc_used);

int fdg_graph_coop_program(const fdg_graph *g, const fdg_opt_params *prm, uint32_t wave, fdg_mop **ops, uint64_t *n_ops,
                           uint32_t *info);

int fdg_graph_pool_program(const fdg_graph *g, const fdg_opt_params *prm, uint32_t wave, fdg_mop **ops, uint64_t *n_ops,
                           uint32_t *info);

#define FDG_DT_F64 0
#define FDG_DT_F32 1
#define FDG_DT_C64 2
#define FDG_DT_C32 3
int fdg_graph_specialize_typed(fdg_graph *g, int dtype, const char *cache_dir, unsigned flags);
int fdg_graph_create_complex_view(const fdg_graph *g, fdg_graph **out);
int fdg_eval_device_typed(fdg_graph *g, int dtype, const void *d_leaf, int64_t leaf_sample_stride, int64_t leaf_leaf_stride,
                          void *d_root, int64_t root_sample_stride, int64_t root_root_stride, int64_t n_sample, void *stream);

int fdg_eval_device(fdg_graph *g, const double *d_leaf, int64_t leaf_sample_stride,
                    int64_t leaf_leaf_stride, double *d_root, int64_t root_sample_stride,
                    int64_t root_root_stride, int64_t n_sample, void *stream);

int fdg_eval(fdg_graph *g, const double *leaf, double *root, int64_t n_sample);

int fdg_eval_strided(fdg_graph *g, const double *leaf, int64_t leaf_sample_stride, int64_t leaf_leaf_stride,
                     double *root, int64_t root_sample_stride, int64_t root_root_stride, int64_t n_sample);

int fdg_accumulate_device(fdg_graph *g, const double *d_leaf, int64_t leaf_sample_stride,
                          int64_t leaf_leaf_stride, const double *d_weight, double *d_acc,
                          int64_t n_sample, void *stream);

#define FDG_TILE_SAMPLES 64
int fdg_eval_device_tiled(fdg_graph *g, const double *d_leaf, int64_t leaf_sample_stride, int64_t leaf_leaf_stride,
                          int64_t leaf_tile_stride, double *d_root, int64_t root_sample_stride, int64_t root_root_stride,
                          int64_t root_tile_stride, int64_t n_sample, void *stream);
int fdg_accumulate_device_tiled(fdg_graph *g, const double *d_leaf, int64_t leaf_sample_stride, int64_t leaf_leaf_stride,
                                int64_t leaf_tile_stride, const double *d_weight, double *d_acc, int64_t n_sample, void *stream);
#define FDG_BIN_MAX 16384
int fdg_accumulate_device_binned(fdg_graph *g, const double *d_leaf, int64_t leaf_sample_stride,
                                 int64_t leaf_leaf_stride, int64_t leaf_tile_stride,
                                 const int32_t *d_bin, int32_t bin_base, uint32_t n_bin,
                                 const double *d_weight, double *d_acc, int64_t n_sample, void *stream);
int fdg_accumulate_device_moments(fdg_graph *g, const double *d_leaf, int64_t leaf_sample_stride, int64_t leaf_leaf_stride,
                                  int64_t leaf_tile_stride, const int32_t *d_bin, int32_t bin_base, uint32_t n_bin,
                                  const double *d_weight, double *d_acc, double *d_acc2, int64_t n_sample, void *stream);

int fdg_fill_uniform_device_tiled(double *d_leaf, int64_t n_sample, uint32_t n_leaf, int64_t leaf_sample_stride,
                                  int64_t leaf_leaf_stride, int64_t leaf_tile_stride, uint64_t seed, uint64_t sample_offset,
                                  void *stream);

int fdg_repack_tile_major(const double *d_src, int64_t sample_stride, int64_t col_stride, double *d_tiled, int64_t n_sample,
// ... 345 lines not shown
```

Baseline: 9.259 billion.

## Add atomic tile-claiming kernel variants for dynamic work distribution on memory-bound graphs

Adds new ISA kernel variants (eval_cl, nt_cl) in which each workgroup claims its next run of tiles through a global atomic counter instead of a static grid-stride walk. Runs of several tiles (default 4) are claimed per atomic to amortise its cost. The runtime picks these variants by default for memory-bound graphs with many tiles per workgroup, resetting the counter with a memset before each launch. The goal is to balance load across CUs and tail workgroups, at the cost of an extra memset, an atomic round trip per run, one fewer pool SGPR pair, and a changed kernel-info struct field.

```diff
diff --git a/feynmandiagram.jl_amd/capi.py b/feynmandiagram.jl_amd/capi.py
--- a/feynmandiagram.jl_amd/capi.py
+++ b/feynmandiagram.jl_amd/capi.py
@@ -99,7 +99,7 @@
                 ("n_panel", C.c_uint32 * 3), ("n_lds", C.c_uint32 * 3), ("waves_per_cu", C.c_uint32 * 3),
                 ("has_acc", C.c_uint32), ("has_rm", C.c_uint32), ("has_coop", C.c_uint32), ("rm_bufs", C.c_uint32),
                 ("has_pool", C.c_uint32), ("pool_fetch", C.c_uint32), ("pool_valu", C.c_uint64),
-                ("has_rl", C.c_uint32), ("rl_reserved", C.c_uint32), ("rl_valu", C.c_uint64)]
+                ("has_rl", C.c_uint32), ("last_launch", C.c_uint32), ("rl_valu", C.c_uint64)]
 
 
 class LeafTables(C.Structure):
@@ -398,6 +398,8 @@
             out[k] = [int(x) for x in getattr(ki, k)]
         for k in ("has_acc", "has_rm", "has_coop", "rm_bufs", "has_pool", "pool_fetch", "pool_valu", "has_rl", "rl_valu"):
             out[k] = int(getattr(ki, k))
+        out["last_grid"] = int(ki.last_launch) & 0x7FFFFFFF
+        out["tile_walk"] = "claimed" if int(ki.last_launch) >> 31 else "static"
         return out
 
     def emit_source(self, flags: int = 0) -> str:
diff --git a/feynmandiagram.jl_amd/csrc/fdg_internal.h b/feynmandiagram.jl_amd/csrc/fdg_internal.h
--- a/feynmandiagram.jl_amd/csrc/fdg_internal.h
+++ b/feynmandiagram.jl_amd/csrc/fdg_internal.h
@@ -74,13 +74,14 @@
   long mem_waves = -1;
   long mem_oversub = 1;
   double mem_ratio = 2.5;
+  int tile_claim = -1;
   uint64_t sm_chunk_bytes = 1ull << 29;
   long long eval_chunk = 0, mc_chunk = 0;
 };
 
-enum { FDG_K_EVAL = 0, FDG_K_NT, FDG_K_W2, FDG_K_ACC, FDG_K_ACC_NT, FDG_K_RM, FDG_K_RM_ACC, FDG_K_RL, FDG_K_RL_ACC, FDG_K_COOP, FDG_K_POOL, FDG_K_COUNT };
+enum { FDG_K_EVAL = 0, FDG_K_NT, FDG_K_W2, FDG_K_ACC, FDG_K_ACC_NT, FDG_K_RM, FDG_K_RM_ACC, FDG_K_RL, FDG_K_RL_ACC, FDG_K_COOP, FDG_K_POOL, FDG_K_EVAL_CL, FDG_K_NT_CL, FDG_K_COUNT };
 static const char *const FDG_ISA_KERNEL[FDG_K_COUNT] = {"fdg_isa_eval", "fdg_isa_eval_nt", "fdg_isa_eval_w2", "fdg_isa_eval_acc", "fdg_isa_eval_acc_nt",
-    "fdg_isa_eval_rm", "fdg_isa_eval_rm_acc", "fdg_isa_eval_rl", "fdg_isa_eval_rl_acc", "fdg_isa_eval_coop", "fdg_isa_eval_pool"};
+    "fdg_isa_eval_rm", "fdg_isa_eval_rm_acc", "fdg_isa_eval_rl", "fdg_isa_eval_rl_acc", "fdg_isa_eval_coop", "fdg_isa_eval_pool", "fdg_isa_eval_cl", "fdg_isa_eval_nt_cl"};
 inline const char *fdg_isa_suffix(int k) { return FDG_ISA_KERNEL[k] + sizeof("fdg_isa_eval") - 1; }
 struct fdg_isa_kernel {
   bool present = false;
@@ -115,6 +116,8 @@
   uint64_t st_valu[3] = {0, 0, 0};
   uint32_t st_ld_leaf[3] = {0, 0, 0}, st_panel[3] = {0, 0, 0}, st_lds[3] = {0, 0, 0};
   const char *last_kernel = "";
+  uint32_t claim_run = 0;
+  uint32_t last_launch = 0;
   uint32_t rm_bufs = 0;
   uint64_t rl_valu = 0;
   bool coop_enabled = false;
diff --git a/feynmandiagram.jl_amd/csrc/fdg_isa.cpp b/feynmandiagram.jl_amd/csrc/fdg_isa.cpp
--- a/feynmandiagram.jl_amd/csrc/fdg_isa.cpp
+++ b/feynmandiagram.jl_amd/csrc/fdg_isa.cpp
@@ -11,6 +11,13 @@
 #include "fdg_opt.h"
 
 namespace fdg {
+int isa_claim_run_log2() {
+  const char *e = fdg::knob("FDG_ISA_CLAIM_RUN");
+  const long tiles = e ? std::atol(e) : 4;
+  int r = 0;
+  while (r < 6 && (1l << (r + 1)) <= tiles) ++r;
+  return r;
+}
 namespace {
 
 constexpr int V_LANE8 = 1, V_LEAFOFF = 2, V_ROOTOFF = 3, V_TMP = 4, V_BASE = 6;
@@ -135,7 +142,7 @@
     if (hz_starts(op, "s_addc") || hz_starts(op, "s_subb") || hz_starts(op, "s_cselect")) {}
     return I;
   }
-  if (hz_starts(op, "global_load") || hz_starts(op, "global_store") || hz_starts(op, "buffer_") || hz_starts(op, "flat_")) {
+  if (hz_starts(op, "global_load") || hz_starts(op, "global_store") || hz_starts(op, "global_atomic") || hz_starts(op, "buffer_") || hz_starts(op, "flat_")) {
     I.vmem = true;
     I.store = op.find("store") != std::string::npos;
     if (op.find("_lds_") != std::string::npos) {
@@ -440,7 +447,7 @@
 struct CoopSec { uint32_t wave, n_shared, priv_base_bytes, panel_wg_bytes, panel_prefix_bytes; bool pooled = false; uint32_t pool_unit = 1;
                  uint32_t slack = 0, flag_base_bytes = 0, n_wave = 4; };
 static KernelMeta emit_kernel(Emit &E, const Lowered &p, const OptProgram &prog, const std::string &kname, int W, bool accumulate = false,
-                              uint32_t rm_bufs = 0, const CoopSec *cs = nullptr, bool rl = false) {
+                              uint32_t rm_bufs = 0, const CoopSec *cs = nullptr, bool rl = false, bool claim_tiles = false) {
   E.vm_issued = E.lg_issued = E.vm_done = E.lg_done = 0;
   E.pend.assign(std::max<uint32_t>(prog.n_reg_used, 1), {0, 0});
   const uint32_t SLOT = 512u * W;
@@ -505,6 +512,10 @@
   int tile_rot = 0;
   if (dbg && std::strstr(dbg, "rot") && !cs && !tile_run && !tile_xcd) tile_rot = std::max(0, std::atoi(std::strstr(dbg, "rot") + 3));
   const int S_ROTB = S_POOL + 2 * (N_POOL - 1), S_ROTS = S_ROTB + 1;
+  const bool claim = claim_tiles && W == 1 && !cs && !accumulate && !rm_bufs && !rl && prog.mc_n_k == 0 && prog.mc_n_t == 0 && !tile_run && !tile_xcd && !tile_rot;
+  const int claim_run = claim ? isa_claim_run_log2() : 0;
+  const int S_CLAIM = S_POOL + 2 * (N_POOL - 1);
+  uint64_t claim_seq = 0;
   E.vm_slack = (dbg && std::strstr(dbg, "noackwait") && !accumulate) ? p.R : 0;
   E.no_vm_wait = dbg && std::strstr(dbg, "novmwait");
   if (cs) E.ins("v_and_b32_e32 v0, 63, v0");
@@ -519,6 +530,7 @@
   const int tile_arg = mc ? 0x80 : 0x50;
   E.ins("s_load_dwordx2 " + S2(S_LTS) + ", s[0:1], " + hex32((uint32_t)tile_arg));
   if (!accumulate) E.ins("s_load_dwordx2 " + S2(S_RTS) + ", s[0:1], " + hex32((uint32_t)tile_arg + 8));
+  if (claim) E.ins("s_load_dwordx2 " + S2(S_CLAIM) + ", s[0:1], " + hex32((uint32_t)tile_arg + 16));
   if (mc) {
     E.ins("s_load_dwordx4 s[" + std::to_string(S_LEAF2) + ":" + std::to_string(S_LEAF2 + 3) + "], s[0:1], 0x50");
     E.ins("s_load_dwordx8 s[" + std::to_string(S_PARAM) + ":" + std::to_string(S_PARAM + 7) + "], s[0:1], 0x60");
@@ -651,7 +663,7 @@
     std::vector<std::pair<int, uint64_t>> v;
     for (auto &kv : hist) v.push_back({kv.second, kv.first});
     std::sort(v.begin(), v.end(), [](const auto &x, const auto &y) { return x.first > y.first || (x.first == y.first && x.second < y.second); });
-    for (size_t i = 0; i < v.size() && i < (size_t)(mc ? N_POOL_MC : (has_macro ? N_POOL : 16)); ++i) pool.push_back(v[i].second);
+    for (size_t i = 0; i < v.size() && i < (size_t)(mc ? N_POOL_MC : (has_macro ? N_POOL - (claim ? 1 : 0) : 16)); ++i) pool.push_back(v[i].second);
   }
   for (size_t k = 0; k < pool.size(); ++k) {
     E.ins("s_mov_b32 " + S(S_POOL + 2 * (int)k) + ", " + hex32((uint32_t)pool[k]));
@@ -672,6 +684,7 @@
     E.ins("s_add_u32 " + S(S_A) + ", " + S(S_A) + ", " + S(S_T));
     E.ins("s_min_u32 " + S(S_NTILES) + ", " + S(S_A) + ", " + S(S_NTILES));
   }
+  else if (claim_run) E.ins("s_lshl_b32 " + S(S_TILE) + ", s2, " + std::to_string(claim_run));
   else {
     E.ins("s_mov_b32 " + S(S_TILE) + ", s2");
     if (tile_rot) { E.ins("s_mov_b32 " + S(S_ROTB) + ", 0"); E.ins("s_mov_b32 " + S(S_ROTS) + ", s2"); }
@@ -696,7 +709,7 @@
     std::vector<std::pair<uint64_t, uint32_t>> v;
     for (auto &kv : hist) v.push_back({kv.second, kv.first});
     std::sort(v.begin(), v.end(), [](const auto &x, const auto &y) { return x.first > y.first || (x.first == y.first && x.second < y.second); });
-    for (size_t i = 0; i < v.size() && pool.size() + i < (size_t)N_POOL; ++i) {
+    for (size_t i = 0; i < v.size() && pool.size() + i < (size_t)(N_POOL - (claim ? 1 : 0)); ++i) {
       const int r = S_POOL + 2 * (int)(pool.size() + i);
       panel_base[v[i].second] = r;
       E.ins("s_add_u32 " + S(r) + ", " + S(S_PANEL) + ", " + hex32(v[i].second * 8192u));
@@ -708,6 +721,18 @@
   E.ins("s_endpgm");
   os << ".Ltile" << sfx << ":\n";
   if (cs && cs->slack) E.ins("s_mov_b32 " + S(S_DELTA + 7) + ", " + S(S_DELTA + 6));
+  const int v_claim = (int)(tmp0 + 2 * n_tmp_pairs);
+  if (claim) {
+    if (claim_run) {
+      E.ins("s_and_b32 " + S(S_X) + ", " + S(S_TILE) + ", " + std::to_string((1 << claim_run) - 1));
+      E.ins("s_cbranch_scc1 .Lheld" + sfx);
+    }
+    E.ins("s_mov_b64 exec, 1");
+    E.ins("v_mov_b32_e32 " + V(V_TMP) + ", 1");
+    E.ins("global_atomic_add " + V(v_claim) + ", " + V(V_LANE8) + ", " + V(V_TMP) + ", " + S2(S_CLAIM) + " sc0");
+    if (claim_run) os << ".Lheld" << sfx << ":\n";
+    claim_seq = ++E.vm_issued;
+  }
   E.ins("s_mov_b32 " + S(S_X + 1) + ", 0");
   E.ins("s_mov_b32 " + S(S_X) + ", " + S(S_TILE));
   E.ins("s_lshl_b64 " + S2(S_X) + ", " + S2(S_X) + ", " + std::to_string(TSH));
@@ -1288,6 +1313,23 @@
     E.ins("s_sub_u32 " + S(S_X) + ", " + S(S_NWG) + ", 1");
     E.ins("s_and_b32 " + S(S_ROTS) + ", " + S(S_ROTS) + ", " + S(S_X));
     E.ins("s_add_u32 " + S(S_TILE) + ", " + S(S_ROTB) + ", " + S(S_ROTS));
+  } else if (claim) {
+    if (claim_run) {
+      E.ins("s_add_u32 " + S(S_TILE) + ", " + S(S_TILE) + ", 1");
+      E.ins("s_and_b32 " + S(S_X) + ", " + S(S_TILE) + ", " + std::to_string((1 << claim_run) - 1));
+      E.ins("s_cbranch_scc1 .Lrun" + sfx);
+    }
+    if (claim_seq > E.vm_done) {
+      const uint64_t n = std::min<uint64_t>(E.vm_issued - claim_seq, 63);
+      E.ins("s_waitcnt vmcnt(" + std::to_string(n) + ")");
+      E.vm_done = std::max(std::max(E.vm_done, E.vm_issued - n), claim_seq);
+    }
+    E.ins("v_readfirstlane_b32 " + S(S_TILE) + ", " + V(v_claim));
+    E.ins("s_add_u32 " + S(S_TILE) + ", " + S(S_TILE) + ", " + S(S_NWG));
+    if (claim_run) {
+      E.ins("s_lshl_b32 " + S(S_TILE) + ", " + S(S_TILE) + ", " + std::to_string(claim_run));
+      os << ".Lrun" << sfx << ":\n";
+    }
   } else {
     E.ins("s_add_u32 " + S(S_TILE) + ", " + S(S_TILE) + ", " + S(S_NWG));
   }
@@ -1340,16 +1382,16 @@
   E.ins("s_setpc_b64 " + S2(S_A));
   E.ins("s_endpgm");
 
-  const uint32_t next_vgpr = std::max<uint32_t>(V_BASE + RW * std::max<uint32_t>(prog.n_reg_used, 1) + 2 * acc_pairs_v + 2 * n_tmp_pairs + (rm_bufs ? 10 : 0) + (cs ? (cs->slack ? 7 : 4) : 0) + (rl ? 2 : 0), 8);
+  const uint32_t next_vgpr = std::max<uint32_t>(V_BASE + RW * std::max<uint32_t>(prog.n_reg_used, 1) + 2 * acc_pairs_v + 2 * n_tmp_pairs + (rm_bufs ? 10 : 0) + (cs ? (cs->slack ? 7 : 4) : 0) + (rl ? 2 : 0) + (claim ? 1 : 0), 8);
   const uint32_t accum = (next_vgpr + 3) & ~3u;
   const uint32_t n_agpr = RW * prog.n_acc_used + (aa ? 2 * p.R : 0);
   if (cs) return KernelMeta{kname, lds_bytes, accum, n_agpr, 12, (mc || has_macro) ? S_END : S_POOL + 2 * 16};
   os << "\t.section\t.rodata,\"a\",@progbits\n\t.p2align\t6, 0x0\n\t.amdhsa_kernel " << kname << "\n";
   os << "\t\t.amdhsa_group_segment_fixed_size " << lds_bytes << "\n";
-  os << "\t\t.amdhsa_private_segment_fixed_size 0\n\t\t.amdhsa_kernarg_size " << (mc ? 144 : 96) << "\n\t\t.amdhsa_user_sgpr_count 2\n";
+  os << "\t\t.amdhsa_private_segment_fixed_size 0\n\t\t.amdhsa_kernarg_size " << (mc ? 144 : (claim ? 104 : 96)) << "\n\t\t.amdhsa_user_sgpr_count 2\n";
   os << "\t\t.amdhsa_user_sgpr_kernarg_segment_ptr 1\n\t\t.amdhsa_system_sgpr_workgroup_id_x 1\n";
   os << "\t\t.amdhsa_system_vgpr_workitem_id 0\n";
-  const int n_sgpr = (mc || has_macro) ? S_END : S_POOL + 2 * 16;
+  const int n_sgpr = (mc || has_macro || claim) ? S_END : S_POOL + 2 * 16;
   os << "\t\t.amdhsa_next_free_vgpr " << (accum + n_agpr) << "\n\t\t.amdhsa_next_free_sgpr " << n_sgpr << "\n";
   os << "\t\t.amdhsa_accum_offset " << accum << "\n\t\t.amdhsa_reserve_vcc 1\n";
   os << "\t\t.amdhsa_float_round_mode_32 0\n\t\t.amdhsa_float_round_mode_16_64 0\n";
@@ -1357,7 +1399,7 @@
   os << "\t\t.amdhsa_dx10_clamp 1\n\t\t.amdhsa_ieee_mode 1\n";
   os << "\t.end_amdhsa_kernel\n";
   (void)p;
-  return KernelMeta{kname, lds_bytes, accum, n_agpr, mc ? 18 : 12, n_sgpr};
+  return KernelMeta{kname, lds_bytes, accum, n_agpr, mc ? 18 : (claim ? 13 : 12), n_sgpr};
 }
 
 }
@@ -1457,6 +1499,10 @@
   return os.str();
 }
 
+static bool isa_has_claimed(const Lowered &p, const OptProgram &prog) {
+  return prog.mc_n_k == 0 && prog.mc_n_t == 0 && prog.ops.size() <= 60000 && (double)prog.n_valu < 10.0 * 8.0 * (double)(p.L + p.R);
+}
+
 std::string emit_isa(const Lowered &p, const IsaPrograms &V, std::vector<IsaKernelRecord> *records) {
   const OptProgram &prog = *V.main, *prog2 = V.w2_prog(), *prog_acc = V.acc_prog(), *prog_rm = V.rm_prog(), *prog_rm_acc = V.rm_acc_prog(), *prog_rl = V.rl_prog(),
                    *prog_rl_acc = V.rl_acc_prog();
@@ -1493,6 +1539,14 @@
   if (prog_rl_acc) ks.push_back(emit_kernel(E, p, *prog_rl_acc, kname + "_rl_acc", 1, true, 0, nullptr, true));
   if (coop) { ks.push_back(emit_coop(E, p, *coop, kname + "_coop")); ks.back().wg = 64 * coop->n_wave; }
   if (pool) { ks.push_back(emit_coop(E, p, *pool, kname + "_pool")); ks.back().wg = 64 * pool->n_wave; }
+  if (isa_has_claimed(p, prog)) {
+    ks.push_back(emit_kernel(E, p, prog, kname + "_cl", 1, false, 0, nullptr, false, true));
+    if (!fdg::knob("FDG_ISA_NO_STREAMING")) {
+      E.streaming = true;
+      ks.push_back(emit_kernel(E, p, prog, kname + "_nt_cl", 1, false, 0, nullptr, false, true));
+      E.streaming = false;
+    }
+  }
   std::ostringstream &os = E.os;
   os << "\t.text\n\t.amdgpu_metadata\n---\namdhsa.kernels:\n";
   const char *kinds[18] = {"global_buffer", "by_value", "by_value", "global_buffer", "by_value", "by_value",
@@ -1501,7 +1555,7 @@
   for (const KernelMeta &k : ks) {
     os << "  - .agpr_count: " << k.n_agpr << "\n    .args:\n";
     for (int i = 0; i < k.n_args; ++i) {
-      const char *kind = (k.n_args == 12 && i >= 10) ? "by_value" : kinds[i];
+      const char *kind = (k.n_args <= 13 && i >= 10) ? (i == 12 ? "global_buffer" : "by_value") : kinds[i];
       os << "      - .offset: " << i * 8 << "\n        .size: 8\n        .value_kind: " << kind << "\n";
       if (std::strcmp(kind, "global_buffer") == 0) os << "        .address_space: global\n";
     }
diff --git a/feynmandiagram.jl_amd/csrc/fdg_opt.h b/feynmandiagram.jl_amd/csrc/fdg_opt.h
--- a/feynmandiagram.jl_amd/csrc/fdg_opt.h
+++ b/feynmandiagram.jl_amd/csrc/fdg_opt.h
@@ -140,6 +140,7 @@
 };
 struct IsaKernelRecord { std::string name; uint32_t vgpr = 0 , lds_bytes = 0, threads = 64; };
 std::string emit_isa(const Lowered &p, const IsaPrograms &V, std::vector<IsaKernelRecord> *records = nullptr);
+int isa_claim_run_log2();
 
 void rm_plan_stats(const Lowered &p, const OptProgram &prog, uint32_t bufs, uint64_t &fetches, uint64_t &gathers);
 int check_isa_hazards(const std::string &text, std::string &report);
diff --git a/feynmandiagram.jl_amd/csrc/fdg_runtime.hip b/feynmandiagram.jl_amd/csrc/fdg_runtime.hip
--- a/feynmandiagram.jl_amd/csrc/fdg_runtime.hip
+++ b/feynmandiagram.jl_amd/csrc/fdg_runtime.hip
@@ -580,6 +580,7 @@
   if (const char *e = get("FDG_ISA_MEM_WAVES")) c.mem_waves = std::max(0l, std::atol(e));
   if (const char *e = get("FDG_ISA_MEM_OVERSUB")) c.mem_oversub = std::max(1l, std::atol(e));
   if (const char *e = get("FDG_ISA_MEM_RATIO")) c.mem_ratio = std::atof(e);
+  if (const char *e = get("FDG_ISA_TILE_CLAIM")) c.tile_claim = e[0] != '0' ? 1 : 0;
   if (const char *e = get("FDG_SM_CHUNK_MB")) c.sm_chunk_bytes = (uint64_t)std::max(1, std::atoi(e)) << 20;
   if (const char *e = get("FDG_EVAL_CHUNK")) c.eval_chunk = std::atoll(e);
   if (const char *e = get("FDG_MC_CHUNK")) c.mc_chunk = std::atoll(e);
@@ -739,7 +740,8 @@
   const bool tiled;
   long ntiles = 0, grid = 0, grid2 = 0, grid3 = 0, grid4 = 0, grid5 = 0;
   size_t panel_all = 0;
-  bool pool_ok = false, fused_acc = false, wide_ss = false, named = false;
+  bool pool_ok = false, fused_acc = false, wide_ss = false, named = false, claim = false;
+  size_t claim_off = 0;
   double *roots = nullptr;
   long a_rs = 0, a_rk = 0;
 
@@ -755,10 +757,15 @@
     while (f > 1 && (ntiles < resident * f * 4 || bytes_per_wg * (size_t)(resident * f) > ((size_t)32 << 20))) f >>= 1;
     return resident * f;
   }
+  long mem_waves_of(bool accumulating) const { return g->cfg.mem_waves >= 0 ? g->cfg.mem_waves : (p.L >= 24 ? 4 : (accumulating ? 8 : 5)); }
+  bool mem_bound(uint64_t valu, uint64_t bytes, const fdg_isa_kernel &k, bool accumulating) const {
+    return mem_waves_of(accumulating) > 0 && g->cfg.waves_per_cu <= 0 && g->cfg.oversub <= 0 && bytes && (double)valu < g->cfg.mem_ratio * (double)bytes &&
+           (long)waves_per_cu(k) > mem_waves_of(accumulating);
+  }
   long shape(uint64_t valu, uint64_t bytes, const fdg_isa_kernel &k, size_t bytes_per_wg, bool accumulating = false) const {
     const long full = (long)waves_per_cu(k);
-    const long mem_waves = g->cfg.mem_waves >= 0 ? g->cfg.mem_waves : (p.L >= 24 ? 4 : (accumulating ? 8 : 5));
-    if (mem_waves > 0 && g->cfg.waves_per_cu <= 0 && g->cfg.oversub <= 0 && bytes && (double)valu < g->cfg.mem_ratio * (double)bytes && full > mem_waves) {
+    const long mem_waves = mem_waves_of(accumulating);
+    if (mem_bound(valu, bytes, k, accumulating)) {
       long f = g->cfg.mem_oversub;
       while (f > 1 && ntiles < (long)g->n_cu * mem_waves * f * 4) f >>= 1;
       return (long)g->n_cu * mem_waves * f;
@@ -786,7 +793,9 @@
     grid5 = rma.present ? (long)g->n_cu * waves_per_cu(rma) : 0;
     const size_t panel5 = (size_t)std::max<uint32_t>(rma.mem_slots, 1) * 512u * (size_t)grid5;
     panel_all = (std::max(std::max(panel, panel3), std::max(panel4, panel5)) + 4095) & ~(size_t)4095;
-    int rc = ensure_ws(g, panel_all + (size_t)std::max(grid3, grid5) * R * 512u + 4096);
+    claim = g->cfg.tile_claim != 0 && K(FDG_K_EVAL_CL).present && mem_bound(g->st_valu[0], 8ull * (p.L + R), ev, false);
+    claim_off = panel_all + (size_t)std::max(grid3, grid5) * R * 512u + 4096;
+    int rc = ensure_ws(g, claim_off + 256);
     if (rc) return rc;
     roots = a.d_root; a_rs = (long)a.rs; a_rk = (long)a.rk;
     if (a.mode == 1 && !fused_acc) {
@@ -800,8 +809,11 @@
 
   int launch(int k, const double *lf, long lss, long lls, double *rt, long rrs, long rrk, long n, long nwg, const double *wt, long tls, long trs) {
     void *a_wsp = g->d_ws;
-    void *args[] = {(void *)&lf, &lss, &lls, (void *)&rt, &rrs, &rrk, &a_wsp, &n, &nwg, (void *)&wt, &tls, &trs};
+    void *a_cnt = (char *)g->d_ws + claim_off;
+    void *args[] = {(void *)&lf, &lss, &lls, (void *)&rt, &rrs, &rrk, &a_wsp, &n, &nwg, (void *)&wt, &tls, &trs, &a_cnt};
+    if (k == FDG_K_EVAL_CL || k == FDG_K_NT_CL) HIP_TRY(hipMemsetAsync(a_cnt, 0, 4, a.st));
     HIP_TRY(hipModuleLaunchKernel((hipFunction_t)K(k).fn, (unsigned)nwg, 1, 1, K(k).threads, 1, 1, 0, a.st, args, nullptr));
+    g->last_launch = (uint32_t)nwg | ((k == FDG_K_EVAL_CL || k == FDG_K_NT_CL) ? FDG_LAUNCH_CLAIMED : 0u);
     return FDG_OK;
   }
   int launch_reduced(int k, const double *lf, long lss, long lls, double *part, long n, long nwg, const double *wt, long tls) {
@@ -830,9 +842,11 @@
       const long n1 = n - done;
       if (!tls) tls = 64 * lss;
       if (!trs) trs = 64 * rrs;
-      const int k = K(FDG_K_NT).fn && line_aligned(lf1, lss, lls) && line_aligned(rt1, rrs, rrk) && ((tls | trs) & 15) == 0 ? FDG_K_NT : FDG_K_EVAL;
+      int k = K(FDG_K_NT).fn && line_aligned(lf1, lss, lls) && line_aligned(rt1, rrs, rrk) && ((tls | trs) & 15) == 0 ? FDG_K_NT : FDG_K_EVAL;
       if (!named && done == 0) g->last_kernel = FDG_ISA_KERNEL[k];
-      return launch(k, lf1, lss, lls, rt1, rrs, rrk, n1, std::min<long>((n1 + 63) / 64, grid), nullptr, tls, trs);
+      long run = 1;
+      if (claim && (g->cfg.tile_claim > 0 || (n1 + 63) / 64 >= 256 * grid) && K(k == FDG_K_NT ? FDG_K_NT_CL : FDG_K_EVAL_CL).fn) { k = k == FDG_K_NT ? FDG_K_NT_CL : FDG_K_EVAL_CL; run = 1l << g->claim_run; }
+      return launch(k, lf1, lss, lls, rt1, rrs, rrk, n1, std::min<long>(((n1 + 63) / 64 + run - 1) / run, grid), nullptr, tls, trs);
     }
     return FDG_OK;
   }
@@ -1339,7 +1353,7 @@
   for (int i = 0; i < 3; ++i) if (g->kern[slot[i]].present) o->waves_per_cu[i] = isa_waves_per_cu(g->kern[slot[i]].vgpr, g->kern[slot[i]].lds_bytes);
   o->has_acc = g->kern[FDG_K_ACC].present; o->has_rm = g->kern[FDG_K_RM].present; o->has_coop = g->kern[FDG_K_COOP].present && g->coop_enabled; o->rm_bufs = g->rm_bufs;
   o->has_pool = g->kern[FDG_K_POOL].present; o->pool_fetch = g->pool_fetch; o->pool_valu = g->pool_valu;
-  o->has_rl = g->kern[FDG_K_RL].present; o->rl_reserved = 0; o->rl_valu = g->rl_valu;
+  o->has_rl = g->kern[FDG_K_RL].present; o->last_launch = g->last_launch; o->rl_valu = g->rl_valu;
   return FDG_OK;
 }
 
@@ -1540,7 +1554,7 @@
 }
 
 static void fill_isa_kernels(fdg_isa_kernel *kern, const fdg::IsaPrograms &V, const std::vector<fdg::IsaKernelRecord> &records) {
-  const fdg::OptProgram *prog[FDG_K_COUNT] = {V.main, V.main, V.w2_prog(), V.acc_prog(), V.acc_prog(), V.rm_prog(), V.rm_acc_prog(), V.rl_prog(), V.rl_acc_prog(), nullptr, nullptr};
+  const fdg::OptProgram *prog[FDG_K_COUNT] = {V.main, V.main, V.w2_prog(), V.acc_prog(), V.acc_prog(), V.rm_prog(), V.rm_acc_prog(), V.rl_prog(), V.rl_acc_prog(), nullptr, nullptr, V.main, V.main};
   for (int k = 0; k < FDG_K_COUNT; ++k) {
     kern[k] = fdg_isa_kernel();
     for (const fdg::IsaKernelRecord &r : records) {
@@ -1570,6 +1584,7 @@
     g->pool_valu = 0;
     for (uint32_t w = 0; w < V.pool.n_wave; ++w) g->pool_valu += V.pool.wave[w].n_valu;
   }
+  g->claim_run = (uint32_t)fdg::isa_claim_run_log2();
   g->coop_enabled = K[FDG_K_COOP].present;
   if (K[FDG_K_COOP].present) g->coop_panel_wg = panel_bytes_per_wg(V.coop);
   g->code_object.swap(co);
diff --git a/include/fdg.h b/include/fdg.h
--- a/include/fdg.h
+++ b/include/fdg.h
@@ -77,6 +77,7 @@
 int fdg_set_default_option(const char *name, const char *value);
 const char *fdg_get_default_option(const char *name);
 
+#define FDG_LAUNCH_CLAIMED 0x80000000u
 typedef struct fdg_kernel_info {
   char last_kernel[48];
   uint64_t n_valu[3];
@@ -89,7 +90,7 @@
   uint32_t pool_fetch;
   uint64_t pool_valu;
   uint32_t has_rl;
-  uint32_t rl_reserved;
+  uint32_t last_launch;
   uint64_t rl_valu;
 } fdg_kernel_info;
 int fdg_graph_kernel_info(fdg_graph *g, fdg_kernel_info *info);
```

After: 9.763 billion, median of 6. 5.4% higher.
